# lms-07/LGTEUN

Hardware: AMD Instinct MI355X
Metric: train image-pairs/sec, GF-2 4-band 128x128, K=4, bs=32/GPU (higher is better)
Workload: dtype f32 (GEMMs and the local mixer: split 16-bit MFMA -- f16 pairs in the forward FFN, the W2 products of its backward and P V, bf16 triples elsewhere -- fp32 accumulate; fp32-equivalent); 1 GPU; BASELINE configs[1]: C=4, MS 32x32, PAN 128x128, K=4, 32 pairs/GPU, train step = fwd + L1 + bwd + Adam + StepLR tick; mode=faithful, global_batch=32, parallelism=dp1, dropout=True

## Files before the change

### include/lgteun_hip.h

```cpp
#ifndef LGTEUN_HIP_H
#define LGTEUN_HIP_H

#include <stddef.h>
#include <stdint.h>

#ifdef __cplusplus
extern "C" {
#endif

#define LG_TENSORS_SHARED 12
#define LG_TENSORS_PER_STAGE 119

#define LG_FLAG_FAITHFUL 1
#define LG_FLAG_SAVE 2
#define LG_FLAG_DROPOUT 4

#define LG_FLAG_BWD_LGT 8
#define LG_FLAG_BWD_DATA 16

#define LG_FLAG_CHAINED 32

#define LG_FLAG_DEFER_DEAD 64

enum lg_kernel_id {
    LG_K_NONE = 0, LG_K_FFN1, LG_K_FFN2, LG_K_FFT, LG_K_ATTN, LG_K_UPFUSE, LG_K_DOWN, LG_K_EMBED, LG_K_TAIL, LG_K_DATASTEP,
    LG_K_FFN1_BWD, LG_K_FFN2_BWD, LG_K_FFT_BWD, LG_K_ATTN_BWD, LG_K_WGRAD, LG_K_BATCH, LG_K_COUNT
};

typedef struct lg_config {
    int32_t C;
    int32_t K;
    int32_t H, W;
    int32_t precision;
    uint32_t variant;
} lg_config;

#define LG_VAR_FFN_IMPL_MASK 3u
#define LG_VAR_FFN_STRIP 1u
#define LG_VAR_FFN_TILE 2u
#define LG_VAR_FFN_XP 3u
#define LG_VAR_FFN_SAVE_MASK (3u << 2)
#define LG_VAR_FFN_SAVE3 (1u << 2)
#define LG_VAR_FFN_SAVE5 (2u << 2)
#define LG_VAR_FFN_BWD32_PAIR (1u << 4)
#define LG_VAR_FFN_DWBWD_TILE (1u << 5)
#define LG_VAR_ATTN_BWD_R3 (1u << 6)
#define LG_VAR_DSTEP_TILES (1u << 7)
#define LG_VAR_ATTN_FWD_VALU (1u << 8)
#define LG_VAR_FFN_BF16X3 (1u << 9)
#define LG_VAR_FFT_FULL (1u << 10)
#define LG_VAR_FFN_BWD_BF16X3 (1u << 11)
#define LG_VAR_ATTN_BWD_CORE_M (1u << 12)
#define LG_VAR_FFN_XS (1u << 13)
#define LG_VAR_ATTN_BF16X3 (1u << 14)
#define LG_VAR_FFN_H3_RECOMPUTE (1u << 15)
#define LG_VAR_ATTN_BWD_RESTATS (1u << 16)
#define LG_VAR_REDUCE_PER_BLOCK (1u << 17)
#define LG_VAR_ALL 0x3ffffu

typedef struct lg_plan lg_plan;

const char* lg_version(void);
#define LG_ABI_VERSION 2
int32_t lg_abi_version(void);
const char* lg_last_error(void);

int lg_plan_create(const lg_config* cfg, const int64_t* offsets, int32_t n_offsets, lg_plan** out);
void lg_plan_destroy(lg_plan* plan);
size_t lg_workspace_bytes(const lg_plan* plan, int32_t B, int32_t train);

int lgteun_forward(const lg_plan* plan, const float* params, const float* ms, const float* pan, float* out,
                   void* workspace, size_t workspace_bytes, int32_t B, int32_t flags, uint64_t seed, void* stream);

int lgteun_dead_forward(const lg_plan* plan, const float* params, void* workspace, size_t workspace_bytes, int32_t B, int32_t flags,
                        uint64_t seed, void* stream);

int lgteun_backward(const lg_plan* plan, const float* params, float* grads, const float* ms, const float* pan,
                    const float* dout, void* workspace, size_t workspace_bytes, int32_t B, int32_t flags,
                    uint64_t seed, void* stream);

int lg_l1_loss(const float* out, const float* gt, float* dout, float* loss_accum, int64_t n_local, int64_t n_global,
               float scale, void* stream);

int lg_adam_step(float* params, const float* grads, float* exp_avg, float* exp_avg_sq, const int64_t* ranges,
                 int32_t n_ranges, int64_t max_range, int32_t step, float lr, float beta1, float beta2, float eps,
                 float grad_scale, void* stream);

int lg_l2_loss(const float* out, const float* gt, float* dout, float* loss_accum, int64_t n_local, int64_t n_global,
               float scale, void* stream);

#define LG_OPT_ADAM 0
#define LG_OPT_ADAMW 1
#define LG_OPT_SGD 2
#define LG_OPT_RMSPROP 3
#define LG_OPT_AMSGRAD 1
#define LG_OPT_NESTEROV 2
#define LG_OPT_CENTERED 4
int lg_optim_step(float* params, const float* grads, float* state0, float* state1, float* state2, const int64_t* ranges,
                  int32_t n_ranges, int64_t max_range, int32_t step, int32_t algo, int32_t flags, double lr, double h0, double h1,
                  double eps, double weight_decay, double grad_scale, void* stream);

int lg_prof_enable(int32_t kernel_id, int32_t max_launches);
int lg_prof_reset(void);
void lg_prof_pause(int32_t paused);
int lg_prof_read(double* total_ms, int64_t* launches);
void lg_prof_disable(void);
const char* lg_kernel_name(int32_t kernel_id);

int lg_dropout_mask(uint64_t seed, int32_t stage, int32_t blk, int64_t first, int64_t n, float* out, void* stream);

int lg_op_resample(const float* x, float* y, int32_t planes, int32_t hi, int32_t wi, int32_t mode, void* stream);
int lg_op_data_step(const lg_plan* plan, const float* params, int32_t stage, const float* z_in, const float* ms,
                    const float* pan, float* z_out, float* tmp, int32_t B, void* stream);
int lg_op_lgt(const lg_plan* plan, const float* params, int32_t stage, const float* z, float* out, void* workspace,
              size_t workspace_bytes, int32_t B, int32_t flags, uint64_t seed, void* stream);
int lg_op_block(const lg_plan* plan, const float* params, int32_t stage, int32_t blk, int32_t which, const float* x,
                float* y, void* workspace, size_t workspace_bytes, int32_t B, void* stream);

int lg_op_block_bwd(const lg_plan* plan, const float* params, float* grads, int32_t stage, int32_t blk, int32_t which,
                    const float* x, const float* dy, float* dx, void* workspace, size_t workspace_bytes, int32_t B,
                    void* stream);

int lg_op_data_step_bwd(const lg_plan* plan, const float* params, float* grads, int32_t stage, const float* z_in, const float* ms,
                        const float* pan, const float* dz_out, float* dz_in, void* workspace, size_t workspace_bytes, int32_t B,
                        void* stream);
int lg_op_lgt_bwd(const lg_plan* plan, const float* params, float* grads, int32_t stage, const float* z, const float* dout, float* dz,
                  void* workspace, size_t workspace_bytes, int32_t B, int32_t flags, uint64_t seed, void* stream);

#define LG_IQA_PEAK 2047.5
#define LG_IQA_SSIM_TAPS 11
#define LG_IQA_SSIM_SIGMA 1.5
#define LG_IQA_Q_BLOCK 8
#define LG_IQA_RATIO 4
#define LG_IQA_QNR_BLOCK 32
#define LG_IQA_MTF_TAPS 41
#define LG_IQA_MTF_GAIN 0.15
#define LG_IQA_MAX_BANDS 16
size_t lg_iqa_workspace_bytes(int32_t B, int32_t C, int32_t H, int32_t W, int32_t no_ref);
int lg_iqa_ref(const float* pred, const float* gt, double* out, int32_t B, int32_t C, int32_t H, int32_t W, float scale,
               void* workspace, size_t workspace_bytes, void* stream);
int lg_iqa_no_ref(const float* pred, const float* pan, const float* ms, double* out, int32_t B, int32_t C, int32_t H, int32_t W,
                  float scale, void* workspace, size_t workspace_bytes, void* stream);

#define LG_DT_U8 0
#define LG_DT_U16 1
#define LG_DT_F32 2
int lg_pyr_down2(const void* pan, float* pan_l, int64_t planes, int32_t H, int32_t W, int32_t dtype, void* stream);
int lg_batch_assemble(const void* pan, const void* lr, const void* mul, const float* pan_l, int64_t N, const int32_t* idx, int64_t idx_offset,
                      const uint32_t* flips, float* o_pan, float* o_lr, float* o_mul, float* o_pan_l, int32_t B, int32_t C, int32_t H, int32_t W,
                      int32_t h, int32_t w, int32_t dtype, float divisor, int32_t n_div, float post_scale, void* stream);

#ifdef __cplusplus
}
#endif
#endif
```

### lgteun_amd/_lib.py

```python
import ctypes
import os
from ctypes import POINTER, c_char_p, c_double, c_float, c_int32, c_int64, c_size_t, c_uint64, c_void_p

_HERE = os.path.dirname(os.path.abspath(__file__))
LIB_PATH = os.environ.get('LGTEUN_HIP_LIB') or os.path.join(_HERE, '_lgteun_hip.so')

LG_FLAG_FAITHFUL = 1
LG_FLAG_SAVE = 2
LG_FLAG_DROPOUT = 4
LG_FLAG_BWD_LGT = 8
LG_FLAG_BWD_DATA = 16
LG_FLAG_CHAINED = 32
LG_FLAG_DEFER_DEAD = 64
KERNEL_IDS = {n: i for i, n in enumerate(['none', 'ffn1', 'ffn', 'fft', 'attn', 'upfuse', 'down', 'embed', 'tail', 'datastep', 'ffn1_bwd',
                                           'ffn2_bwd', 'fft_bwd', 'attn_bwd', 'wgrad', 'batch'])}


class LgConfig(ctypes.Structure):
    _fields_ = [('C', c_int32), ('K', c_int32), ('H', c_int32), ('W', c_int32), ('precision', c_int32), ('variant', ctypes.c_uint32)]


LG_VAR_FFN_STRIP, LG_VAR_FFN_TILE, LG_VAR_FFN_XP = 1, 2, 3
LG_VAR_FFN_SAVE3, LG_VAR_FFN_SAVE5 = 1 << 2, 2 << 2
LG_VAR_FFN_BWD32_PAIR, LG_VAR_FFN_DWBWD_TILE, LG_VAR_ATTN_BWD_R3 = 1 << 4, 1 << 5, 1 << 6
LG_VAR_DSTEP_TILES = 1 << 7
LG_VAR_ATTN_FWD_VALU = 1 << 8
LG_VAR_FFN_BF16X3 = 1 << 9
LG_VAR_FFT_FULL = 1 << 10
LG_VAR_FFN_BWD_BF16X3 = 1 << 11
LG_VAR_ATTN_BWD_CORE_M = 1 << 12
LG_VAR_FFN_XS = 1 << 13
LG_VAR_ATTN_BF16X3 = 1 << 14
LG_VAR_FFN_H3_RECOMPUTE = 1 << 15
LG_VAR_ATTN_BWD_RESTATS = 1 << 16
LG_VAR_REDUCE_PER_BLOCK = 1 << 17
LG_OPT_ADAM, LG_OPT_ADAMW, LG_OPT_SGD, LG_OPT_RMSPROP = 0, 1, 2, 3
LG_OPT_AMSGRAD, LG_OPT_NESTEROV, LG_OPT_CENTERED = 1, 2, 4
LG_DT_U8, LG_DT_U16, LG_DT_F32 = 0, 1, 2
LG_ABI_VERSION = 2


def variant_from_env(env=None):
    env = os.environ if env is None else env
    v = {'strip': LG_VAR_FFN_STRIP, 'tile': LG_VAR_FFN_TILE, 'xp': LG_VAR_FFN_XP}.get(env.get('LG_FFN_IMPL', ''), 0)
    v |= {'3': LG_VAR_FFN_SAVE3, '5': LG_VAR_FFN_SAVE5}.get(env.get('LG_FFN_SAVE', ''), 0)
    if env.get('LG_FFN_BWD32') == 'pair':
        v |= LG_VAR_FFN_BWD32_PAIR
    if env.get('LG_FFN_DWBWD') == 'tile':
        v |= LG_VAR_FFN_DWBWD_TILE
    if env.get('LG_ATTN_BWD') in ('old', 'r3'):
        v |= LG_VAR_ATTN_BWD_R3
    if env.get('LG_DSTEP') == 'tiles':
        v |= LG_VAR_DSTEP_TILES
    if env.get('LG_ATTN_FWD', '') == 'valu':
        v |= LG_VAR_ATTN_FWD_VALU
    if env.get('LG_FFN_SPLIT', '') == 'bf16x3':
        v |= LG_VAR_FFN_BF16X3
    if env.get('LG_FFT', '') == 'full':
        v |= LG_VAR_FFT_FULL
    if env.get('LG_FFN_BWD_SPLIT', '') == 'bf16x3':
        v |= LG_VAR_FFN_BWD_BF16X3
    if env.get('LG_ATTN_BWD_CORE', '') == 'm':
        v |= LG_VAR_ATTN_BWD_CORE_M
    if env.get('LG_FFN_FWD', '') == 'xs':
        v |= LG_VAR_FFN_XS
    if env.get('LG_ATTN_SPLIT', '') == 'bf16x3':
        v |= LG_VAR_ATTN_BF16X3
    if env.get('LG_FFN_H3', '') == 'recompute':
        v |= LG_VAR_FFN_H3_RECOMPUTE
    if env.get('LG_ATTN_BWD_STATS', '') == 'recompute':
        v |= LG_VAR_ATTN_BWD_RESTATS
    if env.get('LG_REDUCE', '') == 'per_block':
        v |= LG_VAR_REDUCE_PER_BLOCK
    return v


class LgteunHipError(RuntimeError):
    pass


_lib = None

SIGNATURES = {
    'lg_version': (c_char_p, []),
    'lg_abi_version': (c_int32, []),
    'lg_last_error': (c_char_p, []),
    'lg_plan_create': (c_int32, [POINTER(LgConfig), POINTER(c_int64), c_int32, POINTER(c_void_p)]),
    'lg_plan_destroy': (None, [c_void_p]),
    'lg_workspace_bytes': (c_size_t, [c_void_p, c_int32, c_int32]),
    'lgteun_forward': (c_int32, [c_void_p, c_void_p, c_void_p, c_void_p, c_void_p, c_void_p, c_size_t, c_int32, c_int32,
                                 c_uint64, c_void_p]),
    'lgteun_backward': (c_int32, [c_void_p, c_void_p, c_void_p, c_void_p, c_void_p, c_void_p, c_void_p, c_size_t, c_int32,
                                  c_int32, c_uint64, c_void_p]),
    'lgteun_dead_forward': (c_int32, [c_void_p, c_void_p, c_void_p, c_size_t, c_int32, c_int32, c_uint64, c_void_p]),
    'lg_l1_loss': (c_int32, [c_void_p, c_void_p, c_void_p, c_void_p, c_int64, c_int64, c_float, c_void_p]),
    'lg_adam_step': (c_int32, [c_void_p, c_void_p, c_void_p, c_void_p, c_void_p, c_int32, c_int64, c_int32, c_float, c_float,
                               c_float, c_float, c_float, c_void_p]),
    'lg_l2_loss': (c_int32, [c_void_p, c_void_p, c_void_p, c_void_p, c_int64, c_int64, c_float, c_void_p]),
    'lg_optim_step': (c_int32, [c_void_p, c_void_p, c_void_p, c_void_p, c_void_p, c_void_p, c_int32, c_int64, c_int32, c_int32, c_int32,
                                c_double, c_double, c_double, c_double, c_double, c_double, c_void_p]),
    'lg_op_resample': (c_int32, [c_void_p, c_void_p, c_int32, c_int32, c_int32, c_int32, c_void_p]),
    'lg_op_data_step': (c_int32, [c_void_p, c_void_p, c_int32, c_void_p, c_void_p, c_void_p, c_void_p, c_void_p, c_int32,
                                  c_void_p]),
    'lg_op_lgt': (c_int32, [c_void_p, c_void_p, c_int32, c_void_p, c_void_p, c_void_p, c_size_t, c_int32, c_int32, c_uint64,
                            c_void_p]),
    'lg_op_block': (c_int32, [c_void_p, c_void_p, c_int32, c_int32, c_int32, c_void_p, c_void_p, c_void_p, c_size_t, c_int32,
                              c_void_p]),
    'lg_dropout_mask': (c_int32, [c_uint64, c_int32, c_int32, c_int64, c_int64, c_void_p, c_void_p]),
    'lg_prof_enable': (c_int32, [c_int32, c_int32]),
    'lg_prof_reset': (c_int32, []),
    'lg_prof_pause': (None, [c_int32]),
    'lg_prof_read': (c_int32, [POINTER(ctypes.c_double), POINTER(c_int64)]),
    'lg_prof_disable': (None, []),
    'lg_kernel_name': (c_char_p, [c_int32]),
    'lg_op_data_step_bwd': (c_int32, [c_void_p, c_void_p, c_void_p, c_int32, c_void_p, c_void_p, c_void_p, c_void_p, c_void_p, c_void_p,
                                      c_size_t, c_int32, c_void_p]),
    'lg_op_lgt_bwd': (c_int32, [c_void_p, c_void_p, c_void_p, c_int32, c_void_p, c_void_p, c_void_p, c_void_p, c_size_t, c_int32, c_int32,
                                c_uint64, c_void_p]),
    'lg_op_block_bwd': (c_int32, [c_void_p, c_void_p, c_void_p, c_int32, c_int32, c_int32, c_void_p, c_void_p, c_void_p, c_void_p,
                                  c_size_t, c_int32, c_void_p]),
    'lg_iqa_workspace_bytes': (c_size_t, [c_int32, c_int32, c_int32, c_int32, c_int32]),
    'lg_iqa_ref': (c_int32, [c_void_p, c_void_p, c_void_p, c_int32, c_int32, c_int32, c_int32, c_float, c_void_p, c_size_t, c_void_p]),
    'lg_iqa_no_ref': (c_int32, [c_void_p, c_void_p, c_void_p, c_void_p, c_int32, c_int32, c_int32, c_int32, c_float, c_void_p, c_size_t,
                                c_void_p]),
    'lg_pyr_down2': (c_int32, [c_void_p, c_void_p, c_int64, c_int32, c_int32, c_int32, c_void_p]),
    'lg_batch_assemble': (c_int32, [c_void_p, c_void_p, c_void_p, c_void_p, c_int64, c_void_p, c_int64, c_void_p, c_void_p, c_void_p, c_void_p,
                                    c_void_p, c_int32, c_int32, c_int32, c_int32, c_int32, c_int32, c_int32, c_float, c_int32, c_float, c_void_p]),
}


def lib():
    global _lib
    if _lib is None:
        if not os.path.exists(LIB_PATH):
            raise LgteunHipError(
                f'HIP extension not built: {LIB_PATH} is missing. Run `make` (or __graft_entry__.build()). '
                'lgteun_amd has no CPU/PyTorch fallback.')
        L = ctypes.CDLL(LIB_PATH)
        for name, (res, args) in SIGNATURES.items():
            fn = getattr(L, name)
            fn.restype = res
            fn.argtypes = args
        got = int(L.lg_abi_version())
        if got != LG_ABI_VERSION:
            raise LgteunHipError(f'{LIB_PATH}: ABI version {got}, this binding was written for {LG_ABI_VERSION} (include/lgteun_hip.h): rebuild with `make`')
        _lib = L
    return _lib


def check(rc, what):
    if rc != 0:
        msg = lib().lg_last_error().decode(errors='replace')
        raise LgteunHipError(f'{what} failed (rc={rc}): {msg}')
```

### lgteun_amd/csrc/api.hip

```cpp
#include <stdarg.h>
#include <stdio.h>
#include <stdlib.h>
#include <string.h>
#include <math.h>
#include <atomic>
#include <mutex>

#pragma GCC visibility push(default)
#include "../../include/lgteun_hip.h"
#pragma GCC visibility pop

#include "kernels.h"
#include "workspace.h"
#include "backward.h"

static thread_local char g_err[512] = "";

void lg_set_error(const char* fmt, ...) {
    va_list ap;
    va_start(ap, fmt);
    vsnprintf(g_err, sizeof(g_err), fmt, ap);
    va_end(ap);
}

static struct {
    std::atomic<int> kid{0};
    std::atomic<int> paused{0};
    int cap = 0, n = 0;
    hipEvent_t* ev = nullptr;
    std::mutex mu;
} g_prof;

void lg_prof_begin(int kid, hipStream_t s) {
    if (kid != g_prof.kid.load(std::memory_order_relaxed) || g_prof.paused.load(std::memory_order_relaxed)) return;
    std::lock_guard<std::mutex> lk(g_prof.mu);
    if (kid != g_prof.kid.load(std::memory_order_relaxed) || g_prof.n >= g_prof.cap) return;
    hipEventRecord(g_prof.ev[2 * g_prof.n], s);
}
void lg_prof_end(int kid, hipStream_t s) {
    if (kid != g_prof.kid.load(std::memory_order_relaxed) || g_prof.paused.load(std::memory_order_relaxed)) return;
    std::lock_guard<std::mutex> lk(g_prof.mu);
    if (kid != g_prof.kid.load(std::memory_order_relaxed) || g_prof.n >= g_prof.cap) return;
    hipEventRecord(g_prof.ev[2 * g_prof.n + 1], s);
    g_prof.n++;
}
static void prof_disable_locked() {
    for (int i = 0; i < 2 * g_prof.cap; ++i) hipEventDestroy(g_prof.ev[i]);
    free(g_prof.ev);
    g_prof.ev = nullptr;
    g_prof.cap = g_prof.n = 0;
    g_prof.kid.store(0);
    g_prof.paused.store(0);
}
extern "C" void lg_prof_disable(void) {
    std::lock_guard<std::mutex> lk(g_prof.mu);
    prof_disable_locked();
}
extern "C" int lg_prof_enable(int32_t kernel_id, int32_t max_launches) {
    if (kernel_id <= 0 || kernel_id >= LG_K_COUNT || max_launches <= 0) { lg_set_error("prof_enable: invalid argument"); return -1; }
    std::lock_guard<std::mutex> lk(g_prof.mu);
    prof_disable_locked();
    g_prof.ev = (hipEvent_t*)malloc(sizeof(hipEvent_t) * 2 * max_launches);
    for (int i = 0; i < 2 * max_launches; ++i) {
        hipError_t e = hipEventCreate(&g_prof.ev[i]);
        if (e != hipSuccess) { lg_set_error("prof_enable: hipEventCreate: %s", hipGetErrorString(e)); return (int)e; }
    }
    g_prof.cap = max_launches;
    g_prof.kid.store(kernel_id);
    return 0;
}
extern "C" void lg_prof_pause(int32_t paused) { g_prof.paused.store(paused ? 1 : 0); }
extern "C" int lg_prof_reset(void) {
    std::lock_guard<std::mutex> lk(g_prof.mu);
    g_prof.n = 0;
    return 0;
}
extern "C" int lg_prof_read(double* total_ms, int64_t* launches) {
    if (!total_ms || !launches) { lg_set_error("prof_read: null argument"); return -1; }
    std::lock_guard<std::mutex> lk(g_prof.mu);
    double tot = 0.0;
    for (int i = 0; i < g_prof.n; ++i) {
        hipError_t e = hipEventSynchronize(g_prof.ev[2 * i + 1]);
        if (e != hipSuccess) { lg_set_error("prof_read: %s", hipGetErrorString(e)); return (int)e; }
        float ms = 0.f;
        hipEventElapsedTime(&ms, g_prof.ev[2 * i], g_prof.ev[2 * i + 1]);
        tot += ms;
    }
    *total_ms = tot;
    *launches = g_prof.n;
    return 0;
}
extern "C" const char* lg_kernel_name(int32_t k) {
    static const char* names[LG_K_COUNT] = {"none", "k_ffn1", "fused FFN forward (k_ffn_xr e=16 / k_ffn_x32 e=32 / k_ffn1_x64+k_ffn2_x64 e=64)", "k_fftmix", "k_attn", "k_upfuse", "k_down", "k_embed", "k_tail",
                                            "k_resample_dw", "k_ffn1_bwd", "k_ffn2_bwd", "k_fftmix_bwd", "k_attn_bwd", "k_wgrad", "k_batch_assemble"};
    return (k >= 0 && k < LG_K_COUNT) ? names[k] : "?";
}

extern "C" const char* lg_version(void) { return "lgteun_hip 0.2 (gfx950)"; }
extern "C" int32_t lg_abi_version(void) { return LG_ABI_VERSION; }
extern "C" const char* lg_last_error(void) { return g_err; }

extern "C" int lg_plan_create(const lg_config* cfg, const int64_t* offsets, int32_t n_offsets, lg_plan** out) {
    if (!cfg || !offsets || !out) { lg_set_error("plan_create: null argument"); return -1; }
    if (cfg->C != 4 && cfg->C != 8) { lg_set_error("plan_create: C must be 4 or 8 (got %d)", cfg->C); return -2; }
    if (cfg->precision != 0 && cfg->precision != 1) { lg_set_error("plan_create: precision must be 0 (fp32) or 1 (bf16 hidden storage)"); return -2; }
    if (cfg->K < 1 || cfg->K > LG_MAX_K) { lg_set_error("plan_create: K out of range (%d)", cfg->K); return -2; }
    if (cfg->H % 16 || cfg->W % 16 || cfg->H <= 0 || cfg->W <= 0) { lg_set_error("plan_create: H,W must be positive multiples of 16"); return -2; }
    if (cfg->H > 1024 || cfg->W > 1024) {
        lg_set_error("plan_create: PAN sizes up to 1024x1024 are supported (got %dx%d)", cfg->H, cfg->W);
        return -2;
    }
    const int expect = S_NSHARED + cfg->K + L_NSLOT * cfg->K;
    if (n_offsets != expect) { lg_set_error("plan_create: expected %d offsets, got %d", expect, n_offsets); return -2; }
    for (int i = 0; i < n_offsets; ++i)
        if (offsets[i] < 0 || (offsets[i] & 3)) { lg_set_error("plan_create: offset %d (=%lld) must be a non-negative multiple of 4 floats", i, (long long)offsets[i]); return -2; }
    if (cfg->variant & ~LG_VAR_ALL) { lg_set_error("plan_create: unknown variant bits 0x%x", cfg->variant & ~LG_VAR_ALL); return -2; }
    if ((cfg->variant & LG_VAR_FFN_SAVE_MASK) == LG_VAR_FFN_SAVE_MASK) { lg_set_error("plan_create: invalid FFN save variant"); return -2; }
#ifndef LG_BUILD_AB
    if ((cfg->variant & LG_VAR_FFN_IMPL_MASK) >= LG_VAR_FFN_TILE) { lg_set_error("plan_create: FFN variants 2 / 3 exist in `make AB=1` builds only"); return -2; }
    if (cfg->precision == 1 && (cfg->variant & LG_VAR_FFN_IMPL_MASK)) { lg_set_error("plan_create: precision = 1 with an FFN variant exists in `make AB=1` builds only"); return -2; }
#endif
    lg_plan* p = new lg_plan;
    p->cfg = *cfg;
    p->n_offsets = n_offsets;
    {
        const uint32_t v = cfg->variant;
        p->ffn_tile = (int)(v & LG_VAR_FFN_IMPL_MASK);
        const uint32_t sv = v & LG_VAR_FFN_SAVE_MASK;
        p->save_mode = sv == LG_VAR_FFN_SAVE5 ? 5 : (sv == LG_VAR_FFN_SAVE3 ? 3 : 2);
        p->bwd32_old = (v & LG_VAR_FFN_BWD32_PAIR) ? 1 : 0;
        p->dwbwd_tile = (v & LG_VAR_FFN_DWBWD_TILE) ? 1 : 0;
        p->attn_bwd_old = (v & LG_VAR_ATTN_BWD_R3) ? 1 : 0;
        p->dstep_tiles = (v & LG_VAR_DSTEP_TILES) ? 1 : 0;
        p->attn_fwd_valu = (v & LG_VAR_ATTN_FWD_VALU) ? 1 : 0;
        p->ffn_bf16x3 = (v & LG_VAR_FFN_BF16X3) ? 1 : 0;
        p->fft_full = (v & LG_VAR_FFT_FULL) ? 1 : 0;
        p->attn_bwd_core_m = (v & LG_VAR_ATTN_BWD_CORE_M) ? 1 : 0;
        p->ffn_bwd_bf16x3 = (v & LG_VAR_FFN_BWD_BF16X3) ? 1 : 0;
        p->ffn_xs = (v & LG_VAR_FFN_XS) ? 1 : 0;
        p->attn_bf16x3 = (v & LG_VAR_ATTN_BF16X3) ? 1 : 0;
        p->ffn_h3_re = (v & LG_VAR_FFN_H3_RECOMPUTE) ? 1 : 0;
        p->attn_restats = (v & LG_VAR_ATTN_BWD_RESTATS) ? 1 : 0;
        p->reduce_per_block = (v & LG_VAR_REDUCE_PER_BLOCK) ? 1 : 0;
    }
    p->off = (int64_t*)malloc(sizeof(int64_t) * n_offsets);
    memcpy(p->off, offsets, sizeof(int64_t) * n_offsets);
    *out = p;
    return 0;
}

extern "C" void lg_plan_destroy(lg_plan* plan) {
    if (!plan) return;
    free(plan->off);
    delete plan;
}

extern "C" size_t lg_workspace_bytes(const lg_plan* plan, int32_t B, int32_t train) {
    if (!plan || B <= 0 || train < 0 || train > 2) return 0;
    NetBufs nb;
    carve(plan, B, train, nullptr, nb);
    size_t fwd = nb.bytes;
    if (train) fwd += bwd_workspace_bytes(plan, B);
    return fwd;
}

static int data_step_fwd(const lg_plan* pl, const float* P, int stage, const float* z_in, const float* ms, const float* pan,
                         float* z_out, float* t1, float* r, float* s1, float* pr, int B, hipStream_t s) {
    const lg_config& c = pl->cfg;
    const int planes = B * c.C, H = c.H, W = c.W;
    if (pl->dstep_fused(H, W)) {
        DstepFwdArgs f;
        f.z = z_in; f.ms = ms; f.pan = pan; f.zout = z_out; f.t1 = t1; f.r = r; f.s1 = s1; f.pr = pr;
        f.d1w = P + pl->shared(S_D1W); f.d1b = P + pl->shared(S_D1B); f.d3w = P + pl->shared(S_D3W); f.d3b = P + pl->shared(S_D3B);
        f.dt1w = P + pl->shared(S_DT1W); f.dt1b = P + pl->shared(S_DT1B); f.dt3w = P + pl->shared(S_DT3W); f.dt3b = P + pl->shared(S_DT3B);
        f.rw = P + pl->shared(S_RW); f.rb = P + pl->shared(S_RB); f.rtw = P + pl->shared(S_RTW); f.rtb = P + pl->shared(S_RTB);
        f.eta = P + pl->eta(stage);
        f.B = B; f.C = c.C; f.N = H;
        return launch_dstep_fwd(f, s);
    }
    DwArgs a;
    memset(&a, 0, sizeof(a));
    a.C = c.C; a.planes = planes;
    int rc;
    a.in = z_in; a.out = t1; a.w9 = P + pl->shared(S_D1W); a.bias = P + pl->shared(S_D1B);
    a.hi = H; a.wi = W; a.ho = H / 2; a.wo = W / 2;
    if ((rc = launch_resample_dw(0, 0, a, s))) return rc;
    a.in = t1; a.out = r; a.w9 = P + pl->shared(S_D3W); a.bias = P + pl->shared(S_D3B); a.sub = ms;
    a.hi = H / 2; a.wi = W / 2; a.ho = H / 4; a.wo = W / 4;
    if ((rc = launch_resample_dw(0, 1, a, s))) return rc;
    a.in = r; a.out = s1; a.w9 = P + pl->shared(S_DT1W); a.bias = P + pl->shared(S_DT1B); a.sub = nullptr;
    a.hi = H / 4; a.wi = W / 4; a.ho = H / 2; a.wo = W / 2;
    if ((rc = launch_resample_dw(1, 0, a, s))) return rc;
    a.in = s1; a.out = z_out; a.w9 = P + pl->shared(S_DT3W); a.bias = P + pl->shared(S_DT3B);
    a.z = z_in; a.pan = pan; a.rw = P + pl->shared(S_RW); a.rb = P + pl->shared(S_RB);
    a.rtw = P + pl->shared(S_RTW); a.rtb = P + pl->shared(S_RTB); a.eta = P + pl->eta(stage);
    a.hi = H / 2; a.wi = W / 2; a.ho = H; a.wo = W;
    return launch_resample_dw(1, 2, a, s);
}

static int block_mixer_fwd(const lg_plan* pl, const float* P, int stage, int j, const BlockBufs& bb, const float* posT, int B,
                           int flags, uint64_t seed, hipStream_t s, float* fft_scratch = nullptr, const float* attn_scales = nullptr) {
    int rc;
    FftArgs f;
    f.g = bb.g; f.o = bb.o2;
    f.amp = (flags & LG_FLAG_SAVE) ? bb.amp : nullptr;
    f.pha = (flags & LG_FLAG_SAVE) ? bb.pha : nullptr;
    f.sgn = (flags & LG_FLAG_SAVE) ? bb.sgn : nullptr;
    f.scratch = fft_scratch;
    f.ampw = P + pl->blk(stage, j, B_AMPW); f.ampb = P + pl->blk(stage, j, B_AMPB);
    f.phaw = P + pl->blk(stage, j, B_PHAW); f.phab = P + pl->blk(stage, j, B_PHAB);
    f.ch = bb.e / 2; f.planes = B * f.ch; f.n = bb.h; f.h = bb.h; f.w = bb.w; f.full = pl->fft_full;
    if ((rc = launch_fftmix(f, s))) return rc;
    AttnArgs t;
    t.x = bb.xin; t.o2 = bb.o2; t.y = bb.xmid; t.posT = posT; t.pos = P + pl->blk(stage, j, B_POS);
    t.bf16 = pl->cfg.precision == 1 ? 1 : 0;
    t.ln1g = P + pl->blk(stage, j, B_LN1G); t.ln1b = P + pl->blk(stage, j, B_LN1B);
    t.qkvw = P + pl->blk(stage, j, B_QKVW); t.qkvb = P + pl->blk(stage, j, B_QKVB);
    t.projw = P + pl->blk(stage, j, B_PROJW); t.projb = P + pl->blk(stage, j, B_PROJB);
    t.B = B; t.h = bb.h; t.w = bb.w;
    t.dropout = (flags & LG_FLAG_DROPOUT) ? 1 : 0;
    t.seed = mix_seed(seed, stage, j);
    t.scales = (attn_scales && pl->attn_f16x2()) ? attn_scales + ((size_t)stage * 5 + j) * 4 : nullptr;
    if ((flags & LG_FLAG_SAVE) && pl->attn_saves_stats(bb.e)) { t.save_o = bb.att_o; t.save_l = bb.att_l; }
    return pl->attn_fwd_valu ? launch_attn(bb.e, t, s) : launch_attn_m(bb.e, t, s);
}

static int block_ffn_fwd(const lg_plan* pl, const float* P, int stage, int j, const BlockBufs& bb, float* g_next, int next_blk,
                         int B, int flags, hipStream_t s, float* wsplit, const float* ffn_scales) {
    int rc;
    Ffn1Args a1;
    const bool pre = pl->ffn_saves_preact(bb.e);
    const bool noh1 = pl->ffn_bwd_x(bb.e) || pl->ffn1_bwd_x32(bb.e);
    a1.x = bb.xmid; a1.a1s = ((flags & LG_FLAG_SAVE) && !noh1) ? bb.a1 : nullptr; a1.g1s = ((flags & LG_FLAG_SAVE) && !pre && !noh1) ? bb.g1 : nullptr; a1.h2 = bb.h2;
    a1.ln2g = P + pl->blk(stage, j, B_LN2G); a1.ln2b = P + pl->blk(stage, j, B_LN2B);
    a1.w1 = P + pl->blk(stage, j, B_W1); a1.b1 = P + pl->blk(stage, j, B_B1);
    a1.w2 = P + pl->blk(stage, j, B_W2); a1.b2 = P + pl->blk(stage, j, B_B2);
    a1.P = (long)B * bb.h * bb.w;
    a1.hbf = pl->hidden_bf16(bb.e) ? 1 : 0;
    a1.tile16 = pl->ffn_tile ? pl->ffn_tile : ((pl->ffn_xs && bb.e == 16) ? 4 : 0);
    a1.wsplit = wsplit ? wsplit + ((size_t)stage * 5 + j) * (ffn_wsplit_bytes(8 * pl->cfg.C) / sizeof(float)) : nullptr;
    a1.wsplit_ready = (wsplit && bb.e >= 32) ? 1 : 0;
    a1.scales = pl->ffn_f16x2(bb.e) ? ffn_scales + ((size_t)stage * 5 + j) * 8 : nullptr;
    Ffn2Args a2;
    a2.h2 = bb.h2; a2.x = bb.xmid; a2.a3s = ((flags & LG_FLAG_SAVE) && !pl->ffn_h3_recompute(bb.e)) ? bb.a3 : nullptr; a2.g3s = ((flags & LG_FLAG_SAVE) && !pre && !pl->ffn_dw_x32(bb.e, bb.h, bb.w)) ? bb.g3 : nullptr; a2.y = bb.xout;
    a2.g = g_next;
    a2.dww = P + pl->blk(stage, j, B_DWW); a2.dwb = P + pl->blk(stage, j, B_DWB);
    a2.w3 = P + pl->blk(stage, j, B_W3); a2.b3 = P + pl->blk(stage, j, B_B3);
    a2.n1g = g_next ? P + pl->blk(stage, next_blk, B_LN1G) : nullptr;
    a2.n1b = g_next ? P + pl->blk(stage, next_blk, B_LN1B) : nullptr;
    a2.B = B; a2.h = bb.h; a2.w = bb.w; a2.hbf = a1.hbf;
    a1.h2 = ((flags & LG_FLAG_SAVE) || bb.e == 64) ? bb.h2 : nullptr;
    rc = launch_ffn_fused(bb.e, a1, a2, s);
    if (rc != LG_FFN_NOT_FUSED) return rc;
    a1.h2 = bb.h2;
    if ((rc = launch_ffn1(bb.e, a1, s))) return rc;
    return launch_ffn2(bb.e, a2, s);
}

static int pos_transpose_stages(const lg_plan* pl, const float* P, int st0, int st1, float* posT_all, hipStream_t s) {
    if (st1 <= st0) return 0;
    const float* src[5 * LG_MAX_K];
    float* dst[5 * LG_MAX_K];
    int n = 0;
    for (int st = st0; st < st1; ++st)
        for (int j = 0; j < 5; ++j, ++n) { src[n] = P + pl->blk(st, j, B_POS); dst[n] = posT_all + ((size_t)st * 5 + j) * 2 * 64 * 64; }
    return launch_pos_transpose_n(n, src, dst, s);
}
static int prep_stages(const lg_plan* pl, const float* P, int st0, int st1, NetBufs& nb, hipStream_t s) {
    int rc = pl->attn_fwd_valu ? pos_transpose_stages(pl, P, st0, st1, nb.posT, s) : 0;
    if (rc || st1 <= st0) return rc;
    const int E = 4 * pl->cfg.C;
    if (pl->ffn_f16x2(E) || pl->ffn_f16x2(2 * E)) {
        FfnPrepJob jobs[5 * LG_MAX_K];
        int n = 0;
        for (int st = st0; st < st1; ++st)
            for (int j = 0; j < 5; ++j, ++n) {
                FfnPrepJob& q = jobs[n];
                q.ln2g = P + pl->blk(st, j, B_LN2G); q.ln2b = P + pl->blk(st, j, B_LN2B);
                q.w1 = P + pl->blk(st, j, B_W1); q.b1 = P + pl->blk(st, j, B_B1); q.w2 = P + pl->blk(st, j, B_W2); q.b2 = P + pl->blk(st, j, B_B2);
                q.dww = P + pl->blk(st, j, B_DWW); q.dwb = P + pl->blk(st, j, B_DWB); q.w3 = P + pl->blk(st, j, B_W3);
                q.e = j == 2 ? 2 * E : E;
                q.ln1g = P + pl->blk(st, j, B_LN1G); q.ln1b = P + pl->blk(st, j, B_LN1B); q.qkvw = P + pl->blk(st, j, B_QKVW); q.qkvb = P + pl->blk(st, j, B_QKVB);
            }
        if ((rc = launch_ffn_scales(n, jobs, nb.ffn_scales + (size_t)st0 * 5 * 8, s, pl->attn_f16x2() ? nb.attn_scales + (size_t)st0 * 5 * 4 : nullptr))) return rc;
    }
    SplitWJob sj[5 * LG_MAX_K];
    int ns = 0;
    const size_t slot = ffn_wsplit_bytes(2 * E) / sizeof(float);
    for (int st = st0; st < st1; ++st)
        for (int j = 0; j < 5; ++j) {
            const int e = j == 2 ? 2 * E : E;
            if (e < 32 || e % 32) continue;
            SplitWJob& q = sj[ns++];
            q.w1 = P + pl->blk(st, j, B_W1); q.w2 = P + pl->blk(st, j, B_W2); q.w3 = P + pl->blk(st, j, B_W3);
            q.e = e; q.np = pl->hidden_bf16(e) ? 1 : (pl->ffn_f16x2(e) ? 2 : 3);
            q.scales = q.np == 2 ? nb.ffn_scales + ((size_t)st * 5 + j) * 8 : nullptr;
            q.out = nb.wsplit + ((size_t)st * 5 + j) * slot;
        }
    return ns ? launch_split_w_jobs(ns, sj, s) : 0;
}

static int lgt_fwd(const lg_plan* pl, const float* P, int stage, const float* z, float* out, NetBufs& nb, int B, int flags,
                   uint64_t seed, hipStream_t s, bool pos_ready = false) {
    const lg_config& c = pl->cfg;
    const int E = 4 * c.C;
    int rc;
    float* posT = nb.posT + (size_t)stage * 5 * 2 * 64 * 64;
    if (!pos_ready && (rc = prep_stages(pl, P, stage, stage + 1, nb, s))) return rc;
    EmbedArgs ea;
    ea.z = z; ea.x = nb.x0; ea.g = nb.blk[0].g;
    ea.dww = P + pl->lgt(stage, L_PE_DWW); ea.dwb = P + pl->lgt(stage, L_PE_DWB);
    ea.w = P + pl->lgt(stage, L_PE_W); ea.b = P + pl->lgt(stage, L_PE_B);
    ea.lng = P + pl->lgt(stage, L_PE_LNG); ea.lnb = P + pl->lgt(stage, L_PE_LNB);
    ea.n1g = P + pl->blk(stage, 0, B_LN1G); ea.n1b = P + pl->blk(stage, 0, B_LN1B);
    ea.HW = c.H * c.W; ea.total = (long)B * c.H * c.W;
    if ((rc = launch_embed(c.C, ea, s))) return rc;
    if ((rc = block_mixer_fwd(pl, P, stage, 0, nb.blk[0], posT + 0 * 8192, B, flags, seed, s, nb.fft_scratch, nb.attn_scales))) return rc;
    if ((rc = block_ffn_fwd(pl, P, stage, 0, nb.blk[0], nb.blk[1].g, 1, B, flags, s, nb.wsplit, nb.ffn_scales))) return rc;
    if ((rc = block_mixer_fwd(pl, P, stage, 1, nb.blk[1], posT + 1 * 8192, B, flags, seed, s, nb.fft_scratch, nb.attn_scales))) return rc;
    if ((rc = block_ffn_fwd(pl, P, stage, 1, nb.blk[1], nullptr, 0, B, flags, s, nb.wsplit, nb.ffn_scales))) return rc;
    DownArgs da;
    da.x = nb.blk[1].xout; da.y = nb.blk[2].xin; da.g = nb.blk[2].g;
    da.u_save = (flags & LG_FLAG_SAVE) ? nb.u_down : nullptr;
    da.w = P + pl->lgt(stage, L_DOWNW); da.b = P + pl->lgt(stage, L_DOWNB);
    da.n1g = P + pl->blk(stage, 2, B_LN1G); da.n1b = P + pl->blk(stage, 2, B_LN1B);
    da.B = B; da.H = c.H; da.W = c.W;
    if ((rc = launch_down(E, da, s))) return rc;
    if ((rc = block_mixer_fwd(pl, P, stage, 2, nb.blk[2], posT + 2 * 8192, B, flags, seed, s, nb.fft_scratch, nb.attn_scales))) return rc;
    if ((rc = block_ffn_fwd(pl, P, stage, 2, nb.blk[2], nullptr, 0, B, flags, s, nb.wsplit, nb.ffn_scales))) return rc;
    UpFuseArgs ua;
    ua.xb = nb.blk[2].xout; ua.skip = nb.blk[1].xout; ua.y = nb.blk[3].xin; ua.g = nb.blk[3].g;
    ua.t_save = (flags & LG_FLAG_SAVE) ? nb.t_up : nullptr;
    ua.upw = P + pl->lgt(stage, L_UPW); ua.upb = P + pl->lgt(stage, L_UPB);
    ua.fw = P + pl->lgt(stage, L_FUSEW); ua.fb = P + pl->lgt(stage, L_FUSEB);
    ua.n1g = P + pl->blk(stage, 3, B_LN1G); ua.n1b = P + pl->blk(stage, 3, B_LN1B);
    ua.B = B; ua.H = c.H; ua.W = c.W;
    if ((rc = launch_upfuse(E, ua, s))) return rc;
    if ((rc = block_mixer_fwd(pl, P, stage, 3, nb.blk[3], posT + 3 * 8192, B, flags, seed, s, nb.fft_scratch, nb.attn_scales))) return rc;
    if ((rc = block_ffn_fwd(pl, P, stage, 3, nb.blk[3], nb.blk[4].g, 4, B, flags, s, nb.wsplit, nb.ffn_scales))) return rc;
    if ((rc = block_mixer_fwd(pl, P, stage, 4, nb.blk[4], posT + 4 * 8192, B, flags, seed, s, nb.fft_scratch, nb.attn_scales))) return rc;
    if ((rc = block_ffn_fwd(pl, P, stage, 4, nb.blk[4], nullptr, 0, B, flags, s, nb.wsplit, nb.ffn_scales))) return rc;
    TailArgs ta;
    ta.x = nb.blk[4].xout; ta.z = z; ta.out = out;
    ta.w = P + pl->lgt(stage, L_TAILW); ta.b = P + pl->lgt(stage, L_TAILB);
    ta.HW = c.H * c.W; ta.total = (long)B * c.H * c.W;
    return launch_tail(c.C, ta, s);
}

extern "C" int lgteun_forward(const lg_plan* plan, const float* params, const float* ms, const float* pan, float* out,
                              void* workspace, size_t workspace_bytes, int32_t B, int32_t flags, uint64_t seed, void* stream) {
    if (!plan || !params || !ms || !pan || !out || !workspace || B <= 0) { lg_set_error("forward: null/invalid argument"); return -1; }
    const bool chained = (flags & LG_FLAG_CHAINED) != 0;
    const int train = (flags & LG_FLAG_SAVE) ? (chained ? 2 : 1) : 0;
    if (workspace_bytes < lg_workspace_bytes(plan, B, train)) {
        lg_set_error("forward: workspace too small (%zu < %zu)", workspace_bytes, lg_workspace_bytes(plan, B, train));
        return -3;
    }
    hipStream_t s = (hipStream_t)stream;
    const lg_config& c = plan->cfg;
    NetBufs nb;
    carve(plan, B, train, workspace, nb);
    int rc;
    const bool all_stages = chained || ((flags & LG_FLAG_FAITHFUL) && !(flags & LG_FLAG_DEFER_DEAD));
    if ((rc = prep_stages(plan, params, all_stages ? 0 : c.K - 1, c.K, nb, s))) return rc;
    if ((rc = launch_resample(2, ms, nb.Z[0], B * c.C, c.H / 4, c.W / 4, s))) return rc;
    if (chained) {
        for (int i = 0; i < c.K; ++i) {
            if ((rc = data_step_fwd(plan, params, i, nb.X[i], ms, pan, nb.Z[i + 1], nb.t1[i], nb.r[i], nb.s1[i], nb.pr, B, s))) return rc;
            NetBufs sv = (train == 2) ? stage_view(nb, i) : nb;
            if ((rc = lgt_fwd(plan, params, i, nb.Z[i + 1], i == c.K - 1 ? out : nb.X[i + 1], sv, B, flags, seed, s, true))) return rc;
        }
        return 0;
    }
    for (int i = 0; i < c.K; ++i) {
        if ((rc = data_step_fwd(plan, params, i, nb.Z[i], ms, pan, nb.Z[i + 1], nb.t1[i], nb.r[i], nb.s1[i], nb.pr, B, s))) return rc;
        const bool last = (i == c.K - 1);
        if (last) {
            if ((rc = lgt_fwd(plan, params, i, nb.Z[i + 1], out, nb, B, flags, seed, s, true))) return rc;
        } else if ((flags & LG_FLAG_FAITHFUL) && !(flags & LG_FLAG_DEFER_DEAD)) {
            if ((rc = lgt_fwd(plan, params, i, nb.Z[i + 1], nb.deadout, nb, B, flags & ~LG_FLAG_SAVE, seed, s, true))) return rc;
        }
    }
    return 0;
}

extern "C" int lgteun_dead_forward(const lg_plan* plan, const float* params, void* workspace, size_t workspace_bytes, int32_t B,
                                   int32_t flags, uint64_t seed, void* stream) {
    if (!plan || !params || !workspace || B <= 0) { lg_set_error("dead_forward: null/invalid argument"); return -1; }
    if ((flags & LG_FLAG_CHAINED) || !(flags & LG_FLAG_FAITHFUL)) { lg_set_error("dead_forward: only the faithful unfolding has dead stages"); return -2; }
    const int train = (flags & LG_FLAG_SAVE) ? 1 : 0;
    if (workspace_bytes < lg_workspace_bytes(plan, B, train)) { lg_set_error("dead_forward: workspace too small"); return -3; }
    NetBufs nb;
    carve(plan, B, train, workspace, nb);
    {
        const int rc = prep_stages(plan, params, 0, plan->cfg.K - 1, nb, (hipStream_t)stream);
        if (rc) return rc;
    }
    for (int i = 0; i + 1 < plan->cfg.K; ++i) {
        const int rc = lgt_fwd(plan, params, i, nb.Z[i + 1], nb.deadout, nb, B, flags & ~LG_FLAG_SAVE, seed, (hipStream_t)stream, true);
        if (rc) return rc;
    }
    return 0;
}

extern "C" int lgteun_backward(const lg_plan* plan, const float* params, float* grads, const float* ms, const float* pan,
                               const float* dout, void* workspace, size_t workspace_bytes, int32_t B, int32_t flags, uint64_t seed,
                               void* stream) {
    if (!plan || !params || !grads || !ms || !pan || !dout || !workspace || B <= 0) { lg_set_error("backward: null/invalid argument"); return -1; }
    const int train = (flags & LG_FLAG_CHAINED) ? 2 : 1;
    if ((flags & LG_FLAG_CHAINED) && (flags & (LG_FLAG_BWD_LGT | LG_FLAG_BWD_DATA))) {
        lg_set_error("backward: LG_FLAG_BWD_LGT / LG_FLAG_BWD_DATA do not apply to LG_FLAG_CHAINED");
        return -2;
    }
    if (workspace_bytes < lg_workspace_bytes(plan, B, train)) { lg_set_error("backward: workspace too small"); return -3; }
    NetBufs nb;
    carve(plan, B, train, workspace, nb);
    return net_backward(plan, params, grads, ms, pan, dout, nb, (char*)workspace + nb.bytes, B, flags, seed, (hipStream_t)stream);
}

extern "C" int lg_op_resample(const float* x, float* y, int32_t planes, int32_t hi, int32_t wi, int32_t mode, void* stream) {
    if (!x || !y || planes <= 0 || hi <= 0 || wi <= 0 || mode < 0 || mode > 2) { lg_set_error("op_resample: invalid argument"); return -1; }
    if (mode == 0 && ((hi & 1) || (wi & 1))) { lg_set_error("op_resample: x0.5 needs even sizes"); return -2; }
    return launch_resample(mode, x, y, planes, hi, wi, (hipStream_t)stream);
}

extern "C" int lg_op_data_step(const lg_plan* plan, const float* params, int32_t stage, const float* z_in, const float* ms,
                               const float* pan, float* z_out, float* tmp, int32_t B, void* stream) {
    if (!plan || !params || !z_in || !ms || !pan || !z_out || !tmp || stage < 0 || stage >= plan->cfg.K) { lg_set_error("op_data_step: invalid argument"); return -1; }
    const lg_config& c = plan->cfg;
    size_t q = (size_t)B * c.C * c.H * c.W / 4;
    return data_step_fwd(plan, params, stage, z_in, ms, pan, z_out, tmp, tmp + q, tmp + 2 * q, tmp + 3 * q, B, (hipStream_t)stream);
}

extern "C" int lg_op_lgt(const lg_plan* plan, const float* params, int32_t stage, const float* z, float* out, void* workspace,
                         size_t workspace_bytes, int32_t B, int32_t flags, uint64_t seed, void* stream) {
    if (!plan || !params || !z || !out || !workspace || stage < 0 || stage >= plan->cfg.K) { lg_set_error("op_lgt: invalid argument"); return -1; }
    const int train = (flags & LG_FLAG_SAVE) ? 1 : 0;
    if (workspace_bytes < lg_workspace_bytes(plan, B, train)) { lg_set_error("op_lgt: workspace too small"); return -3; }
    NetBufs nb;
    carve(plan, B, train, workspace, nb);
    return lgt_fwd(plan, params, stage, z, out, nb, B, flags, seed, (hipStream_t)stream);
}

extern "C" int lg_op_block(const lg_plan* plan, const float* params, int32_t stage, int32_t blk, int32_t which, const float* x,
                           float* y, void* workspace, size_t workspace_bytes, int32_t B, void* stream) {
    if (!plan || !params || !x || !y || !workspace || stage < 0 || stage >= plan->cfg.K || blk < 0 || blk > 4 || which < 0 || which > 2) {
        lg_set_error("op_block: invalid argument");
        return -1;
    }
    if (workspace_bytes < lg_workspace_bytes(plan, B, 0)) { lg_set_error("op_block: workspace too small"); return -3; }
    hipStream_t s = (hipStream_t)stream;
    NetBufs nb;
    carve(plan, B, 0, workspace, nb);
    BlockBufs bb = nb.blk[blk];
    int rc;
    const size_t npix = (size_t)B * bb.h * bb.w;
    if (which == 0 || which == 1) {
        if ((rc = launch_ln_split(bb.e, x, params + plan->blk(stage, blk, B_LN1G), params + plan->blk(stage, blk, B_LN1B), bb.g, B,
                                  bb.h * bb.w, s)))
            return rc;
    }
    if (which == 0) {
        FftArgs f;
        f.g = bb.g; f.o = y; f.amp = nullptr; f.pha = nullptr; f.sgn = nullptr; f.scratch = nb.fft_scratch;
        f.ampw = params + plan->blk(stage, blk, B_AMPW); f.ampb = params + plan->blk(stage, blk, B_AMPB);
        f.phaw = params + plan->blk(stage, blk, B_PHAW); f.phab = params + plan->blk(stage, blk, B_PHAB);
        f.ch = bb.e / 2; f.planes = B * f.ch; f.n = bb.h; f.h = bb.h; f.w = bb.w; f.full = plan->fft_full;
        return launch_fftmix(f, s);
    }
    if (which == 1) {
        float* posT = nb.posT;
        if ((rc = prep_stages(plan, params, stage, stage + 1, nb, s))) return rc;
        if ((rc = launch_pos_transpose(params + plan->blk(stage, blk, B_POS), posT, s))) return rc;
        bb.xin = const_cast<float*>(x);
        bb.xmid = y;
        return block_mixer_fwd(plan, params, stage, blk, bb, posT, B, 0, 0, s, nb.fft_scratch, nb.attn_scales);
    }
    bb.xmid = const_cast<float*>(x);
    bb.xout = y;
    (void)npix;
    if ((rc = prep_stages(plan, params, stage, stage + 1, nb, s))) return rc;
    return block_ffn_fwd(plan, params, stage, blk, bb, nullptr, 0, B, 0, s, nb.wsplit, nb.ffn_scales);
}

extern "C" int lg_op_block_bwd(const lg_plan* plan, const float* params, float* grads, int32_t stage, int32_t blk, int32_t which,
                               const float* x, const float* dy, float* dx, void* workspace, size_t workspace_bytes, int32_t B,
                               void* stream) {
    if (!plan || !params || !grads || !x || !dy || !dx || !workspace || stage < 0 || stage >= plan->cfg.K || blk < 0 || blk > 4 ||
        which < 0 || which > 2) {
        lg_set_error("op_block_bwd: invalid argument");
        return -1;
    }
    if (workspace_bytes < lg_workspace_bytes(plan, B, 1)) { lg_set_error("op_block_bwd: workspace too small"); return -3; }
    hipStream_t s = (hipStream_t)stream;
    NetBufs nb;
    carve(plan, B, 1, workspace, nb);
    BlockBufs& bb = nb.blk[blk];
    int rc;
    if (which == 0 || which == 1) {
        if ((rc = launch_ln_split(bb.e, x, params + plan->blk(stage, blk, B_LN1G), params + plan->blk(stage, blk, B_LN1B), bb.g, B,
                                  bb.h * bb.w, s)))
            return rc;
        if ((rc = prep_stages(plan, params, stage, stage + 1, nb, s))) return rc;
        if ((rc = launch_pos_transpose(params + plan->blk(stage, blk, B_POS), nb.posT, s))) return rc;
        bb.xin = const_cast<float*>(x);
        if ((rc = block_mixer_fwd(plan, params, stage, blk, bb, nb.posT, B, LG_FLAG_SAVE, 0, s, nb.fft_scratch, nb.attn_scales))) return rc;
    } else {
        bb.xmid = const_cast<float*>(x);
        if ((rc = prep_stages(plan, params, stage, stage + 1, nb, s))) return rc;
        if ((rc = block_ffn_fwd(plan, params, stage, blk, bb, nullptr, 0, B, LG_FLAG_SAVE, s, nb.wsplit, nb.ffn_scales))) return rc;
    }
    return op_block_bwd(plan, params, grads, stage, blk, which, dy, dx, nb, (char*)workspace + nb.bytes, B, s);
}

extern "C" int lg_op_data_step_bwd(const lg_plan* plan, const float* params, float* grads, int32_t stage, const float* z_in,
                                   const float* ms, const float* pan, const float* dz_out, float* dz_in, void* workspace,
                                   size_t workspace_bytes, int32_t B, void* stream) {
    if (!plan || !params || !grads || !z_in || !ms || !pan || !dz_out || !dz_in || !workspace || B <= 0 || stage < 0 || stage >= plan->cfg.K) {
        lg_set_error("op_data_step_bwd: invalid argument");
        return -1;
    }
    if (workspace_bytes < lg_workspace_bytes(plan, B, 1)) { lg_set_error("op_data_step_bwd: workspace too small"); return -3; }
    hipStream_t s = (hipStream_t)stream;
    NetBufs nb;
    carve(plan, B, 1, workspace, nb);
    int rc;
    if ((rc = data_step_fwd(plan, params, stage, z_in, ms, pan, nb.Z[stage + 1], nb.t1[stage], nb.r[stage], nb.s1[stage], nb.pr, B, s))) return rc;
    return op_data_step_bwd(plan, params, grads, stage, nb, (char*)workspace + nb.bytes, z_in, pan, dz_out, dz_in, B, s);
}

extern "C" int lg_op_lgt_bwd(const lg_plan* plan, const float* params, float* grads, int32_t stage, const float* z, const float* dout,
                             float* dz, void* workspace, size_t workspace_bytes, int32_t B, int32_t flags, uint64_t seed, void* stream) {
    if (!plan || !params || !grads || !z || !dout || !dz || !workspace || B <= 0 || stage < 0 || stage >= plan->cfg.K) {
        lg_set_error("op_lgt_bwd: invalid argument");
        return -1;
    }
    if (flags & ~LG_FLAG_DROPOUT) { lg_set_error("op_lgt_bwd: only LG_FLAG_DROPOUT applies"); return -2; }
    if (workspace_bytes < lg_workspace_bytes(plan, B, 1)) { lg_set_error("op_lgt_bwd: workspace too small"); return -3; }
    hipStream_t s = (hipStream_t)stream;
    NetBufs nb;
    carve(plan, B, 1, workspace, nb);
    int rc;
    if ((rc = lgt_fwd(plan, params, stage, z, nb.deadout, nb, B, flags | LG_FLAG_SAVE, seed, s))) return rc;
    return op_lgt_bwd(plan, params, grads, stage, nb, (char*)workspace + nb.bytes, z, dout, dz, B, flags, seed, s);
}

__global__ __launch_bounds__(256) void k_dropout_mask(uint64_t seed, long first, long n, float* __restrict__ out) {
    for (long i = blockIdx.x * 256L + threadIdx.x; i < n; i += gridDim.x * 256L) out[i] = dropout_scale(seed, (uint64_t)(first + i));
}
extern "C" int lg_dropout_mask(uint64_t seed, int32_t stage, int32_t blk, int64_t first, int64_t n, float* out, void* stream) {
    if (!out || n < 0 || first < 0 || stage < 0 || stage >= LG_MAX_K || blk < 0 || blk > 4) { lg_set_error("dropout_mask: invalid argument"); return -1; }
    if (n == 0) return 0;
    const int grid = (int)((n + 255) / 256 < 1024 ? (n + 255) / 256 : 1024);
    k_dropout_mask<<<grid, 256, 0, (hipStream_t)stream>>>(mix_seed(seed, stage, blk), first, n, out);
    LG_CHECK_LAUNCH();
    return 0;
}

__global__ __launch_bounds__(256) void k_l1(const float* __restrict__ out, const float* __restrict__ gt, float* __restrict__ dout,
                                            float* loss_accum, long n, float inv_n, float gscale) {
    float part = 0.f;
    const long n4 = n >> 2, stride = (long)gridDim.x * 256L;
    const float4* __restrict__ o4 = reinterpret_cast<const float4*>(out);
    const float4* __restrict__ g4 = reinterpret_cast<const float4*>(gt);
    float4* __restrict__ d4 = reinterpret_cast<float4*>(dout);
    auto one = [&](float d) { part += fabsf(d); return d > 0.f ? gscale : (d < 0.f ? -gscale : 0.f); };
    long i = blockIdx.x * 256L + threadIdx.x;
    for (; i + 3 * stride < n4; i += 4 * stride) {
        float4 a[4], b[4];
#pragma unroll
        for (int u = 0; u < 4; ++u) { a[u] = o4[i + u * stride]; b[u] = g4[i + u * stride]; }
#pragma unroll
        for (int u = 0; u < 4; ++u)
            d4[i + u * stride] = make_float4(one(a[u].x - b[u].x), one(a[u].y - b[u].y), one(a[u].z - b[u].z), one(a[u].w - b[u].w));
    }
    for (; i < n4; i += stride) {
        const float4 a = o4[i], b = g4[i];
        d4[i] = make_float4(one(a.x - b.x), one(a.y - b.y), one(a.z - b.z), one(a.w - b.w));
    }
    for (long j = 4 * n4 + blockIdx.x * 256L + threadIdx.x; j < n; j += stride) dout[j] = one(out[j] - gt[j]);
#pragma unroll
    for (int off = 32; off > 0; off >>= 1) part += __shfl_xor(part, off);
    __shared__ float sm[4];
    if ((threadIdx.x & 63) == 0) sm[threadIdx.x >> 6] = part;
    __syncthreads();
    if (threadIdx.x == 0) atomicAdd(loss_accum, (sm[0] + sm[1] + sm[2] + sm[3]) * inv_n);
}

extern "C" int lg_l1_loss(const float* out, const float* gt, float* dout, float* loss_accum, int64_t n_local, int64_t n_global,
                          float scale, void* stream) {
    if (!out || !gt || !dout || !loss_accum || n_local <= 0 || n_global <= 0) { lg_set_error("l1_loss: invalid argument"); return -1; }
    if (((uintptr_t)out | (uintptr_t)gt | (uintptr_t)dout) & 15) { lg_set_error("l1_loss: tensors must be 16-byte aligned"); return -1; }
    int grid = (int)((n_local / 4 + 255) / 256);
    if (grid > 256) grid = 256;
    if (grid < 1) grid = 1;
    k_l1<<<grid, 256, 0, (hipStream_t)stream>>>(out, gt, dout, loss_accum, n_local, 1.0f / (float)n_global, scale / (float)n_global);
    LG_CHECK_LAUNCH();
    return 0;
}

#define LG_L2_SLOTS 64
struct l2_slot { double acc; unsigned int arrived; unsigned int pad; };
__device__ l2_slot g_l2_slots[LG_L2_SLOTS];

__global__ __launch_bounds__(256) void k_l2(const float* __restrict__ out, const float* __restrict__ gt, float* __restrict__ dout,
                                            float* loss_accum, long n, double inv_n, float norm, float scale, int slot_id) {
    l2_slot* slot = &g_l2_slots[slot_id];
    double part = 0.0;
    const long n4 = n >> 2, stride = (long)gridDim.x * 256L;
    const float4* __restrict__ o4 = reinterpret_cast<const float4*>(out);
    const float4* __restrict__ g4 = reinterpret_cast<const float4*>(gt);
    float4* __restrict__ d4 = reinterpret_cast<float4*>(dout);
    auto one = [&](float d) { part += (double)d * (double)d; return (norm * d) * scale; };
    long i = blockIdx.x * 256L + threadIdx.x;
    for (; i + 3 * stride < n4; i += 4 * stride) {
        float4 a[4], b[4];
#pragma unroll
        for (int u = 0; u < 4; ++u) { a[u] = o4[i + u * stride]; b[u] = g4[i + u * stride]; }
#pragma unroll
        for (int u = 0; u < 4; ++u)
            d4[i + u * stride] = make_float4(one(a[u].x - b[u].x), one(a[u].y - b[u].y), one(a[u].z - b[u].z), one(a[u].w - b[u].w));
    }
    for (; i < n4; i += stride) {
        const float4 a = o4[i], b = g4[i];
        d4[i] = make_float4(one(a.x - b.x), one(a.y - b.y), one(a.z - b.z), one(a.w - b.w));
    }
    for (long j = 4 * n4 + blockIdx.x * 256L + threadIdx.x; j < n; j += stride) dout[j] = one(out[j] - gt[j]);
#pragma unroll
    for (int off = 32; off > 0; off >>= 1) part += __shfl_xor(part, off);
    __shared__ double sm[4];
    if ((threadIdx.x & 63) == 0) sm[threadIdx.x >> 6] = part;
    __syncthreads();
    if (threadIdx.x == 0) {
        atomicAdd(&slot->acc, sm[0] + sm[1] + sm[2] + sm[3]);
        __threadfence();
        if (atomicAdd(&slot->arrived, 1u) == gridDim.x - 1) {
            __threadfence();
            const double total = __longlong_as_double((long long)atomicExch((unsigned long long*)&slot->acc, 0ull));
            atomicExch(&slot->arrived, 0u);
            atomicAdd(loss_accum, (float)(total * inv_n));
        }
    }
}

extern "C" int lg_l2_loss(const float* out, const float* gt, float* dout, float* loss_accum, int64_t n_local, int64_t n_global,
                          float scale, void* stream) {
    if (!out || !gt || !dout || !loss_accum || n_local <= 0 || n_global <= 0) { lg_set_error("l2_loss: invalid argument"); return -1; }
    if (((uintptr_t)out | (uintptr_t)gt | (uintptr_t)dout) & 15) { lg_set_error("l2_loss: tensors must be 16-byte aligned"); return -1; }
    int grid = (int)((n_local / 4 + 255) / 256);
    if (grid > 256) grid = 256;
    if (grid < 1) grid = 1;
    static std::atomic<unsigned> next_slot{0};
    k_l2<<<grid, 256, 0, (hipStream_t)stream>>>(out, gt, dout, loss_accum, n_local, 1.0 / (double)n_global, (float)(2.0 / (double)n_global), scale,
                                                (int)(next_slot.fetch_add(1) % LG_L2_SLOTS));
    LG_CHECK_LAUNCH();
    return 0;
}

extern "C" int lg_pyr_down2(const void* pan, float* pan_l, int64_t planes, int32_t H, int32_t W, int32_t dtype, void* stream) {
    return launch_pyr_down2(pan, pan_l, planes, H, W, dtype, (hipStream_t)stream);
}
extern "C" int lg_batch_assemble(const void* pan, const void* lr, const void* mul, const float* pan_l, int64_t N, const int32_t* idx, int64_t idx_offset,
                                 const uint32_t* flips, float* o_pan, float* o_lr, float* o_mul, float* o_pan_l, int32_t B, int32_t C, int32_t H, int32_t W,
                                 int32_t h, int32_t w, int32_t dtype, float divisor, int32_t n_div, float post_scale, void* stream) {
    return launch_batch_assemble(pan, lr, mul, pan_l, N, idx, idx_offset, flips, o_pan, o_lr, o_mul, o_pan_l, B, C, H, W, h, w, dtype, divisor, n_div,
                                 post_scale, (hipStream_t)stream);
}

extern "C" size_t lg_iqa_workspace_bytes(int32_t B, int32_t C, int32_t H, int32_t W, int32_t no_ref) {
    return iqa_workspace_bytes(B, C, H, W, no_ref);
}
extern "C" int lg_iqa_ref(const float* pred, const float* gt, double* out, int32_t B, int32_t C, int32_t H, int32_t W, float scale,
                          void* workspace, size_t workspace_bytes, void* stream) {
    return launch_iqa_ref(pred, gt, out, B, C, H, W, scale, workspace, workspace_bytes, (hipStream_t)stream);
}
extern "C" int lg_iqa_no_ref(const float* pred, const float* pan, const float* ms, double* out, int32_t B, int32_t C, int32_t H, int32_t W,
                             float scale, void* workspace, size_t workspace_bytes, void* stream) {
    return launch_iqa_no_ref(pred, pan, ms, out, B, C, H, W, scale, workspace, workspace_bytes, (hipStream_t)stream);
}

__global__ __launch_bounds__(256) void k_adam(float* __restrict__ p, const float* __restrict__ g, float* __restrict__ m,
                                              float* __restrict__ v, const int64_t* __restrict__ ranges, float step_size, float b1,
                                              float b2, float inv_bc2_sqrt, float eps, float gscale) {
    const int64_t lo = ranges[2 * blockIdx.y], hi = ranges[2 * blockIdx.y + 1];
    for (int64_t i = lo + blockIdx.x * 256L + threadIdx.x; i < hi; i += (int64_t)gridDim.x * 256L) {
        float gi = g[i] * gscale;
        float mi = b1 * m[i] + (1.0f - b1) * gi;
        float vi = b2 * v[i] + (1.0f - b2) * gi * gi;
        m[i] = mi;
        v[i] = vi;
        float denom = sqrtf(vi) * inv_bc2_sqrt + eps;
        p[i] = p[i] - step_size * (mi / denom);
    }
}

extern "C" int lg_adam_step(float* params, const float* grads, float* exp_avg, float* exp_avg_sq, const int64_t* ranges,
                            int32_t n_ranges, int64_t max_range, int32_t step, float lr, float beta1, float beta2, float eps,
                            float grad_scale, void* stream) {
    if (!params || !grads || !exp_avg || !exp_avg_sq || !ranges || n_ranges <= 0 || step < 1) { lg_set_error("adam_step: invalid argument"); return -1; }
    double bc1 = 1.0 - pow((double)beta1, (double)step);
    double bc2 = 1.0 - pow((double)beta2, (double)step);
    int gx = (int)((max_range + 255) / 256);
    if (gx < 1) gx = 1;
    if (gx > 512) gx = 512;
    dim3 grid(gx, n_ranges);
    k_adam<<<grid, 256, 0, (hipStream_t)stream>>>(params, grads, exp_avg, exp_avg_sq, ranges, (float)(lr / bc1), beta1, beta2,
                                                   (float)(1.0 / sqrt(bc2)), eps, grad_scale);
    LG_CHECK_LAUNCH();
    return 0;
}

enum { OPT_WD = 1, OPT_ALT = 2, OPT_MOM = 4, OPT_FIRST = 8 };
struct optim_args {
    float lr;
    float h0, h1;
    float c0, c1;
    float eps, wd, gscale;
    float bc2_sqrt;
    float decay;
};

#ifndef LG_OPT_FMA
#define LG_OPT_FMA(a, b, c) __builtin_fmaf(a, b, c)
#endif
template <int ALGO, int OPT>
__global__ __launch_bounds__(256) void k_optim(float* __restrict__ p, const float* __restrict__ g, float* __restrict__ s0,
                                               float* __restrict__ s1, float* __restrict__ s2, const int64_t* __restrict__ ranges,
                                               optim_args a) {
#pragma clang fp contract(off)
    const int64_t lo = ranges[2 * blockIdx.y], hi = ranges[2 * blockIdx.y + 1];
    for (int64_t i = lo + blockIdx.x * 256L + threadIdx.x; i < hi; i += (int64_t)gridDim.x * 256L) {
        float pi = p[i];
        float gi = g[i] * a.gscale;
        if constexpr (ALGO == LG_OPT_ADAMW) pi = pi * a.decay;
        else if constexpr ((OPT & OPT_WD) != 0) gi = LG_OPT_FMA(a.wd, pi, gi);
        if constexpr (ALGO == LG_OPT_ADAM || ALGO == LG_OPT_ADAMW) {
            float mi = s0[i];
            mi = LG_OPT_FMA(a.c0, gi - mi, mi);
            const float vb = s1[i] * a.h1;
            float vi = LG_OPT_FMA(a.c1, gi * gi, vb);
            s0[i] = mi;
            s1[i] = vi;
            if constexpr ((OPT & OPT_ALT) != 0) { vi = fmaxf(s2[i], vi); s2[i] = vi; }
            float denom = sqrtf(vi) / a.bc2_sqrt;
// ... 90 lines not shown
```

### lgteun_amd/csrc/common.h

```cpp
#pragma once
#include <hip/hip_runtime.h>
#include <stdint.h>
#include <stddef.h>
#include <atomic>
#include "../../include/lgteun_hip.h"

enum SharedSlot { S_D1W, S_D1B, S_D3W, S_D3B, S_DT1W, S_DT1B, S_DT3W, S_DT3B, S_RW, S_RB, S_RTW, S_RTB, S_NSHARED };

enum BlockSlot {
    B_POS, B_QKVW, B_QKVB, B_AMPW, B_AMPB, B_PHAW, B_PHAB, B_PROJW, B_PROJB, B_LN1G, B_LN1B,
    B_W1, B_B1, B_W2, B_B2, B_DWW, B_DWB, B_W3, B_B3, B_LN2G, B_LN2B, B_NSLOT
};
enum LgtSlot {
    L_PE_DWW = 0, L_PE_DWB, L_PE_W, L_PE_B, L_PE_LNG, L_PE_LNB,
    L_ENC0 = 6, L_ENC1 = 27, L_DOWNW = 48, L_DOWNB, L_BOTT = 50, L_UPW = 71, L_UPB, L_FUSEW, L_FUSEB,
    L_DEC0 = 75, L_DEC1 = 96, L_TAILW = 117, L_TAILB, L_NSLOT = 119
};
static inline int block_base(int blk) {
    const int b[5] = {L_ENC0, L_ENC1, L_BOTT, L_DEC0, L_DEC1};
    return b[blk];
}

struct lg_plan {
    lg_config cfg;
    int n_offsets;
    int ffn_tile;
    int save_mode;
    int dwbwd_tile;
    bool hidden_bf16(int e) const { return cfg.precision == 1 && e != 64; }
    int attn_bwd_old;
    int ffn_bwd_bf16x3;
    int attn_bwd_core_m;
    int fft_full;
    int ffn_bf16x3;
    bool ffn_f16x2(int e) const { return cfg.precision == 0 && ffn_tile == 0 && !ffn_bf16x3 && (e == 16 || e == 32 || e == 64); }
    int attn_restats;
    int ffn_h3_re;
    bool ffn_h3_recompute(int e) const { return e == 16 && ffn_bwd_x(e) && cfg.precision == 0 && !dwbwd_tile && ffn_h3_re && !ffn_xs && ffn_f16x2(e); }
    int ffn_xs;
    int attn_bf16x3;
    bool attn_saves_stats(int e) const { return cfg.precision == 0 && !attn_fwd_valu && !attn_restats && !(e == 32 && attn_bwd_core_m); }
    bool attn_f16x2() const { return cfg.precision == 0 && !attn_bf16x3 && !attn_fwd_valu && ffn_tile == 0 && !ffn_bf16x3; }
    int attn_fwd_valu;
    int reduce_per_block;
    int dstep_tiles;
    bool dstep_fused(int h, int w) const;
    int bwd32_old;
    bool ffn1_bwd_x32(int e) const { return e == 32 && ffn_tile == 0 && !bwd32_old; }
    bool ffn_dw_x32(int e, int h, int w) const { return e == 32 && ffn_tile == 0 && !dwbwd_tile && (h & 7) == 0 && (w & 15) == 0; }
    bool ffn_bwd_x(int e) const { return e == 16 && ffn_tile == 0 && save_mode == 2; }
    bool ffn_saves_preact(int e) const { return e == 16 && ffn_tile == 0 && (save_mode == 2 || (save_mode == 3 && cfg.precision == 0)); }
    int64_t* off;
    int64_t shared(int s) const { return off[s]; }
    int64_t eta(int i) const { return off[S_NSHARED + i]; }
    int64_t lgt(int stage, int slot) const { return off[S_NSHARED + cfg.K + stage * L_NSLOT + slot]; }
    int64_t blk(int stage, int b, int slot) const { return lgt(stage, block_base(b) + slot); }
};

void lg_set_error(const char* fmt, ...);

struct DeviceOnce {
    std::atomic<uint64_t> mask{0};
    static int dev() { int d = 0; (void)hipGetDevice(&d); return d & 63; }
    bool need() const { return !((mask.load(std::memory_order_acquire) >> dev()) & 1); }
    void done() { mask.fetch_or(1ull << dev(), std::memory_order_release); }
};

static inline uint64_t mix_seed(uint64_t seed, int stage, int blk) {
    uint64_t z = seed + 0x9E3779B97F4A7C15ull * (uint64_t)(stage * 8 + blk + 1);
    z = (z ^ (z >> 30)) * 0xBF58476D1CE4E5B9ull;
    z = (z ^ (z >> 27)) * 0x94D049BB133111EBull;
    return z ^ (z >> 31);
}


#define LG_CHECK_LAUNCH()                                                              \
    do {                                                                               \
        hipError_t e__ = hipGetLastError();                                            \
        if (e__ != hipSuccess) {                                                       \
            lg_set_error("%s:%d launch failed: %s", __FILE__, __LINE__, hipGetErrorString(e__)); \
            return (int)e__;                                                           \
        }                                                                              \
    } while (0)

#define LG_EPS 1e-5f

void lg_prof_begin(int kid, hipStream_t s);
void lg_prof_end(int kid, hipStream_t s);
struct ProfScope {
    int kid;
    hipStream_t s;
    ProfScope(int k, hipStream_t st) : kid(k), s(st) { lg_prof_begin(kid, s); }
    ~ProfScope() { lg_prof_end(kid, s); }
};

#ifdef __HIPCC__
__device__ __forceinline__ float erfc_abs_f(float az) {
    const float t = __builtin_amdgcn_rcpf(1.0f + 0.3275911f * az);
    const float poly = ((((1.061405429f * t - 1.453152027f) * t + 1.421413741f) * t - 0.284496736f) * t + 0.254829592f) * t;
    return poly * __expf(-az * az);
}
__device__ __forceinline__ float gelu_f(float x) {
    const float z = x * 0.70710678118654752440f;
    const float e = 0.5f * erfc_abs_f(fabsf(z));
    const float phi = z >= 0.f ? 1.0f - e : e;
    return x * phi;
}
__device__ __forceinline__ void gelu_both_f(float x, float& a, float& g) {
    const float az = fabsf(x) * 0.70710678118654752440f;
    const float t = __builtin_amdgcn_rcpf(1.0f + 0.3275911f * az);
    const float poly = ((((1.061405429f * t - 1.453152027f) * t + 1.421413741f) * t - 0.284496736f) * t + 0.254829592f) * t;
    const float ex = __expf(-az * az);
    const float e = 0.5f * poly * ex;
    const float cdf = x >= 0.f ? 1.0f - e : e;
    a = x * cdf;
    g = cdf + x * (0.39894228040143267794f * ex);
}
typedef float lg_v2f __attribute__((ext_vector_type(2)));
__device__ __forceinline__ lg_v2f gelu2_core(lg_v2f x, lg_v2f& absx, lg_v2f& ex) {
    absx = (lg_v2f){fabsf(x.x), fabsf(x.y)};
    const lg_v2f az = absx * 0.70710678118654752440f;
    const lg_v2f d = az * 0.3275911f + 1.0f;
    const lg_v2f t = (lg_v2f){__builtin_amdgcn_rcpf(d.x), __builtin_amdgcn_rcpf(d.y)};
    const lg_v2f poly = ((((1.061405429f * t - 1.453152027f) * t + 1.421413741f) * t - 0.284496736f) * t + 0.254829592f) * t;
    const lg_v2f m = az * az * -1.44269504088896340736f;
    ex = (lg_v2f){__builtin_amdgcn_exp2f(m.x), __builtin_amdgcn_exp2f(m.y)};
    return poly * ex * -0.5f + 0.5f;
}
__device__ __forceinline__ lg_v2f gelu2_f(lg_v2f x) {
    lg_v2f absx, ex;
    const lg_v2f sv = gelu2_core(x, absx, ex);
    return absx * sv + x * 0.5f;
}
__device__ __forceinline__ void gelu2_both_f(lg_v2f x, lg_v2f& a, lg_v2f& g) {
    lg_v2f absx, ex;
    const lg_v2f sv = gelu2_core(x, absx, ex);
    a = absx * sv + x * 0.5f;
    const lg_v2f cs = (lg_v2f){copysignf(sv.x, x.x), copysignf(sv.y, x.y)};
    g = x * (ex * 0.39894228040143267794f) + (cs + 0.5f);
}
__device__ __forceinline__ lg_v2f gelu2_scaled(lg_v2f x, float c1, float hr) {
    const lg_v2f absx = (lg_v2f){fabsf(x.x), fabsf(x.y)};
    const lg_v2f az = absx * c1;
    const lg_v2f d = az * 0.3275911f + 1.0f;
    const lg_v2f t = (lg_v2f){__builtin_amdgcn_rcpf(d.x), __builtin_amdgcn_rcpf(d.y)};
    const lg_v2f poly = ((((1.061405429f * t - 1.453152027f) * t + 1.421413741f) * t - 0.284496736f) * t + 0.254829592f) * t;
    const lg_v2f m = az * az * -1.44269504088896340736f;
    const lg_v2f ex = (lg_v2f){__builtin_amdgcn_exp2f(m.x), __builtin_amdgcn_exp2f(m.y)};
    const lg_v2f sv = poly * ex * (0.0f - hr) + hr;
    return absx * sv + x * hr;
}
struct GeluK { float k1, kd, hr, a1, a2, a3, a4, a5; };
__device__ __forceinline__ GeluK gelu_k(float c1, float hr) {
    GeluK k;
    k.k1 = c1 * 1.20112240878645f;
    k.kd = 0.3275911f / 1.20112240878645f;
    k.hr = hr;
    k.a1 = -hr * 0.254829592f; k.a2 = -hr * -0.284496736f; k.a3 = -hr * 1.421413741f; k.a4 = -hr * -1.453152027f; k.a5 = -hr * 1.061405429f;
    return k;
}
__device__ __forceinline__ lg_v2f gelu2_k(lg_v2f x, const GeluK& k) {
    const lg_v2f w = (lg_v2f){fabsf(x.x) * k.k1, fabsf(x.y) * k.k1};
    const lg_v2f d = w * k.kd + 1.0f;
    const lg_v2f t = (lg_v2f){__builtin_amdgcn_rcpf(d.x), __builtin_amdgcn_rcpf(d.y)};
    const lg_v2f ph = ((((k.a5 * t + k.a4) * t + k.a3) * t + k.a2) * t + k.a1) * t;
    const lg_v2f w2 = w * w;
    const lg_v2f ex = (lg_v2f){__builtin_amdgcn_exp2f(-w2.x), __builtin_amdgcn_exp2f(-w2.y)};
    const lg_v2f sv = ph * ex + k.hr;
    return (lg_v2f){__builtin_fmaf(fabsf(x.x), sv.x, x.x * k.hr), __builtin_fmaf(fabsf(x.y), sv.y, x.y * k.hr)};
}
__device__ __forceinline__ lg_v2f gelu2_fast_sig(lg_v2f x, lg_v2f& x2) {
    x2 = x * x;
    const lg_v2f v = x * (x2 * -0.1029432395800235f + -2.302208198144325f);
    const lg_v2f d = (lg_v2f){__builtin_amdgcn_exp2f(v.x), __builtin_amdgcn_exp2f(v.y)} + 1.0f;
    return (lg_v2f){__builtin_amdgcn_rcpf(d.x), __builtin_amdgcn_rcpf(d.y)};
}
template <bool FAST>
__device__ __forceinline__ lg_v2f gelu2_t(lg_v2f x) {
    if constexpr (FAST) {
        lg_v2f x2;
        return x * gelu2_fast_sig(x, x2);
    } else {
        return gelu2_f(x);
    }
}
template <bool FAST>
__device__ __forceinline__ void gelu2_both_t(lg_v2f x, lg_v2f& a, lg_v2f& g) {
    if constexpr (FAST) {
        lg_v2f x2;
        const lg_v2f sg = gelu2_fast_sig(x, x2);
        a = x * sg;
        g = a * (1.0f - sg) * (x2 * 0.21406444881780073f + 1.5957691216057308f) + sg;
    } else {
        gelu2_both_f(x, a, g);
    }
}
__device__ __forceinline__ float gelu_grad_f(float x) {
    const float z = x * 0.70710678118654752440f;
    const float e = 0.5f * erfc_abs_f(fabsf(z));
    const float cdf = z >= 0.f ? 1.0f - e : e;
    const float pdf = 0.39894228040143267794f * __expf(-0.5f * x * x);
    return cdf + x * pdf;
}
__device__ __forceinline__ int clampi(int v, int lo, int hi) { return v < lo ? lo : (v > hi ? hi : v); }

__device__ __forceinline__ void cubic_w(float t, float w[4]) {
    const float A = -0.75f;
    float x;
    x = t + 1.0f; w[0] = ((A * x - 5.0f * A) * x + 8.0f * A) * x - 4.0f * A;
    x = t;        w[1] = ((A + 2.0f) * x - (A + 3.0f)) * x * x + 1.0f;
    x = 1.0f - t; w[2] = ((A + 2.0f) * x - (A + 3.0f)) * x * x + 1.0f;
    x = 2.0f - t; w[3] = ((A * x - 5.0f * A) * x + 8.0f * A) * x - 4.0f * A;
}
template <int MODE>
__device__ __forceinline__ void resample_plan(int o, int& i0, float w[4]) {
    if (MODE == 0) { i0 = 2 * o; cubic_w(0.5f, w); }
    else if (MODE == 1) {
        int m = o >> 1;
        if (o & 1) { i0 = m; cubic_w(0.25f, w); } else { i0 = m - 1; cubic_w(0.75f, w); }
    } else {
        int m = o >> 2, r = o & 3;
        if (r == 0) { i0 = m - 1; cubic_w(0.625f, w); }
        else if (r == 1) { i0 = m - 1; cubic_w(0.875f, w); }
        else if (r == 2) { i0 = m; cubic_w(0.125f, w); }
        else { i0 = m; cubic_w(0.375f, w); }
    }
}
template <int MODE>
__device__ __forceinline__ float resample_at(const float* __restrict__ p, int hi, int wi, int oy, int ox) {
    int iy0, ix0;
    float wy[4], wx[4];
    resample_plan<MODE>(oy, iy0, wy);
    resample_plan<MODE>(ox, ix0, wx);
    float acc = 0.f;
#pragma unroll
    for (int a = 0; a < 4; ++a) {
        int yy = clampi(iy0 - 1 + a, 0, hi - 1);
        float r = 0.f;
#pragma unroll
        for (int b = 0; b < 4; ++b) r += wx[b] * p[yy * wi + clampi(ix0 - 1 + b, 0, wi - 1)];
        acc += wy[a] * r;
    }
    return acc;
}

template <int E>
__device__ __forceinline__ void ln_stats(const float (&x)[E], float& mu, float& rstd) {
    float s = 0.f;
#pragma unroll
    for (int i = 0; i < E; ++i) s += x[i];
    mu = s * (1.0f / E);
    float v = 0.f;
#pragma unroll
    for (int i = 0; i < E; ++i) { float d = x[i] - mu; v += d * d; }
    rstd = __builtin_amdgcn_rsqf(v * (1.0f / E) + LG_EPS);
}

template <int N>
__device__ __forceinline__ float lane_group_sum(float v) {
    static_assert(N == 4 || N == 8 || N == 16, "group of 4, 8 or 16 lanes");
    v += __builtin_bit_cast(float, __builtin_amdgcn_mov_dpp(__builtin_bit_cast(int, v), 0xB1, 0xF, 0xF, true));
    v += __builtin_bit_cast(float, __builtin_amdgcn_mov_dpp(__builtin_bit_cast(int, v), 0x4E, 0xF, 0xF, true));
    if (N >= 8) v += __shfl_xor(v, 4);
    if (N >= 16) v += __shfl_xor(v, 8);
    return v;
}
#define LG_DROP_T16 6554u
__device__ __forceinline__ uint32_t dropout_hash(uint64_t seed, uint64_t pair) {
    uint32_t x = (uint32_t)pair + (uint32_t)seed;
    x ^= x >> 16; x *= 0x7feb352du;
    x ^= (uint32_t)(seed >> 32) ^ (uint32_t)(pair >> 32);
    x ^= x >> 15; x *= 0x846ca68bu;
    x ^= x >> 16;
    return x;
}
__device__ __forceinline__ float dropout_scale(uint64_t seed, uint64_t idx) {
    const uint32_t x = dropout_hash(seed, idx >> 1);
    return ((idx & 1) ? (x >> 16) : (x & 0xffffu)) < LG_DROP_T16 ? 0.0f : (1.0f / 0.9f);
}
__device__ __forceinline__ void dropout_scale2(uint64_t seed, uint64_t idx_even, float& s0, float& s1) {
    const uint32_t x = dropout_hash(seed, idx_even >> 1);
    s0 = (x & 0xffffu) < LG_DROP_T16 ? 0.0f : (1.0f / 0.9f);
    s1 = (x >> 16) < LG_DROP_T16 ? 0.0f : (1.0f / 0.9f);
}
__device__ __forceinline__ void lds_stage(float* dst, const float* __restrict__ src, int n) {
    for (int i = threadIdx.x; i < n; i += blockDim.x) dst[i] = src[i];
}
template <int NT, int N>
__device__ __forceinline__ void lds_stage_ld(float (&v)[(N + NT - 1) / NT], const float* __restrict__ src) {
#pragma unroll
    for (int k = 0; k < (N + NT - 1) / NT; ++k) { const int i = k * NT + (int)threadIdx.x; v[k] = src[i < N ? i : N - 1]; }
}
template <int NT, int N>
__device__ __forceinline__ void lds_stage_st(float* dst, const float (&v)[(N + NT - 1) / NT]) {
#pragma unroll
    for (int k = 0; k < (N + NT - 1) / NT; ++k) { const int i = k * NT + (int)threadIdx.x; if (i < N) dst[i] = v[k]; }
}
#endif
```

### lgteun_amd/csrc/k_ffn.hip

```cpp
#include "kernels.h"

#include "mfma.h"
#include "hstore.h"

template <int E, int MT, bool BF>
__global__ __launch_bounds__(256) void k_ffn1(Ffn1Args a) {
    constexpr int N1 = 4 * E, MW = 16 * MT, LDA = E + 4, LDH = N1 + 4;
    constexpr int LPP = 64 / MW;
    constexpr int CPL = E / LPP;
    extern __shared__ float smem[];
    const int wave = threadIdx.x >> 6, lane = threadIdx.x & 63, r = lane & 15, g = lane >> 4;
    float* bufA = smem + wave * (MW * LDA);
    float* bufH = smem + 4 * MW * LDA + wave * (MW * LDH);
    const long p0 = ((long)blockIdx.x * 4 + wave) * MW;
    {
        const int m = lane % MW, part = lane / MW;
        long p = p0 + m;
        if (p >= a.P) p = a.P - 1;
        float xv[CPL];
        const float4* src = reinterpret_cast<const float4*>(a.x + p * E + part * CPL);
#pragma unroll
        for (int k = 0; k < CPL / 4; ++k) {
            float4 v = src[k];
            xv[4 * k] = v.x; xv[4 * k + 1] = v.y; xv[4 * k + 2] = v.z; xv[4 * k + 3] = v.w;
// ... 783 lines not shown
    static DeviceOnce attr_once;
    if (attr_once.need()) {
        hipError_t e = hipFuncSetAttribute((const void*)k_ffn_strip<false>, hipFuncAttributeMaxDynamicSharedMemorySize, 152 * 1024);
        if (e == hipSuccess) e = hipFuncSetAttribute((const void*)k_ffn_strip<true>, hipFuncAttributeMaxDynamicSharedMemorySize, 152 * 1024);
        if (e != hipSuccess) { lg_set_error("ffn_strip: hipFuncSetAttribute: %s", hipGetErrorString(e)); return (int)e; }
        attr_once.done();
    }
    const int tiles_x = (a2.w + 15) / 16;
    int SH = (a2.h + 7) / 8 * 8;
    while (SH > 16 && (long)a2.B * tiles_x * ((a2.h + SH - 1) / SH) < 512) SH = (SH / 2 + 7) / 8 * 8;
    const int strips_y = (a2.h + SH - 1) / SH;
    const int nstrips = a2.B * tiles_x * strips_y;
    const int grid = nstrips < 512 ? nstrips : 512;
    if (a1.a1s != nullptr) k_ffn_strip<true><<<grid, 256, lds, s>>>(a1, a2, tiles_x, strips_y, nstrips, SH);
    else k_ffn_strip<false><<<grid, 256, lds, s>>>(a1, a2, tiles_x, strips_y, nstrips, SH);
    LG_CHECK_LAUNCH();
    return 0;
}

template <int E>
static int launch_ffn_fused_t(const Ffn1Args& a1, const Ffn2Args& a2, hipStream_t s) {
    ProfScope prof__(LG_K_FFN2, s);
    constexpr int N1 = 4 * E;
    size_t lds = (size_t)(192 * (E == 16 ? E : E + 4) + 180 * (N1 + 4) + 4 * 16 * (N1 + 4)) * sizeof(float);
    static DeviceOnce attr_once;
    if (attr_once.need()) {
        hipError_t e = hipFuncSetAttribute((const void*)k_ffn_fused<E, false, false>, hipFuncAttributeMaxDynamicSharedMemorySize, 152 * 1024);
        if (e == hipSuccess) e = hipFuncSetAttribute((const void*)k_ffn_fused<E, true, false>, hipFuncAttributeMaxDynamicSharedMemorySize, 152 * 1024);
        if (e == hipSuccess) e = hipFuncSetAttribute((const void*)k_ffn_fused<E, true, true>, hipFuncAttributeMaxDynamicSharedMemorySize, 152 * 1024);
        if (e != hipSuccess) { lg_set_error("ffn_fused: hipFuncSetAttribute: %s", hipGetErrorString(e)); return (int)e; }
        attr_once.done();
    }
    int tiles_x = (a2.w + 15) / 16, tiles_y = (a2.h + 7) / 8;
    const int ntiles = a2.B * tiles_x * tiles_y;
    const int cap = (E == 32) ? 256 : 512;
    const int grid = ntiles < cap ? ntiles : cap;
    const bool save = a1.a1s != nullptr;
    if (save && a1.hbf) k_ffn_fused<E, true, true><<<grid, 256, lds, s>>>(a1, a2, tiles_x, tiles_y, ntiles);
    else if (save) k_ffn_fused<E, true, false><<<grid, 256, lds, s>>>(a1, a2, tiles_x, tiles_y, ntiles);
    else k_ffn_fused<E, false, false><<<grid, 256, lds, s>>>(a1, a2, tiles_x, tiles_y, ntiles);
    LG_CHECK_LAUNCH();
    return 0;
}


template <int E, bool SAVE, bool BF>
__global__ __launch_bounds__(256) void k_ffn_fused_bf(Ffn1Args a1, Ffn2Args a2, int tiles_x, int tiles_y, int ntiles) {
    constexpr int N1 = 4 * E, TY = 8, TX = 16, HX = TX + 2, HY = TY + 2, NH = HX * HY , MH = 192, M = TY * TX;
    constexpr int LDA = E + 8, LDS16 = N1 + 8 , LDH = N1 + 4, LDO = E + 1, CQ = N1 / 4, NT3 = E / 16;
    constexpr int KB2 = N1 / 32;
    extern __shared__ __attribute__((aligned(16))) float smem[];
    float* bufH2 = smem;
    float* bufO = bufH2 + NH * LDH;
    __bf16* bufA = reinterpret_cast<__bf16*>(bufO + M * LDO + 3);
    bufA = reinterpret_cast<__bf16*>((reinterpret_cast<uintptr_t>(bufA) + 15) & ~(uintptr_t)15);
    __bf16* scr = bufA + MH * LDA;
    const int wave = threadIdx.x >> 6, lane = threadIdx.x & 63, r = lane & 15, g = lane >> 4;
    __bf16* my = scr + wave * 16 * LDS16;
    const int h = a2.h, w = a2.w;
    __shared__ __attribute__((aligned(16))) float sPar[5 * E + 10 * N1 + 2 * N1];
    float* sLn2g = sPar;            float* sLn2b = sPar + E;
    float* sN1g = sPar + 2 * E;     float* sN1b = sPar + 3 * E;
    float* sB3 = sPar + 4 * E;      float* sDww = sPar + 5 * E;
    float* sDwb = sDww + 9 * N1;    float* sB1 = sDwb + N1;         float* sB2 = sB1 + N1;
    for (int i = threadIdx.x; i < E; i += 256) {
        sLn2g[i] = a1.ln2g[i]; sLn2b[i] = a1.ln2b[i]; sB3[i] = a2.b3[i];
        sN1g[i] = a2.g ? a2.n1g[i] : 0.f; sN1b[i] = a2.g ? a2.n1b[i] : 0.f;
    }
    for (int i = threadIdx.x; i < 9 * N1; i += 256) sDww[i] = a2.dww[i];
    for (int i = threadIdx.x; i < N1; i += 256) { sDwb[i] = a2.dwb[i]; sB1[i] = a1.b1[i]; sB2[i] = a1.b2[i]; }
    s16x4 w1k16[4];
    bf16x8 w2f[4][KB2], w3f[NT3][KB2];
    if constexpr (E == 16) {
        load_bfrag_bf16_k16<4>(w1k16, a1.w1);
        load_bfrag_bf16<4, KB2>(w2f, a1.w2, N1);
        load_bfrag_bf16<NT3, KB2>(w3f, a2.w3, N1);
    }
#pragma unroll 1
    for (int tile = blockIdx.x; tile < ntiles; tile += gridDim.x) {
    int t = tile;
    const int tx_i = t % tiles_x;
    t /= tiles_x;
    const int ty_i = t % tiles_y;
    const long b = t / tiles_y;
    const int y0 = ty_i * TY, x0 = tx_i * TX;
    __syncthreads();
    if (threadIdx.x < MH) {
        const int m = threadIdx.x;
        const int hy = m / HX, hx = m - hy * HX;
        const int y = y0 + hy - 1, x = x0 + hx - 1;
        float xv[E];
        const bool in = (m < NH) && y >= 0 && y < h && x >= 0 && x < w;
        if (in) {
            const float4* src = reinterpret_cast<const float4*>(a1.x + ((b * h + y) * (long)w + x) * E);
#pragma unroll
            for (int k = 0; k < E / 4; ++k) {
                float4 v = src[k];
                xv[4 * k] = v.x; xv[4 * k + 1] = v.y; xv[4 * k + 2] = v.z; xv[4 * k + 3] = v.w;
            }
            float mu, rstd;
            ln_stats<E>(xv, mu, rstd);
#pragma unroll
            for (int c = 0; c < E; ++c) xv[c] = (xv[c] - mu) * rstd * sLn2g[c] + sLn2b[c];
        } else {
#pragma unroll
            for (int c = 0; c < E; ++c) xv[c] = 0.f;
        }
#pragma unroll
        for (int k = 0; k < E / 4; ++k) {
            const bf16x4 hv = (bf16x4){(__bf16)xv[4 * k], (__bf16)xv[4 * k + 1], (__bf16)xv[4 * k + 2], (__bf16)xv[4 * k + 3]};
            *reinterpret_cast<bf16x4*>(bufA + m * LDA + 4 * k) = hv;
        }
    }
    __syncthreads();
    for (int ch = 0; ch < 3; ++ch) {
        const int row0 = (wave * 3 + ch) * 16;
        long prow[4];
        bool inner[4], inimg[4];
#pragma unroll
        for (int v = 0; v < 4; ++v) {
            const int m = row0 + 4 * g + v;
            const int hy = m / HX, hx = m - hy * HX;
            const int y = y0 + hy - 1, x = x0 + hx - 1;
            inimg[v] = (m < NH) && y >= 0 && y < h && x >= 0 && x < w;
            inner[v] = inimg[v] && hy >= 1 && hy <= TY && hx >= 1 && hx <= TX;
            prow[v] = (b * h + y) * (long)w + x;
        }
        for (int nc = 0; nc < N1; nc += 64) {
            f32x4 acc[1][4];
#pragma unroll
            for (int nt = 0; nt < 4; ++nt) acc[0][nt] = (f32x4){0.f, 0.f, 0.f, 0.f};
            if constexpr (E == 16) {
                wave_gemm_bf_k16<1, 4>(acc, bufA + row0 * LDA, LDA, w1k16);
            } else {
                constexpr int KB1 = E / 32;
                bf16x8 wf[4][KB1];
                load_bfrag_bf16<4, KB1>(wf, a1.w1 + (size_t)nc * E, E);
                wave_gemm_bf<1, 4, KB1>(acc, bufA + row0 * LDA, LDA, wf);
            }
#pragma unroll
            for (int nt = 0; nt < 4; ++nt) {
                const int col = nc + nt * 16 + r;
                const float bias = sB1[col];
#pragma unroll
                for (int v = 0; v < 4; v += 2) {
                    const lg_v2f hh = (lg_v2f){acc[0][nt][v] + bias, acc[0][nt][v + 1] + bias};
                    lg_v2f av;
                    if (SAVE) {
                        lg_v2f gv;
                        gelu2_both_f(hh, av, gv);
                        if (inner[v]) { HS<BF>::st1(a1.a1s, prow[v] * N1 + col, av.x); HS<BF>::st1(a1.g1s, prow[v] * N1 + col, gv.x); }
                        if (inner[v + 1]) { HS<BF>::st1(a1.a1s, prow[v + 1] * N1 + col, av.y); HS<BF>::st1(a1.g1s, prow[v + 1] * N1 + col, gv.y); }
                    } else {
                        av = gelu2_f(hh);
                    }
                    my[(4 * g + v) * LDS16 + col] = (__bf16)av.x;
                    my[(4 * g + v + 1) * LDS16 + col] = (__bf16)av.y;
                }
            }
        }
        __builtin_amdgcn_fence(__ATOMIC_RELEASE, "wavefront");
        __builtin_amdgcn_wave_barrier();
        for (int nc = 0; nc < N1; nc += 64) {
            f32x4 acc[1][4];
#pragma unroll
            for (int nt = 0; nt < 4; ++nt) acc[0][nt] = (f32x4){0.f, 0.f, 0.f, 0.f};
            if constexpr (E == 16) {
                wave_gemm_bf<1, 4, KB2>(acc, my, LDS16, w2f);
            } else {
                bf16x8 wf[4][KB2];
                load_bfrag_bf16<4, KB2>(wf, a1.w2 + (size_t)nc * N1, N1);
                wave_gemm_bf<1, 4, KB2>(acc, my, LDS16, wf);
            }
#pragma unroll
            for (int nt = 0; nt < 4; ++nt) {
                const int col = nc + nt * 16 + r;
                const float bias = sB2[col];
#pragma unroll
                for (int v = 0; v < 4; ++v) {
                    const int m = row0 + 4 * g + v;
                    const float hh = inimg[v] ? acc[0][nt][v] + bias : 0.f;
                    if (SAVE && inner[v]) HS<BF>::st1(a1.h2, prow[v] * N1 + col, hh);
                    if (m < NH) bufH2[m * LDH + col] = hh;
                }
            }
        }
        __builtin_amdgcn_wave_barrier();
    }
    __syncthreads();
    {
        const int q = lane % CQ;
        float wq[4][9], bq[4];
#pragma unroll
        for (int u = 0; u < 4; ++u) {
#pragma unroll
            for (int k = 0; k < 9; ++k) wq[u][k] = sDww[(4 * q + u) * 9 + k];
            bq[u] = sDwb[4 * q + u];
        }
        for (int ch = 0; ch < 2; ++ch) {
            const int m0 = (wave * 2 + ch) * 16;
            for (int mm = lane / CQ; mm < 16; mm += 64 / CQ) {
                const int m = m0 + mm;
                const int ty = m / TX, tx = m - ty * TX;
                float4 acc = make_float4(bq[0], bq[1], bq[2], bq[3]);
#pragma unroll
                for (int dy = 0; dy < 3; ++dy)
#pragma unroll
                    for (int dx = 0; dx < 3; ++dx) {
                        const float4 v = *reinterpret_cast<const float4*>(bufH2 + ((ty + dy) * HX + tx + dx) * LDH + 4 * q);
                        acc.x += wq[0][dy * 3 + dx] * v.x; acc.y += wq[1][dy * 3 + dx] * v.y;
                        acc.z += wq[2][dy * 3 + dx] * v.z; acc.w += wq[3][dy * 3 + dx] * v.w;
                    }
                const int y = y0 + ty, x = x0 + tx;
                float4 av;
                if (SAVE) {
                    lg_v2f a01, a23, g01, g23;
                    gelu2_both_f((lg_v2f){acc.x, acc.y}, a01, g01);
                    gelu2_both_f((lg_v2f){acc.z, acc.w}, a23, g23);
                    av = make_float4(a01.x, a01.y, a23.x, a23.y);
                    if (y < h && x < w) {
                        const long o = ((b * h + y) * (long)w + x) * N1 + 4 * q;
                        HS<BF>::st4(a2.a3s, o, av);
                        HS<BF>::st4(a2.g3s, o, make_float4(g01.x, g01.y, g23.x, g23.y));
                    }
                } else {
                    const lg_v2f a01 = gelu2_f((lg_v2f){acc.x, acc.y}), a23 = gelu2_f((lg_v2f){acc.z, acc.w});
                    av = make_float4(a01.x, a01.y, a23.x, a23.y);
                }
                *reinterpret_cast<bf16x4*>(my + mm * LDS16 + 4 * q) = (bf16x4){(__bf16)av.x, (__bf16)av.y, (__bf16)av.z, (__bf16)av.w};
            }
            __builtin_amdgcn_fence(__ATOMIC_RELEASE, "wavefront");
            __builtin_amdgcn_wave_barrier();
            f32x4 acc3[1][NT3];
#pragma unroll
            for (int nt = 0; nt < NT3; ++nt) acc3[0][nt] = (f32x4){0.f, 0.f, 0.f, 0.f};
            if constexpr (E == 16) {
                wave_gemm_bf<1, NT3, KB2>(acc3, my, LDS16, w3f);
            } else {
                bf16x8 wf[NT3][KB2];
                load_bfrag_bf16<NT3, KB2>(wf, a2.w3, N1);
                wave_gemm_bf<1, NT3, KB2>(acc3, my, LDS16, wf);
            }
#pragma unroll
            for (int nt = 0; nt < NT3; ++nt) {
                const int col = nt * 16 + r;
                const float bias = sB3[col];
#pragma unroll
                for (int v = 0; v < 4; ++v) bufO[(m0 + 4 * g + v) * LDO + col] = acc3[0][nt][v] + bias;
            }
            __builtin_amdgcn_wave_barrier();
        }
    }
    __syncthreads();
    if (threadIdx.x < M) {
        const int m = threadIdx.x;
        const int y = y0 + m / TX, x = x0 + m % TX;
        if (y < h && x < w) {
            const long p = (b * h + y) * (long)w + x;
            float o[E];
            const float4* xs = reinterpret_cast<const float4*>(a2.x + p * E);
            float4* yo = reinterpret_cast<float4*>(a2.y + p * E);
#pragma unroll
            for (int k = 0; k < E / 4; ++k) {
                float4 xr = xs[k];
                o[4 * k] = xr.x + bufO[m * LDO + 4 * k];
                o[4 * k + 1] = xr.y + bufO[m * LDO + 4 * k + 1];
                o[4 * k + 2] = xr.z + bufO[m * LDO + 4 * k + 2];
                o[4 * k + 3] = xr.w + bufO[m * LDO + 4 * k + 3];
                yo[k] = make_float4(o[4 * k], o[4 * k + 1], o[4 * k + 2], o[4 * k + 3]);
            }
            if (a2.g) {
                float mu, rstd;
                ln_stats<E>(o, mu, rstd);
                const long hw = (long)h * w, s = (long)y * w + x;
#pragma unroll
                for (int n = E / 2; n < E; ++n) a2.g[(b * (E / 2) + (n - E / 2)) * hw + s] = (o[n] - mu) * rstd * sN1g[n] + sN1b[n];
            }
        }
    }
    }
}

template <int E>
static int launch_ffn_fused_bf_t(const Ffn1Args& a1, const Ffn2Args& a2, hipStream_t s) {
    ProfScope prof__(LG_K_FFN2, s);
    constexpr int N1 = 4 * E;
    const size_t lds = (size_t)(180 * (N1 + 4) + 128 * (E + 1) + 8) * sizeof(float) + (size_t)(192 * (E + 8) + 4 * 16 * (N1 + 8)) * 2;
    static DeviceOnce attr_once;
    if (attr_once.need()) {
        hipError_t e = hipFuncSetAttribute((const void*)k_ffn_fused_bf<E, false, true>, hipFuncAttributeMaxDynamicSharedMemorySize, 152 * 1024);
        if (e == hipSuccess) e = hipFuncSetAttribute((const void*)k_ffn_fused_bf<E, true, true>, hipFuncAttributeMaxDynamicSharedMemorySize, 152 * 1024);
        if (e != hipSuccess) { lg_set_error("ffn_fused_bf: hipFuncSetAttribute: %s", hipGetErrorString(e)); return (int)e; }
        attr_once.done();
    }
    int tiles_x = (a2.w + 15) / 16, tiles_y = (a2.h + 7) / 8;
    const int ntiles = a2.B * tiles_x * tiles_y;
    const int grid = ntiles < 512 ? ntiles : 512;
    if (a1.a1s != nullptr) k_ffn_fused_bf<E, true, true><<<grid, 256, lds, s>>>(a1, a2, tiles_x, tiles_y, ntiles);
    else k_ffn_fused_bf<E, false, true><<<grid, 256, lds, s>>>(a1, a2, tiles_x, tiles_y, ntiles);
    LG_CHECK_LAUNCH();
    return 0;
}

int launch_ffn_fused(int e, const Ffn1Args& a1, const Ffn2Args& a2, hipStream_t s) {
    if (a1.hbf) {
#ifdef LG_BUILD_AB
        if (e == 16 && a1.tile16 != 0) return launch_ffn_fused_bf_t<16>(a1, a2, s);
        if (e == 32 && (a1.tile16 != 0 || !a1.wsplit)) return launch_ffn_fused_bf_t<32>(a1, a2, s);
#endif
        if (e == 16 && (a1.tile16 == 0 || a1.tile16 == 4)) {
            const bool save = a1.h2 != nullptr, h2h3 = save && !a1.a1s && !a1.g1s && a2.a3s && !a2.g3s;
            if (a1.tile16 == 0 && (!save || h2h3)) return launch_ffn_xr(a1, a2, s);
            return launch_ffn_xs(a1, a2, s);
        }
        if (e == 32 && a1.tile16 == 0 && a1.wsplit) return launch_ffn_x32(a1, a2, s);
        if (e == 64) return LG_FFN_NOT_FUSED;
        lg_set_error("ffn: precision = 1 with an FFN variant needs a `make AB=1` build");
        return -2;
    }
#ifdef LG_BUILD_AB
    if (e == 16 && a1.tile16 == 3) return launch_ffn_xp(a1, a2, s);
#else
    if (e == 16 && a1.tile16 == 3) { lg_set_error("LG_FFN_IMPL=xp: k_ffn_xp is an A/B kernel, build the library with `make AB=1`"); return -2; }
#endif
#ifdef LG_BUILD_AB
    if (e == 16 && a1.tile16 == 2) return launch_ffn_fused_t<16>(a1, a2, s);
#endif
    if (e == 16 && a1.tile16 == 1) return launch_ffn_strip(a1, a2, s);
    if (e == 16) {
        const bool save = a1.h2 != nullptr, h2h3 = save && !a1.a1s && !a1.g1s && !a2.g3s;
        if (a1.tile16 == 0 && a1.scales && (!save || h2h3)) return launch_ffn_xr(a1, a2, s);
        return launch_ffn_xs(a1, a2, s);
    }
    if (e == 32) return (a1.tile16 == 0 && a1.wsplit) ? launch_ffn_x32(a1, a2, s) : launch_ffn_fused_t<32>(a1, a2, s);
    if (e == 64 && a1.tile16 == 0 && a1.wsplit && a1.h2) return launch_ffn_x64(a1, a2, s);
    return LG_FFN_NOT_FUSED;
}
```

### lgteun_amd/csrc/k_ffn_xr.hip

```cpp
#include "kernels.h"

#include "hstore.h"
#include "split_bf16.h"

#ifndef LG_XR_GRID
#define LG_XR_GRID 512
#endif
#ifdef LG_STAMPS
__device__ unsigned long long g_xr_stamps[512 * 4 * 10 * 8];
#define XSTAMP_AT(si_, i) do { unsigned long long t__; asm volatile("s_memtime %0\n\ts_waitcnt lgkmcnt(0)" : "=s"(t__)); \
                       g_xr_stamps[(((blockIdx.x & 511) * 4 + wave) * 10 + (si_)) * 8 + (i)] = t__; } while (0)
#define XSTAMP(i) do { unsigned long long t__; asm volatile("s_memtime %0\n\ts_waitcnt lgkmcnt(0)" : "=s"(t__)); \
                       g_xr_stamps[(((blockIdx.x & 511) * 4 + wave) * 10 + (stamp_si < 9 ? stamp_si : 9)) * 8 + (i)] = t__; } while (0)
extern "C" __attribute__((visibility("default"))) int lg_debug_xr_stamps(unsigned long long* host) {
    return (int)hipMemcpyFromSymbol(host, HIP_SYMBOL(g_xr_stamps), sizeof(g_xr_stamps));
}
#else
#define XSTAMP_AT(si_, i) do { } while (0)
#define XSTAMP(i) do { } while (0)
#endif

#ifndef LG_XR_TURN
#define LG_XR_TURN 0
#endif
#ifndef LG_XR_UNEVEN
#define LG_XR_UNEVEN 16
#endif
#define XR_TAKE_TURNS() do { if (LG_XR_TURN) { \
        const unsigned long long tt__ = __builtin_amdgcn_s_memtime(); \
        if ((((unsigned)(tt__ >> LG_XR_TURN)) ^ slot_par) & 1u) __builtin_amdgcn_s_setprio(3); else __builtin_amdgcn_s_setprio(0); } } while (0)
__device__ unsigned g_xr_turn[8192];

namespace xr {

constexpr int E = 16, N1 = 64, TX = 16, HX = 18, TY = 8, RING = 10, LDR = 68;
constexpr int NF1 = 8, NF2 = 16, NF3 = 4, NFRAG = NF1 + NF2 + NF3;
constexpr size_t OFF_W = 0;
constexpr size_t OFF_TAPS = OFF_W + (size_t)NFRAG * 64 * 16;
constexpr size_t OFF_PAR = OFF_TAPS + (size_t)N1 * 9 * 4;
constexpr int P_B1 = 0, P_B2 = 64, P_DWB = 128, P_B3 = 192, P_N1G = 208, P_N1B = 224, P_FLOATS = 240;
constexpr size_t OFF_RING = OFF_PAR + (size_t)P_FLOATS * 4;
constexpr size_t LDS_BYTES = OFF_RING + (size_t)RING * HX * LDR * 4;
static_assert(LDS_BYTES <= 80 * 1024, "two workgroups per CU");
static_assert(OFF_RING % 16 == 0 && OFF_TAPS % 16 == 0 && OFF_PAR % 16 == 0, "16-byte aligned LDS regions");

#ifndef LG_XR_NT
#define LG_XR_NT 0
#endif
#ifndef LG_XR_FENCES
#define LG_XR_FENCES 1
#endif
#define XR_ST2(base, idx, v) do { if (LG_XR_NT & 1) HS<BF>::st4_nt(base, idx, v); else HS<BF>::st4(base, idx, v); } while (0)
#define XR_ST3(base, idx, v) do { if (LG_XR_NT & 2) HS<BF>::st4_nt(base, idx, v); else HS<BF>::st4(base, idx, v); } while (0)
#define XR_FENCE() do { if (LG_XR_FENCES) __builtin_amdgcn_sched_barrier(0); } while (0)
template <int N>
struct IC { static constexpr int value = N; };

__device__ __forceinline__ float xg_sum(float v) {
    u32x2_t r = __builtin_amdgcn_permlane32_swap(__float_as_uint(v), __float_as_uint(v), false, false);
    v = __uint_as_float(r.x) + __uint_as_float(r.y);
    r = __builtin_amdgcn_permlane16_swap(__float_as_uint(v), __float_as_uint(v), false, false);
    return __uint_as_float(r.x) + __uint_as_float(r.y);
}
__device__ __forceinline__ f32x4_t mfma_h(u32x4_t a, u32x4_t b, f32x4_t c) {
    return __builtin_amdgcn_mfma_f32_16x16x32_f16(__builtin_bit_cast(f16x8_t, a), __builtin_bit_cast(f16x8_t, b), c, 0, 0, 0);
}
__device__ __forceinline__ void pair2(float a, float b, uint32_t& hi, uint32_t& lo) {
    hi = sb_cvt_f16x2(a, b);
    lo = sb_cvt_f16x2(sb_res_lo(hi, a), sb_res_hi(hi, b));
}

template <int NP>
__device__ __forceinline__ void pairN(float a, float b, uint32_t& hi, uint32_t& lo) {
    if (NP == 2) pair2(a, b, hi, lo);
    else {
        typedef __bf16 bf16x2_t __attribute__((ext_vector_type(2)));
        const bf16x2_t v = {(__bf16)a, (__bf16)b};
        hi = __builtin_bit_cast(uint32_t, v);
        lo = 0u;
    }
}
__device__ __forceinline__ f32x4_t mfma_b(u32x4_t a, u32x4_t b, f32x4_t c) {
    return __builtin_amdgcn_mfma_f32_16x16x32_bf16(__builtin_bit_cast(bf16x8_t, a), __builtin_bit_cast(bf16x8_t, b), c, 0, 0, 0);
}
template <int NP>
__device__ __forceinline__ f32x4_t mfma3(u32x4_t wh, u32x4_t wl, u32x4_t bh, u32x4_t bl, f32x4_t acc) {
    if (NP == 2) {
        acc = mfma_h(wl, bh, acc);
        acc = mfma_h(wh, bl, acc);
        return mfma_h(wh, bh, acc);
    }
    return mfma_b(wh, bh, acc);
}
template <int NP>
__device__ __forceinline__ f32x4_t mfma_g1(u32x4_t wa, u32x4_t wb, u32x4_t xb1, u32x4_t xb2, f32x4_t acc) {
    if (NP == 2) {
        acc = mfma_h(wa, xb1, acc);
        return mfma_h(wb, xb2, acc);
    }
    return mfma_b(wb, xb2, acc);
}
struct GKold { float c1, hr; };
__device__ __forceinline__ lg_v2f gelu2_k(lg_v2f x, const GKold& k) { return gelu2_scaled(x, k.c1, k.hr); }

template <int NP, class GK>
__device__ __forceinline__ lg_v2f geluN(lg_v2f x, const GK& k) {
    if constexpr (NP == 2) return gelu2_k(x, k);
    else return gelu2_t<true>(x);
}

}

template <int SAVE, int NP>
__global__ __launch_bounds__(256) __attribute__((amdgpu_waves_per_eu(2))) void k_ffn_xr(Ffn1Args a1, Ffn2Args a2, int tiles_x, int strips_y, int nstrips,
                                                                                       int SH, int dS) {
    using namespace xr;
    extern __shared__ __attribute__((aligned(16))) unsigned char smem_raw[];
    float* ring = reinterpret_cast<float*>(smem_raw + OFF_RING);
    u32x4_t* sW = reinterpret_cast<u32x4_t*>(smem_raw + OFF_W);
    float* sTaps = reinterpret_cast<float*>(smem_raw + OFF_TAPS);
    float* sPar = reinterpret_cast<float*>(smem_raw + OFF_PAR);
    const int wave = threadIdx.x >> 6, lane = threadIdx.x & 63, g = lane >> 4, c_ = lane & 15, c = c_;
    const int uwave = __builtin_amdgcn_readfirstlane(wave);
    unsigned slot_par = 0;
    if (LG_XR_TURN) {
        const unsigned hw = __builtin_amdgcn_s_getreg((12 - 1) << 11 | 4 << 6 | 4);
        const unsigned xcc = __builtin_amdgcn_s_getreg((3 - 1) << 11 | 0 << 6 | 20);
        const unsigned key = (xcc << 10) | (((hw >> 9) & 7u) << 7) | (((hw >> 8) & 1u) << 6) | (((hw >> 4) & 15u) << 2) | (hw & 3u);
        unsigned old_ = 0;
        if (lane == 0) old_ = atomicXor(&g_xr_turn[key & 8191u], 1u);
        slot_par = (unsigned)__builtin_amdgcn_readfirstlane((int)old_) & 1u;
    }
    const int h = a2.h, w = a2.w;
    constexpr bool BF = NP == 1;
    float sx = 1.f, sa1 = 1.f, sa3 = 1.f, sw1 = 1.f, sw2 = 1.f, sw3 = 1.f;
    if (NP == 2) { sx = a1.scales[0]; sa1 = a1.scales[1]; sa3 = a1.scales[2]; sw1 = a1.scales[3]; sw2 = a1.scales[4]; sw3 = a1.scales[5]; }
    const float S1 = sx * sw1, S2 = sa1 * sw2, S3 = sa3 * sw3;
    const float inv2 = 1.0f / S2, inv3 = 1.0f / S3;
#ifdef LG_XR_OLDGELU
    const xr::GKold gk1 = {0.70710678118654752440f / S1, 0.5f * sa1 / S1}, gk3 = {0.70710678118654752440f, 0.5f * sa3};
#else
    const GeluK gk1 = gelu_k(0.70710678118654752440f / S1, 0.5f * sa1 / S1), gk3 = gelu_k(0.70710678118654752440f, 0.5f * sa3);
#endif

    auto strip_geo = [&](int strip, int& tx_i, long& b, int& Y0, int& Yend) {
        if (dS) {
            const int half = nstrips >> 1, shortone = strip >= half ? 1 : 0;
            int p_ = strip - (shortone ? half : 0);
            tx_i = p_ % tiles_x;
            p_ /= tiles_x;
            const int hy2 = strips_y >> 1, ky = p_ % hy2;
            b = p_ / hy2;
            Y0 = ky * 2 * SH + (shortone ? SH + dS : 0);
            Yend = min(Y0 + (shortone ? SH - dS : SH + dS), h);
        } else {
            int t_ = strip;
            tx_i = t_ % tiles_x;
            t_ /= tiles_x;
            const int sy = t_ % strips_y;
            b = t_ / strips_y;
            Y0 = sy * SH;
            Yend = min(Y0 + SH, h);
        }
    };
    XSTAMP_AT(9, 0);
    float4 xp_first;
    {
        int tx_i, Y0f, Yendf;
        long b;
        strip_geo(blockIdx.x, tx_i, b, Y0f, Yendf);
        const int m = 16 * (wave < 3 ? wave : 0) + c, hy = m / HX, hx = m - hy * HX;
        const int y = clampi(Y0f - 1 + hy, 0, h - 1), x = clampi(tx_i * TX + hx - 1, 0, w - 1);
        xp_first = *reinterpret_cast<const float4*>(a1.x + ((b * h + y) * (long)w + x) * E + 4 * g);
    }
    float4 lng, lnb;
    {
        const int t = threadIdx.x, ln = t >> 2, i = t & 3, lg = ln >> 4, lr = ln & 15;
        constexpr int NTP = (N1 * 9 + 255) / 256;
        float tp[NTP];
#pragma unroll
        for (int j = 0; j < NTP; ++j) {
            const int k = min(t + 256 * j, N1 * 9 - 1);
            tp[j] = a2.dww[(4 * (k / 36) + (k & 3)) * 9 + (k % 36) / 4];
        }
        const int tn = t < N1 ? t : N1 - 1, te = t < E ? t : E - 1;
        const float pb1 = a1.b1[tn], pb2 = a1.b2[tn], pdwb = a2.dwb[tn], pb3 = a2.b3[te];
        const float* const ng = a2.g ? a2.n1g : a2.b3;
        const float* const nb_ = a2.g ? a2.n1b : a2.b3;
        const float png = ng[te], pnb = nb_[te];
        lng = *reinterpret_cast<const float4*>(a1.ln2g + 4 * g);
        lnb = *reinterpret_cast<const float4*>(a1.ln2b + 4 * g);
        float2 v1[4], v2[8], v3[2];
#pragma unroll
        for (int mt = 0; mt < 4; ++mt) v1[mt] = *reinterpret_cast<const float2*>(a1.w1 + (size_t)(16 * mt + lr) * E + 4 * lg + 2 * (i & 1));
#pragma unroll
        for (int f = 0; f < 8; ++f) {
            const int mt2 = f >> 1, s = f & 1;
            v2[f] = *reinterpret_cast<const float2*>(a1.w2 + (size_t)(16 * mt2 + lr) * N1 + 16 * (2 * s + (i >> 1)) + 4 * lg + 2 * (i & 1));
        }
#pragma unroll
        for (int s = 0; s < 2; ++s) v3[s] = *reinterpret_cast<const float2*>(a2.w3 + (size_t)lr * N1 + 16 * (2 * s + (i >> 1)) + 4 * lg + 2 * (i & 1));
        __builtin_amdgcn_sched_barrier(0);
        uint32_t* d32 = reinterpret_cast<uint32_t*>(sW);
#pragma unroll
        for (int mt = 0; mt < 4; ++mt) {
            uint32_t hi, lo;
            pairN<NP>(v1[mt].x * sw1, v1[mt].y * sw1, hi, lo);
            d32[(2 * mt) * 256 + t] = i < 2 ? lo : hi;
            d32[(2 * mt + 1) * 256 + t] = i < 2 ? hi : 0u;
        }
#pragma unroll
        for (int f = 0; f < 8; ++f) {
            uint32_t hi, lo;
            pairN<NP>(v2[f].x * sw2, v2[f].y * sw2, hi, lo);
            d32[(NF1 + 2 * f) * 256 + t] = hi;
            d32[(NF1 + 2 * f + 1) * 256 + t] = lo;
        }
#pragma unroll
        for (int s = 0; s < 2; ++s) {
            uint32_t hi, lo;
            pairN<NP>(v3[s].x * sw3, v3[s].y * sw3, hi, lo);
            d32[(NF1 + NF2 + 2 * s) * 256 + t] = hi;
            d32[(NF1 + NF2 + 2 * s + 1) * 256 + t] = lo;
        }
#pragma unroll
        for (int j = 0; j < NTP; ++j) asm volatile("" : "+v"(tp[j]));
#pragma unroll
        for (int j = 0; j < NTP; ++j)
            if (t + 256 * j < N1 * 9) sTaps[t + 256 * j] = tp[j];
        if (t < N1) { sPar[P_B1 + t] = pb1 * S1; sPar[P_B2 + t] = pb2 * S2; sPar[P_DWB + t] = pdwb; }
        if (t < E) {
            sPar[P_B3 + t] = pb3 * S3;
            sPar[P_N1G + t] = a2.g ? png : 0.f;
            sPar[P_N1B + t] = a2.g ? pnb : 0.f;
        }
    }
    lng = make_float4(lng.x * sx, lng.y * sx, lng.z * sx, lng.w * sx);
    lnb = make_float4(lnb.x * sx, lnb.y * sx, lnb.z * sx, lnb.w * sx);
    __syncthreads();
    XSTAMP_AT(9, 1);

#pragma unroll 1
    for (int strip = blockIdx.x; strip < nstrips; strip += gridDim.x) {
        int tx_i, Y0, Yend;
        long b;
        strip_geo(strip, tx_i, b, Y0, Yend);
#ifdef LG_XR_SAMEX
        b = 0;
#endif
        const int x0 = tx_i * TX;

        auto xload = [&](int ya, int blk) -> float4 {
            const int m = 16 * blk + c;
            const int hy = m / HX, hx = m - hy * HX;
            const int y = clampi(ya + hy, 0, h - 1), x = clampi(x0 + hx - 1, 0, w - 1);
            return *reinterpret_cast<const float4*>(a1.x + ((b * h + y) * (long)w + x) * E + 4 * g);
        };

        struct Geo { float mk; int rp; bool inner; uint32_t prow; };
        auto halo = [&](auto nbc, auto partc, int ya, int npx, int blk0, const float4* xin, f32x4_t* part, Geo* geo_out) {
            constexpr int NB = decltype(nbc)::value, PART = decltype(partc)::value;
            constexpr int MT0 = PART == 2 ? 2 : 0, NMT = PART == 0 ? 4 : 2;
            constexpr int S0 = PART == 2 ? 1 : 0, NS = PART == 0 ? 2 : 1;
            int c = c_;
            asm volatile("" : "+v"(c));
            const int ring0 = ((ya - Y0 + 1) % RING) * HX;
            u32x4_t wa[NMT], wb[NMT];
            float4 b1v[NMT];
#pragma unroll
            for (int i = 0; i < NMT; ++i) {
                wa[i] = sW[(2 * (MT0 + i)) * 64 + lane];
                wb[i] = sW[(2 * (MT0 + i) + 1) * 64 + lane];
                b1v[i] = *reinterpret_cast<const float4*>(sPar + P_B1 + 16 * (MT0 + i) + 4 * g);
            }
            u32x4_t xb1[NB], xb2[NB];
            Geo geo[NB];
#pragma unroll
            for (int nb = 0; nb < NB; ++nb) {
                const int m = 16 * (blk0 + nb) + c;
                const int hy = m / HX, hx = m - hy * HX;
                const int y = ya + hy, x = x0 + hx - 1;
                const bool in = m < npx && y >= 0 && y < h && x >= 0 && x < w;
                geo[nb].mk = in ? inv2 : 0.0f;
                int r_ = ring0 + m;
                r_ = r_ >= RING * HX ? r_ - RING * HX : r_;
                geo[nb].rp = m < npx ? r_ : -1;
                geo[nb].inner = SAVE && m < npx && hx >= 1 && hx <= TX && x < w && y >= Y0 && y < Yend;
                geo[nb].prow = (uint32_t)(((b * h + y) * (long)w + x) * N1 + 4 * g);
                const float4 xv = xin[nb];
                const float s = xg_sum((xv.x + xv.y) + (xv.z + xv.w));
                const float mu = s * (1.0f / E);
                const float d0 = xv.x - mu, d1 = xv.y - mu, d2 = xv.z - mu, d3 = xv.w - mu;
                const float vs = xg_sum((d0 * d0 + d1 * d1) + (d2 * d2 + d3 * d3));
                const float rstd = __builtin_amdgcn_rsqf(vs * (1.0f / E) + LG_EPS);
                uint32_t h01, l01, h23, l23;
                pairN<NP>(d0 * rstd * lng.x + lnb.x, d1 * rstd * lng.y + lnb.y, h01, l01);
                pairN<NP>(d2 * rstd * lng.z + lnb.z, d3 * rstd * lng.w + lnb.w, h23, l23);
                xb1[nb] = (u32x4_t){h01, h23, l01, l23};
                xb2[nb] = (u32x4_t){h01, h23, 0u, 0u};
            }
            XR_FENCE();
            f32x4_t a1c[NB][NMT];
#pragma unroll
            for (int i = 0; i < NMT; ++i)
#pragma unroll
                for (int nb = 0; nb < NB; ++nb) {
                    f32x4_t acc = {b1v[i].x, b1v[i].y, b1v[i].z, b1v[i].w};
                    a1c[nb][i] = mfma_g1<NP>(wa[i], wb[i], xb1[nb], xb2[nb], acc);
                }
            u32x4_t wh[NS], wl[NS];
            float4 b2v = make_float4(0.f, 0.f, 0.f, 0.f);
#pragma unroll
            for (int s = 0; s < NS; ++s) { wh[s] = sW[(NF1 + 2 * (S0 + s)) * 64 + lane]; wl[s] = sW[(NF1 + 2 * (S0 + s) + 1) * 64 + lane]; }
            if (PART != 2) b2v = *reinterpret_cast<const float4*>(sPar + P_B2 + 4 * g);
            XR_FENCE();
            uint32_t ghi[NB][NMT][2], glo[NB][NMT][2];
#pragma unroll
            for (int i = 0; i < NMT; ++i) {
#pragma unroll
                for (int nb = 0; nb < NB; ++nb) {
                    const lg_v2f a01 = geluN<NP>((lg_v2f){a1c[nb][i][0], a1c[nb][i][1]}, gk1);
                    const lg_v2f a23 = geluN<NP>((lg_v2f){a1c[nb][i][2], a1c[nb][i][3]}, gk1);
                    pairN<NP>(a01.x, a01.y, ghi[nb][i][0], glo[nb][i][0]);
                    pairN<NP>(a23.x, a23.y, ghi[nb][i][1], glo[nb][i][1]);
                    asm volatile("" : "+v"(ghi[nb][i][0]), "+v"(glo[nb][i][0]), "+v"(ghi[nb][i][1]), "+v"(glo[nb][i][1]));
                }
                XR_FENCE();
            }
            auto leave = [&](int mt2, const f32x4_t (&k0)[NB], const f32x4_t (&k1)[NB]) {
#pragma unroll
                for (int nb = 0; nb < NB; ++nb) {
                    if (PART == 2) { part[mt2] = k1[nb]; continue; }
                    const float mk = geo[nb].mk;
                    float4 hh = make_float4(k0[nb][0] * mk, k0[nb][1] * mk, k0[nb][2] * mk, k0[nb][3] * mk);
                    if (PART == 0) hh = make_float4(__builtin_fmaf(k1[nb][0], mk, hh.x), __builtin_fmaf(k1[nb][1], mk, hh.y), __builtin_fmaf(k1[nb][2], mk, hh.z), __builtin_fmaf(k1[nb][3], mk, hh.w));
                    if (SAVE && PART == 0 && geo[nb].inner) XR_ST2(a1.h2, geo[nb].prow + 16 * mt2, hh);
                    if (geo[nb].rp >= 0) *reinterpret_cast<float4*>(ring + geo[nb].rp * LDR + 16 * mt2 + 4 * g) = hh;
                }
            };
            f32x4_t accp0[NB], accp1[NB];
#pragma unroll
            for (int mt2 = 0; mt2 < 4; ++mt2) {
                f32x4_t acc0[NB], acc1[NB];
#pragma unroll
                for (int nb = 0; nb < NB; ++nb) { acc0[nb] = (f32x4_t){b2v.x, b2v.y, b2v.z, b2v.w}; acc1[nb] = (f32x4_t){0.f, 0.f, 0.f, 0.f}; }
#pragma unroll
                for (int s = 0; s < NS; ++s)
#pragma unroll
                    for (int nb = 0; nb < NB; ++nb) {
                        const u32x4_t bh = {ghi[nb][2 * s][0], ghi[nb][2 * s][1], ghi[nb][2 * s + 1][0], ghi[nb][2 * s + 1][1]};
                        const u32x4_t bl = {glo[nb][2 * s][0], glo[nb][2 * s][1], glo[nb][2 * s + 1][0], glo[nb][2 * s + 1][1]};
                        f32x4_t& acc = (S0 + s) == 0 ? acc0[nb] : acc1[nb];
                        acc = mfma3<NP>(wh[s], wl[s], bh, bl, acc);
                    }
                if (mt2 < 3) {
#pragma unroll
                    for (int s = 0; s < NS; ++s) {
                        wh[s] = sW[(NF1 + 2 * (2 * (mt2 + 1) + S0 + s)) * 64 + lane];
                        wl[s] = sW[(NF1 + 2 * (2 * (mt2 + 1) + S0 + s) + 1) * 64 + lane];
                    }
                    if (PART != 2) b2v = *reinterpret_cast<const float4*>(sPar + P_B2 + 16 * (mt2 + 1) + 4 * g);
                }
                if (mt2 > 0) leave(mt2 - 1, accp0, accp1);
#pragma unroll
                for (int nb = 0; nb < NB; ++nb) { accp0[nb] = acc0[nb]; accp1[nb] = acc1[nb]; }
                XR_FENCE();
            }
            leave(3, accp0, accp1);
            if (PART == 2) *geo_out = geo[0];
        };
        auto halo_pair = [&](int ya, int blk0, const float4* xin) {
            constexpr int npx = TY * HX;
            int c = c_;
            asm volatile("" : "+v"(c));
            const int ring0 = ((ya - Y0 + 1) % RING) * HX;
            u32x4_t wa[4], wb[4];
            float4 b1v[4];
#pragma unroll
            for (int i = 0; i < 4; ++i) {
                wa[i] = sW[(2 * i) * 64 + lane];
                wb[i] = sW[(2 * i + 1) * 64 + lane];
                b1v[i] = *reinterpret_cast<const float4*>(sPar + P_B1 + 16 * i + 4 * g);
            }
            u32x4_t xb1[2], xb2[2];
            Geo geo[2];
#pragma unroll
            for (int nb = 0; nb < 2; ++nb) {
                const int m = 16 * (blk0 + nb) + c;
                const int hy = m / HX, hx = m - hy * HX;
                const int y = ya + hy, x = x0 + hx - 1;
                const bool in = y >= 0 && y < h && x >= 0 && x < w;
                geo[nb].mk = in ? inv2 : 0.0f;
                int r_ = ring0 + m;
                r_ = r_ >= RING * HX ? r_ - RING * HX : r_;
                geo[nb].rp = r_;
                geo[nb].inner = SAVE && hx >= 1 && hx <= TX && x < w && y >= Y0 && y < Yend;
                geo[nb].prow = (uint32_t)(((b * h + y) * (long)w + x) * N1 + 4 * g);
                const float4 xv = xin[nb];
                const float s = xg_sum((xv.x + xv.y) + (xv.z + xv.w));
                const float mu = s * (1.0f / E);
                const float d0 = xv.x - mu, d1 = xv.y - mu, d2 = xv.z - mu, d3 = xv.w - mu;
                const float vs = xg_sum((d0 * d0 + d1 * d1) + (d2 * d2 + d3 * d3));
                const float rstd = __builtin_amdgcn_rsqf(vs * (1.0f / E) + LG_EPS);
                uint32_t h01, l01, h23, l23;
                pairN<NP>(d0 * rstd * lng.x + lnb.x, d1 * rstd * lng.y + lnb.y, h01, l01);
                pairN<NP>(d2 * rstd * lng.z + lnb.z, d3 * rstd * lng.w + lnb.w, h23, l23);
                xb1[nb] = (u32x4_t){h01, h23, l01, l23};
                xb2[nb] = (u32x4_t){h01, h23, 0u, 0u};
            }
            XR_FENCE();
            f32x4_t a1c[2][4];
#pragma unroll
            for (int nb = 0; nb < 2; ++nb)
#pragma unroll
                for (int i = 0; i < 4; ++i) {
                    f32x4_t acc = {b1v[i].x, b1v[i].y, b1v[i].z, b1v[i].w};
                    a1c[nb][i] = mfma_g1<NP>(wa[i], wb[i], xb1[nb], xb2[nb], acc);
                }
            u32x4_t wh[2], wl[2];
#pragma unroll
            for (int s = 0; s < 2; ++s) { wh[s] = sW[(NF1 + 2 * s) * 64 + lane]; wl[s] = sW[(NF1 + 2 * s + 1) * 64 + lane]; }
            float4 b2v = *reinterpret_cast<const float4*>(sPar + P_B2 + 4 * g);
            XR_FENCE();
            uint32_t ghi[2][4][2], glo[2][4][2];
            auto gelu_tile = [&](int nb, int i) {
                const lg_v2f a01 = geluN<NP>((lg_v2f){a1c[nb][i][0], a1c[nb][i][1]}, gk1);
                const lg_v2f a23 = geluN<NP>((lg_v2f){a1c[nb][i][2], a1c[nb][i][3]}, gk1);
                pairN<NP>(a01.x, a01.y, ghi[nb][i][0], glo[nb][i][0]);
                pairN<NP>(a23.x, a23.y, ghi[nb][i][1], glo[nb][i][1]);
                asm volatile("" : "+v"(ghi[nb][i][0]), "+v"(glo[nb][i][0]), "+v"(ghi[nb][i][1]), "+v"(glo[nb][i][1]));
            };
            struct Acc2 { f32x4_t k0, k1; };
            auto gemm2_tile = [&](int nb) -> Acc2 {
                Acc2 r;
                r.k0 = (f32x4_t){b2v.x, b2v.y, b2v.z, b2v.w};
                r.k1 = (f32x4_t){0.f, 0.f, 0.f, 0.f};
#pragma unroll
                for (int s = 0; s < 2; ++s) {
                    const u32x4_t bh = {ghi[nb][2 * s][0], ghi[nb][2 * s][1], ghi[nb][2 * s + 1][0], ghi[nb][2 * s + 1][1]};
                    const u32x4_t bl = {glo[nb][2 * s][0], glo[nb][2 * s][1], glo[nb][2 * s + 1][0], glo[nb][2 * s + 1][1]};
                    f32x4_t& acc = s == 0 ? r.k0 : r.k1;
                    acc = mfma3<NP>(wh[s], wl[s], bh, bl, acc);
                }
                return r;
            };
            auto next_w2 = [&](int mt2) {
#pragma unroll
                for (int s = 0; s < 2; ++s) {
                    wh[s] = sW[(NF1 + 2 * (2 * mt2 + s)) * 64 + lane];
                    wl[s] = sW[(NF1 + 2 * (2 * mt2 + s) + 1) * 64 + lane];
                }
                b2v = *reinterpret_cast<const float4*>(sPar + P_B2 + 16 * mt2 + 4 * g);
            };
            auto leave = [&](int nb, int mt2, const Acc2& acc) {
                const float mk = geo[nb].mk;
                const float4 hh = make_float4(__builtin_fmaf(acc.k1[0], mk, acc.k0[0] * mk), __builtin_fmaf(acc.k1[1], mk, acc.k0[1] * mk),
                                              __builtin_fmaf(acc.k1[2], mk, acc.k0[2] * mk), __builtin_fmaf(acc.k1[3], mk, acc.k0[3] * mk));
                if (SAVE && geo[nb].inner) XR_ST2(a1.h2, geo[nb].prow + 16 * mt2, hh);
                *reinterpret_cast<float4*>(ring + geo[nb].rp * LDR + 16 * mt2 + 4 * g) = hh;
            };
#pragma unroll
            for (int i = 0; i < 4; ++i) { gelu_tile(0, i); XR_FENCE(); }
            Acc2 accp;
#pragma unroll
            for (int j = 0; j < 4; ++j) {
                const Acc2 acc = gemm2_tile(0);
                next_w2(j < 3 ? j + 1 : 0);
                gelu_tile(1, j);
                if (j > 0) leave(0, j - 1, accp);
                accp = acc;
                XR_FENCE();
            }
#pragma unroll
            for (int j = 0; j < 4; ++j) {
                const Acc2 acc = gemm2_tile(1);
                if (j < 3) next_w2(j + 1);
                leave(j > 0 ? 1 : 0, j > 0 ? j - 1 : 3, accp);
                accp = acc;
                XR_FENCE();
            }
            leave(1, 3, accp);
        };
        auto ninth_add = [&](const f32x4_t (&part)[4], const Geo& ge) {
            if (ge.rp < 0) return;
#pragma unroll
            for (int mt2 = 0; mt2 < 4; ++mt2) {
                float4* rp4 = reinterpret_cast<float4*>(ring + ge.rp * LDR + 16 * mt2 + 4 * g);
                float4 r = *rp4;
                r = make_float4(__builtin_fmaf(part[mt2][0], ge.mk, r.x), __builtin_fmaf(part[mt2][1], ge.mk, r.y), __builtin_fmaf(part[mt2][2], ge.mk, r.z), __builtin_fmaf(part[mt2][3], ge.mk, r.w));
                *rp4 = r;
                if (SAVE && ge.inner) XR_ST2(a1.h2, ge.prow + 16 * mt2, r);
            }
        };

        float4 xh[3];
        {
            const float4 xp = strip == (int)blockIdx.x ? xp_first : xload(Y0 - 1, wave < 3 ? wave : 0);
            xh[0] = xload(Y0 + 1, 2 * wave); xh[1] = xload(Y0 + 1, 2 * wave + 1); xh[2] = xload(Y0 + 1, 8);
            __syncthreads();
            if (uwave < 3) halo(IC<1>{}, IC<0>{}, Y0 - 1, 2 * HX, wave, &xp, nullptr, nullptr);
            XSTAMP_AT(9, 2);
        }
#pragma unroll 1
        for (int y0 = Y0; y0 < Yend; y0 += TY) {
            const int si = (y0 - Y0) >> 3;
            const int role = (uwave + si) & 3, ty0 = 2 * role;
#ifdef LG_STAMPS
            const int stamp_si = si;
#endif
            XSTAMP(0);
            float4 xres[2];
#pragma unroll
            for (int r2 = 0; r2 < 2; ++r2) {
                const int y = min(y0 + ty0 + r2, h - 1), x = min(x0 + c, w - 1);
                xres[r2] = *reinterpret_cast<const float4*>(a2.x + ((b * h + y) * (long)w + x) * E + 4 * g);
            }
            halo_pair(y0 + 1, 2 * wave, xh);
            XSTAMP(1);
            f32x4_t part9[4];
            Geo geo9;
            if (role == 1) halo(IC<1>{}, IC<1>{}, y0 + 1, TY * HX, 8, xh + 2, nullptr, nullptr);
            if (role == 3) halo(IC<1>{}, IC<2>{}, y0 + 1, TY * HX, 8, xh + 2, part9, &geo9);
            XSTAMP(2);
            xh[0] = xload(y0 + TY + 1, 2 * wave); xh[1] = xload(y0 + TY + 1, 2 * wave + 1); xh[2] = xload(y0 + TY + 1, 8);
            __syncthreads();
            XR_TAKE_TURNS();
            XSTAMP(3);
            if (role == 3) ninth_add(part9, geo9);
            {
                const int sbase = (y0 - Y0) % RING;
                const float* rrow[4];
#pragma unroll
                for (int r4 = 0; r4 < 4; ++r4) {
                    int sl = sbase + ty0 + r4;
                    sl = sl >= RING ? sl - RING : sl;
                    sl = sl >= RING ? sl - RING : sl;
                    rrow[r4] = ring + (sl * HX + c) * LDR + 4 * g;
                }
                float h3[2][4][4];
                float4 tq[9], tqn[9], rv[3], rvn[3], bq, bqn;
#pragma unroll
                for (int k = 0; k < 9; ++k) { tq[k] = *reinterpret_cast<const float4*>(sTaps + 36 * g + 4 * k); tqn[k] = tq[k]; }
                bq = *reinterpret_cast<const float4*>(sPar + P_DWB + 4 * g); bqn = bq;
#pragma unroll
                for (int dx = 0; dx < 3; ++dx) rv[dx] = *reinterpret_cast<const float4*>(rrow[0] + dx * LDR);
                lg_v2f acc01[2], acc23[2];
#pragma unroll
                for (int it = 0; it < 16; ++it) {
                    const int m = it >> 2, r4 = it & 3;
                    if (r4 == 0) {
                        acc01[0] = acc01[1] = (lg_v2f){bq.x, bq.y};
                        acc23[0] = acc23[1] = (lg_v2f){bq.z, bq.w};
                    }
                    if (it < 15) {
                        const int mn = (it + 1) >> 2, rn = (it + 1) & 3;
#pragma unroll
                        for (int dx = 0; dx < 3; ++dx) rvn[dx] = *reinterpret_cast<const float4*>(rrow[rn] + dx * LDR + 16 * mn);
                    }
                    if (r4 == 1 && m < 3) {
#pragma unroll
                        for (int k = 0; k < 9; ++k) tqn[k] = *reinterpret_cast<const float4*>(sTaps + 36 * (4 * (m + 1) + g) + 4 * k);
                        bqn = *reinterpret_cast<const float4*>(sPar + P_DWB + 16 * (m + 1) + 4 * g);
                    }
#pragma unroll
                    for (int dx = 0; dx < 3; ++dx) {
                        const lg_v2f v01 = (lg_v2f){rv[dx].x, rv[dx].y}, v23 = (lg_v2f){rv[dx].z, rv[dx].w};
                        if (r4 <= 2) {
                            const float4 t4 = tq[r4 * 3 + dx];
                            acc01[0] = (lg_v2f){t4.x, t4.y} * v01 + acc01[0]; acc23[0] = (lg_v2f){t4.z, t4.w} * v23 + acc23[0];
                        }
                        if (r4 >= 1) {
                            const float4 t4 = tq[(r4 - 1) * 3 + dx];
                            acc01[1] = (lg_v2f){t4.x, t4.y} * v01 + acc01[1]; acc23[1] = (lg_v2f){t4.z, t4.w} * v23 + acc23[1];
                        }
                    }
                    asm volatile("" : "+v"(acc01[0]), "+v"(acc23[0]), "+v"(acc01[1]), "+v"(acc23[1]));
                    if (r4 == 3) {
#pragma unroll
                        for (int r2 = 0; r2 < 2; ++r2) { h3[r2][m][0] = acc01[r2].x; h3[r2][m][1] = acc01[r2].y; h3[r2][m][2] = acc23[r2].x; h3[r2][m][3] = acc23[r2].y; }
#pragma unroll
                        for (int k = 0; k < 9; ++k) tq[k] = tqn[k];
                        bq = bqn;
                    }
#pragma unroll
                    for (int dx = 0; dx < 3; ++dx) rv[dx] = rvn[dx];
                    XR_FENCE();
                }
                u32x4_t w3h[2], w3l[2];
#pragma unroll
                for (int s = 0; s < 2; ++s) { w3h[s] = sW[(NF1 + NF2 + 2 * s) * 64 + lane]; w3l[s] = sW[(NF1 + NF2 + 2 * s + 1) * 64 + lane]; }
                const float4 b3v = *reinterpret_cast<const float4*>(sPar + P_B3 + 4 * g);
                const float4 ng = *reinterpret_cast<const float4*>(sPar + P_N1G + 4 * g), nbv = *reinterpret_cast<const float4*>(sPar + P_N1B + 4 * g);
#pragma unroll
                for (int r2 = 0; r2 < 2; ++r2) {
                    const int y = y0 + ty0 + r2, x = x0 + c;
                    const bool ok = y < Yend && x < w;
                    uint32_t phi[4][2], plo[4][2];
#pragma unroll
                    for (int m = 0; m < 4; ++m) {
#ifndef LG_XR_NOH3
                        if (SAVE && ok && a2.a3s) XR_ST3(a2.a3s, ((b * h + y) * (long)w + x) * N1 + 16 * m + 4 * g, make_float4(h3[r2][m][0], h3[r2][m][1], h3[r2][m][2], h3[r2][m][3]));
#endif
                        const lg_v2f a01 = geluN<NP>((lg_v2f){h3[r2][m][0], h3[r2][m][1]}, gk3);
                        const lg_v2f a23 = geluN<NP>((lg_v2f){h3[r2][m][2], h3[r2][m][3]}, gk3);
                        pairN<NP>(a01.x, a01.y, phi[m][0], plo[m][0]);
                        pairN<NP>(a23.x, a23.y, phi[m][1], plo[m][1]);
                    }
                    f32x4_t o = {b3v.x, b3v.y, b3v.z, b3v.w};
#pragma unroll
                    for (int s = 0; s < 2; ++s) {
                        const u32x4_t bh = {phi[2 * s][0], phi[2 * s][1], phi[2 * s + 1][0], phi[2 * s + 1][1]};
                        const u32x4_t bl = {plo[2 * s][0], plo[2 * s][1], plo[2 * s + 1][0], plo[2 * s + 1][1]};
                        o = mfma3<NP>(w3h[s], w3l[s], bh, bl, o);
                    }
                    const float o0 = o[0] * inv3 + xres[r2].x, o1 = o[1] * inv3 + xres[r2].y, o2 = o[2] * inv3 + xres[r2].z, o3 = o[3] * inv3 + xres[r2].w;
#ifdef LG_XR_NOSTORE
                    if (ok && o0 == 12345.678f) *reinterpret_cast<float4*>(a2.y + ((b * h + y) * (long)w + x) * E + 4 * g) = make_float4(o0, o1, o2, o3);
#else
                    if (ok) *reinterpret_cast<float4*>(a2.y + ((b * h + y) * (long)w + x) * E + 4 * g) = make_float4(o0, o1, o2, o3);
#endif
                    if (a2.g) {
                        const float s = xg_sum((o0 + o1) + (o2 + o3));
                        const float mu = s * (1.0f / E);
                        const float d0 = o0 - mu, d1 = o1 - mu, d2 = o2 - mu, d3 = o3 - mu;
                        const float vs = xg_sum((d0 * d0 + d1 * d1) + (d2 * d2 + d3 * d3));
                        const float rstd = __builtin_amdgcn_rsqf(vs * (1.0f / E) + LG_EPS);
#ifdef LG_XR_NOSTORE
                        if (ok && g >= 2 && d0 == 12345.678f) {
#else
                        if (ok && g >= 2) {
#endif
                            const long hw = (long)h * w, sp = (long)y * w + x;
                            float* dst = a2.g + (b * (E / 2) + (4 * g - E / 2)) * hw + sp;
                            dst[0] = d0 * rstd * ng.x + nbv.x;
                            dst[hw] = d1 * rstd * ng.y + nbv.y;
                            dst[2 * hw] = d2 * rstd * ng.z + nbv.z;
                            dst[3 * hw] = d3 * rstd * ng.w + nbv.w;
                        }
                    }
                    XR_FENCE();
                }
            }
            XSTAMP(4);
            __syncthreads();
            XR_TAKE_TURNS();
            XSTAMP(5);
        }
    }
}

int launch_ffn_xr(const Ffn1Args& a1, const Ffn2Args& a2, hipStream_t s) {
    using namespace xr;
    ProfScope prof__(LG_K_FFN2, s);
    static DeviceOnce attr_once;
    if (attr_once.need()) {
        hipError_t e = hipFuncSetAttribute((const void*)k_ffn_xr<0, 2>, hipFuncAttributeMaxDynamicSharedMemorySize, (int)LDS_BYTES);
        if (e == hipSuccess) e = hipFuncSetAttribute((const void*)k_ffn_xr<3, 2>, hipFuncAttributeMaxDynamicSharedMemorySize, (int)LDS_BYTES);
        if (e == hipSuccess) e = hipFuncSetAttribute((const void*)k_ffn_xr<0, 1>, hipFuncAttributeMaxDynamicSharedMemorySize, (int)LDS_BYTES);
        if (e == hipSuccess) e = hipFuncSetAttribute((const void*)k_ffn_xr<3, 1>, hipFuncAttributeMaxDynamicSharedMemorySize, (int)LDS_BYTES);
        if (e != hipSuccess) { lg_set_error("ffn_xr: hipFuncSetAttribute: %s", hipGetErrorString(e)); return (int)e; }
        attr_once.done();
    }
    if (!a1.hbf && !a1.scales) { lg_set_error("ffn_xr: the f16-pair instance needs the operand scales"); return -2; }
    const bool save = a1.h2 != nullptr;
    if (save && (a1.a1s || a1.g1s || a2.g3s)) { lg_set_error("ffn_xr: saves h2 / h3 (or h2 alone: a3s null, the backward re-computes h3) only"); return -2; }
    if ((long)a2.B * a2.h * a2.w * N1 >= (1ll << 32)) { lg_set_error("ffn_xr: hidden tensor of %ld elements exceeds the 32-bit save index", (long)a2.B * a2.h * a2.w * N1); return -2; }
    const int tiles_x = (a2.w + 15) / 16;
    int SH = (a2.h + 7) / 8 * 8;
    while (SH > 16 && (long)a2.B * tiles_x * ((a2.h + SH - 1) / SH) < LG_XR_GRID) SH = (SH / 2 + 7) / 8 * 8;
    const int strips_y = (a2.h + SH - 1) / SH;
    const int nstrips = a2.B * tiles_x * strips_y;
    const int grid = nstrips < LG_XR_GRID ? nstrips : LG_XR_GRID;
    int dS = 0;
    if (LG_XR_UNEVEN && nstrips == LG_XR_GRID && LG_XR_GRID == 512 && (strips_y & 1) == 0 && SH >= 32 && a2.h % (2 * SH) == 0) dS = (SH * LG_XR_UNEVEN / 64 + 7) / 8 * 8;
    if (a1.hbf) {
        if (save) k_ffn_xr<3, 1><<<grid, 256, LDS_BYTES, s>>>(a1, a2, tiles_x, strips_y, nstrips, SH, dS);
        else k_ffn_xr<0, 1><<<grid, 256, LDS_BYTES, s>>>(a1, a2, tiles_x, strips_y, nstrips, SH, dS);
    } else if (save) k_ffn_xr<3, 2><<<grid, 256, LDS_BYTES, s>>>(a1, a2, tiles_x, strips_y, nstrips, SH, dS);
    else k_ffn_xr<0, 2><<<grid, 256, LDS_BYTES, s>>>(a1, a2, tiles_x, strips_y, nstrips, SH, dS);
    LG_CHECK_LAUNCH();
    return 0;
}
```

### lgteun_amd/csrc/k_pixel.hip

```cpp
#include "kernels.h"
#include "resample_tile.h"

template <int MODE>
__global__ __launch_bounds__(256) void k_resample(const float* __restrict__ x, float* __restrict__ y, int planes, int hi,
                                                  int wi, int ho, int wo) {
    long total = (long)planes * ho * wo;
    for (long i = blockIdx.x * 256L + threadIdx.x; i < total; i += (long)gridDim.x * 256L) {
        int ox = (int)(i % wo);
        long r = i / wo;
        int oy = (int)(r % ho);
        long p = r / ho;
        y[i] = resample_at<MODE>(x + p * hi * wi, hi, wi, oy, ox);
    }
}

int launch_resample(int mode, const float* x, float* y, int planes, int hi, int wi, hipStream_t s) {
    int ho, wo;
    if (mode == 0) { ho = hi / 2; wo = wi / 2; } else if (mode == 1) { ho = hi * 2; wo = wi * 2; } else { ho = hi * 4; wo = wi * 4; }
    long total = (long)planes * ho * wo;
    int grid = (int)((total + 255) / 256);
    if (grid > 4096) grid = 4096;
    if (mode == 0) k_resample<0><<<grid, 256, 0, s>>>(x, y, planes, hi, wi, ho, wo);
    else if (mode == 1) k_resample<1><<<grid, 256, 0, s>>>(x, y, planes, hi, wi, ho, wo);
    else k_resample<2><<<grid, 256, 0, s>>>(x, y, planes, hi, wi, ho, wo);
    LG_CHECK_LAUNCH();
    return 0;
}

template <int MODE, int EPI>
__global__ __launch_bounds__(256) void k_resample_dw(DwArgs a) {
    __shared__ float U[34][35];
    __shared__ float rs_scratch[MODE == 1 ? RsTile<1>::FLOATS : 1];
    const int plane = blockIdx.z;
    const int c = plane % a.C;
    const int b = plane / a.C;
    const int ty0 = blockIdx.y * 32, tx0 = blockIdx.x * 32;
    const float* __restrict__ in = a.in + (size_t)plane * a.hi * a.wi;
    float rzp[EPI == 2 ? 4 : 1], zc[EPI == 2 ? 4 : 1];
    if constexpr (EPI == 2) {
        const size_t hw = (size_t)a.ho * a.wo;
        const float* __restrict__ zb = a.z + (size_t)b * a.C * hw;
        constexpr int CMAX = 8;
        float zv[4][CMAX], pn[4], rwv[CMAX];
#pragma unroll
        for (int cc = 0; cc < CMAX; ++cc) rwv[cc] = cc < a.C ? a.rw[cc < a.C ? cc : 0] : 0.f;
#pragma unroll
        for (int k = 0; k < 4; ++k) {
            const int i = threadIdx.x + 256 * k;
            const int oy = ty0 + (i >> 5), ox = tx0 + (i & 31);
            const size_t pix = (oy < a.ho && ox < a.wo) ? (size_t)oy * a.wo + ox : 0;
#pragma unroll
            for (int cc = 0; cc < CMAX; ++cc) zv[k][cc] = zb[(size_t)(cc < a.C ? cc : a.C - 1) * hw + pix];
            pn[k] = a.pan[(size_t)b * hw + pix];
        }
        const float rb0 = a.rb[0];
#pragma unroll
        for (int k = 0; k < 4; ++k) {
            float r = rb0;
            zc[k] = 0.f;
#pragma unroll
            for (int cc = 0; cc < CMAX; ++cc) {
                if (cc < a.C) r += rwv[cc] * zv[k][cc];
                zc[k] = cc == c ? zv[k][cc] : zc[k];
            }
            rzp[k] = r - pn[k];
        }
    }
    if constexpr (MODE == 1) resample_tile34<1>(in, a.hi, a.wi, a.ho, a.wo, ty0, tx0, U, rs_scratch);
    else {
        for (int i = threadIdx.x; i < 34 * 34; i += 256) {
            int uy = i / 34, ux = i - uy * 34;
            int oy = ty0 + uy - 1, ox = tx0 + ux - 1;
            float v = 0.f;
            if (oy >= 0 && oy < a.ho && ox >= 0 && ox < a.wo) v = resample_at<MODE>(in, a.hi, a.wi, oy, ox);
            U[uy][ux] = v;
        }
    }
    __syncthreads();
    float w[9];
#pragma unroll
    for (int k = 0; k < 9; ++k) w[k] = a.w9[c * 9 + k];
    const float bias = a.bias[c];
    float rtw_c = 0.f, rtb_c = 0.f, eta = 0.f;
    if (EPI == 2) { rtw_c = a.rtw[c]; rtb_c = a.rtb[c]; eta = a.eta[0]; }
#pragma unroll
    for (int k = 0; k < 4; ++k) {
        const int i = threadIdx.x + 256 * k;
        int ly = i >> 5, lx = i & 31;
        int oy = ty0 + ly, ox = tx0 + lx;
        if (oy < a.ho && ox < a.wo) {
            float v = 0.f;
#pragma unroll
            for (int dy = 0; dy < 3; ++dy)
#pragma unroll
                for (int dx = 0; dx < 3; ++dx) v += w[dy * 3 + dx] * U[ly + dy][lx + dx];
            v += bias;
            size_t o = ((size_t)plane * a.ho + oy) * a.wo + ox;
            if (EPI == 1) v -= a.sub[o];
            if (EPI == 2) {
                const float pan_term = rtw_c * rzp[k] + rtb_c;
                v = zc[k] - eta * (v + pan_term);
            }
            a.out[o] = v;
        }
    }
}

int launch_resample_dw(int mode, int epi, const DwArgs& a, hipStream_t s) {
    ProfScope prof__(LG_K_DATASTEP, s);
    dim3 grid((a.wo + 31) / 32, (a.ho + 31) / 32, a.planes);
    if (epi == 2 && a.C > 8) { lg_set_error("resample_dw: the fused update holds at most 8 bands per pixel (C=%d)", a.C); return -2; }
#define LG_RDW(M, E) k_resample_dw<M, E><<<grid, 256, 0, s>>>(a)
    if (mode == 0 && epi == 0) LG_RDW(0, 0);
    else if (mode == 0 && epi == 1) LG_RDW(0, 1);
    else if (mode == 1 && epi == 0) LG_RDW(1, 0);
    else if (mode == 1 && epi == 2) LG_RDW(1, 2);
    else { lg_set_error("resample_dw: unsupported mode/epi %d/%d", mode, epi); return -1; }
#undef LG_RDW
    LG_CHECK_LAUNCH();
    return 0;
}

template <int E>
__device__ __forceinline__ void emit_g(const float (&x)[E], const float* __restrict__ n1g, const float* __restrict__ n1b,
                                       float* __restrict__ g, long b, long s, long HW) {
    float mu, rstd;
    ln_stats<E>(x, mu, rstd);
#pragma unroll
    for (int n = E / 2; n < E; ++n) g[(b * (E / 2) + (n - E / 2)) * HW + s] = (x[n] - mu) * rstd * n1g[n] + n1b[n];
}

template <int C, int E>
__global__ __launch_bounds__(256) void k_embed(EmbedArgs a) {
    long p = blockIdx.x * 256L + threadIdx.x;
    if (p >= a.total) return;
    long b = p / a.HW, s = p - b * a.HW;
    float t[C];
#pragma unroll
    for (int c = 0; c < C; ++c) t[c] = a.z[(b * C + c) * a.HW + s] * a.dww[c] + a.dwb[c];
    float e[E];
#pragma unroll
    for (int n = 0; n < E; ++n) {
        float v = 0.f;
#pragma unroll
        for (int c = 0; c < C; ++c) v += a.w[n * C + c] * t[c];
        e[n] = v + a.b[n];
    }
    float mu, rstd;
    ln_stats<E>(e, mu, rstd);
#pragma unroll
    for (int n = 0; n < E; ++n) e[n] = (e[n] - mu) * rstd * a.lng[n] + a.lnb[n];
#ifndef LG_EMBED_TR
#define LG_EMBED_TR 1
#endif
    if (LG_EMBED_TR && a.total % 64 == 0) {
        constexpr int Q4 = E / 4, LDT = E + 4;
            __shared__ __attribute__((aligned(16))) float tr[4][64 * LDT];
        const int lane = threadIdx.x & 63;
        float* mine = tr[threadIdx.x >> 6];
#pragma unroll
        for (int n = 0; n < Q4; ++n) *reinterpret_cast<float4*>(mine + lane * LDT + 4 * n) = make_float4(e[4 * n], e[4 * n + 1], e[4 * n + 2], e[4 * n + 3]);
        __builtin_amdgcn_fence(__ATOMIC_RELEASE, "wavefront");
        __builtin_amdgcn_wave_barrier();
        __builtin_amdgcn_fence(__ATOMIC_ACQUIRE, "wavefront");
        float4* xo = reinterpret_cast<float4*>(a.x + (p - lane) * E);
#pragma unroll
        for (int j = 0; j < Q4; ++j) {
            const int i = j * 64 + lane;
            xo[i] = *reinterpret_cast<const float4*>(mine + (i / Q4) * LDT + 4 * (i % Q4));
        }
    } else {
        float4* xo = reinterpret_cast<float4*>(a.x + p * E);
#pragma unroll
        for (int n = 0; n < E / 4; ++n) xo[n] = make_float4(e[4 * n], e[4 * n + 1], e[4 * n + 2], e[4 * n + 3]);
    }
    if (a.g) emit_g<E>(e, a.n1g, a.n1b, a.g, b, s, a.HW);
}

int launch_embed(int C, const EmbedArgs& a, hipStream_t s) {
    ProfScope prof__(LG_K_EMBED, s);
    int grid = (int)((a.total + 255) / 256);
    if (C == 4) k_embed<4, 16><<<grid, 256, 0, s>>>(a);
    else if (C == 8) k_embed<8, 32><<<grid, 256, 0, s>>>(a);
    else { lg_set_error("embed: C=%d unsupported", C); return -1; }
    LG_CHECK_LAUNCH();
    return 0;
}

template <int E>
__global__ __launch_bounds__(256) void k_down(DownArgs a) {
    constexpr int LPP = E / 4, PPW = 256 / LPP, NO = 2 * E / LPP, LDU = E + 4;
    static_assert(NO == 8, "eight outputs per lane");
    __shared__ __attribute__((aligned(16))) float sW[2 * E * E];
    __shared__ float sB[2 * E], sNg[2 * E], sNb[2 * E];
    __shared__ __attribute__((aligned(16))) float ux[PPW * LDU];
    {
        float vw[(2 * E * E + 255) / 256], vb[1], vg[1], vn[1];
        lds_stage_ld<256, 2 * E * E>(vw, a.w);
        lds_stage_ld<256, 2 * E>(vb, a.b);
        lds_stage_ld<256, 2 * E>(vg, a.g ? a.n1g : a.b);
        lds_stage_ld<256, 2 * E>(vn, a.g ? a.n1b : a.b);
#pragma unroll
        for (int k = 0; k < (2 * E * E + 255) / 256; ++k) {
            const int i = k * 256 + threadIdx.x;
            if (i < 2 * E * E) sW[(i % E) * (2 * E) + i / E] = vw[k];
        }
        lds_stage_st<256, 2 * E>(sB, vb);
        lds_stage_st<256, 2 * E>(sNg, vg);
        lds_stage_st<256, 2 * E>(sNb, vn);
    }
    __syncthreads();
    const int q = threadIdx.x % LPP, slot = threadIdx.x / LPP;
    const int ho = a.H / 2, wo = a.W / 2;
    const long total = (long)a.B * ho * wo;
    const long p = (long)blockIdx.x * PPW + slot;
    const bool pv = p < total;
    const long pc_ = pv ? p : 0;
    const int ox = (int)(pc_ % wo);
    const long r = pc_ / wo;
    const int oy = (int)(r % ho);
    const long b = r / ho;
    int iy0, ix0;
    float wy[4], wx[4];
    resample_plan<0>(oy, iy0, wy);
    resample_plan<0>(ox, ix0, wx);
    float4 u4 = make_float4(0.f, 0.f, 0.f, 0.f);
    const float* __restrict__ xin = a.x + 4 * q;
#pragma unroll
    for (int ta = 0; ta < 4; ++ta) {
        const int yy = clampi(iy0 - 1 + ta, 0, a.H - 1);
#pragma unroll
        for (int tb = 0; tb < 4; ++tb) {
            const int xx = clampi(ix0 - 1 + tb, 0, a.W - 1);
            const float wgt = wy[ta] * wx[tb];
            const float4 v = *reinterpret_cast<const float4*>(xin + ((b * a.H + yy) * (long)a.W + xx) * E);
            u4.x += wgt * v.x; u4.y += wgt * v.y; u4.z += wgt * v.z; u4.w += wgt * v.w;
        }
    }
    if (a.u_save && pv) *reinterpret_cast<float4*>(a.u_save + p * E + 4 * q) = u4;
    *reinterpret_cast<float4*>(ux + slot * LDU + 4 * q) = u4;
    __builtin_amdgcn_fence(__ATOMIC_RELEASE, "wavefront");
    __builtin_amdgcn_wave_barrier();
    __builtin_amdgcn_fence(__ATOMIC_ACQUIRE, "wavefront");
    float u[E];
#pragma unroll
    for (int k = 0; k < E / 4; ++k) {
        const float4 v = *reinterpret_cast<const float4*>(ux + slot * LDU + 4 * k);
        u[4 * k] = v.x; u[4 * k + 1] = v.y; u[4 * k + 2] = v.z; u[4 * k + 3] = v.w;
    }
    float o[NO];
#pragma unroll
    for (int j = 0; j < NO; ++j) o[j] = 0.f;
#pragma unroll
    for (int k = 0; k < E; ++k) {
        const float4 w0 = *reinterpret_cast<const float4*>(sW + k * (2 * E) + NO * q), w1 = *reinterpret_cast<const float4*>(sW + k * (2 * E) + NO * q + 4);
        o[0] += w0.x * u[k]; o[1] += w0.y * u[k]; o[2] += w0.z * u[k]; o[3] += w0.w * u[k];
        o[4] += w1.x * u[k]; o[5] += w1.y * u[k]; o[6] += w1.z * u[k]; o[7] += w1.w * u[k];
    }
#pragma unroll
    for (int j = 0; j < NO; ++j) o[j] += sB[NO * q + j];
    if (pv) {
        float4* yo = reinterpret_cast<float4*>(a.y + p * (2 * E) + NO * q);
        yo[0] = make_float4(o[0], o[1], o[2], o[3]);
        yo[1] = make_float4(o[4], o[5], o[6], o[7]);
    }
    if (a.g) {
        float s = 0.f;
#pragma unroll
        for (int j = 0; j < NO; ++j) s += o[j];
        const float mu = lane_group_sum<LPP>(s) * (1.0f / (2 * E));
        float vs = 0.f;
#pragma unroll
        for (int j = 0; j < NO; ++j) { const float d = o[j] - mu; vs += d * d; }
        const float rstd = __builtin_amdgcn_rsqf(lane_group_sum<LPP>(vs) * (1.0f / (2 * E)) + LG_EPS);
        if (pv && q >= LPP / 2) {
            const long HWo = (long)ho * wo, sp = (long)oy * wo + ox;
#pragma unroll
            for (int j = 0; j < NO; ++j) {
                const int n = NO * q + j;
                a.g[(b * E + (n - E)) * HWo + sp] = (o[j] - mu) * rstd * sNg[n] + sNb[n];
            }
        }
    }
}

int launch_down(int E, const DownArgs& a, hipStream_t s) {
    ProfScope prof__(LG_K_DOWN, s);
    const long total = (long)a.B * (a.H / 2) * (a.W / 2);
    const int ppw = 256 / (E / 4);
    int grid = (int)((total + ppw - 1) / ppw);
    if (E == 16) k_down<16><<<grid, 256, 0, s>>>(a);
    else if (E == 32) k_down<32><<<grid, 256, 0, s>>>(a);
    else { lg_set_error("down: E=%d unsupported", E); return -1; }
    LG_CHECK_LAUNCH();
    return 0;
}

#ifdef LG_UPF_STAMPS
__device__ unsigned long long g_upf_stamps[4096 * 4 * 12];
#define USTAMP(i) do { unsigned long long t__; asm volatile("s_memtime %0\n\ts_waitcnt lgkmcnt(0)" : "=s"(t__)); \
                       g_upf_stamps[((blockIdx.x & 4095) * 4 + (threadIdx.x >> 6)) * 12 + (i)] = t__; } while (0)
extern "C" __attribute__((visibility("default"))) int lg_debug_upf_stamps(unsigned long long* host) {
    return (int)hipMemcpyFromSymbol(host, HIP_SYMBOL(g_upf_stamps), sizeof(g_upf_stamps));
}
#else
#define USTAMP(i) do { } while (0)
#endif
template <int E>
__global__ __launch_bounds__(256) __attribute__((amdgpu_waves_per_eu(E == 16 ? 4 : 2, E == 16 ? 4 : 2))) void k_upfuse(UpFuseArgs a, int tiles_x, int tiles_y) {
    constexpr int TY = 8, TX = 32, SY = TY / 2 + 4, SX = TX / 2 + 4, NS = SY * SX , LDV = E + 4, Q = 2 * E / 4;
    USTAMP(0);
    constexpr int QP = Q + 1;
    __shared__ float4 srcb[NS * QP];
    __shared__ __attribute__((aligned(16))) float vb[NS * LDV];
    __shared__ float sFw[E * 2 * E], sFb[2 * E];
    const int hi = a.H / 2, wi = a.W / 2;
    int t = blockIdx.x;
    const int tx_i = t % tiles_x;
    t /= tiles_x;
    const int ty_i = t % tiles_y;
    const long b = t / tiles_y;
    const int Y0 = ty_i * TY, X0 = tx_i * TX;
// ... 287 lines not shown
```

### lgteun_amd/csrc/kernels.h

```cpp
#pragma once
#include "common.h"

int launch_pyr_down2(const void* pan, float* pan_l, int64_t planes, int H, int W, int dtype, hipStream_t s);
int launch_batch_assemble(const void* pan, const void* lr, const void* mul, const float* pan_l, int64_t N, const int32_t* idx, int64_t idx_offset,
                          const uint32_t* flips, float* o_pan, float* o_lr, float* o_mul, float* o_pan_l, int B, int C, int H, int W, int h, int w,
                          int dtype, float divisor, int n_div, float post_scale, hipStream_t s);
size_t iqa_workspace_bytes(int B, int C, int H, int W, int no_ref);
int launch_iqa_ref(const float* pred, const float* gt, double* out, int B, int C, int H, int W, float scale, void* workspace,
                   size_t workspace_bytes, hipStream_t s);
int launch_iqa_no_ref(const float* pred, const float* pan, const float* ms, double* out, int B, int C, int H, int W, float scale,
                      void* workspace, size_t workspace_bytes, hipStream_t s);

struct DwArgs {
    const float* in;
    float* out;
    const float* w9;
    const float* bias;
    const float* sub;
    const float* z;
    const float* pan;
    const float* rw;
    const float* rb;
    const float* rtw;
    const float* rtb;
    const float* eta;
    int C, planes, hi, wi, ho, wo;
};
int launch_resample_dw(int mode, int epi, const DwArgs& a, hipStream_t s);
int launch_resample(int mode, const float* x, float* y, int planes, int hi, int wi, hipStream_t s);
struct DstepFwdArgs {
    const float* z;
    const float* ms;
    const float* pan;
    float* zout;
    float *t1, *r, *s1;
    float* pr;
    const float *d1w, *d1b, *d3w, *d3b, *dt1w, *dt1b, *dt3w, *dt3b, *rw, *rb, *rtw, *rtb, *eta;
    int B, C, N;
};
bool dstep_fused_ok(int C, int H, int W);
int launch_dstep_fwd(const DstepFwdArgs& a, hipStream_t s);

struct EmbedArgs {
    const float* z;
    float* x;
    float* g;
    const float *dww, *dwb, *w, *b, *lng, *lnb, *n1g, *n1b;
    int HW;
    long total;
};
int launch_embed(int C, const EmbedArgs& a, hipStream_t s);

struct DownArgs {
    const float* x;
    float* y;
    float* g;
    float* u_save;
    const float *w, *b, *n1g, *n1b;
    int B, H, W;
};
int launch_down(int E, const DownArgs& a, hipStream_t s);

struct UpFuseArgs {
    const float* xb;
    const float* skip;
    float* y;
    float* g;
    float* t_save;
    const float *upw, *upb, *fw, *fb, *n1g, *n1b;
    int B, H, W;
};
int launch_upfuse(int E, const UpFuseArgs& a, hipStream_t s);

struct TailArgs {
    const float* x;
    const float* z;
    float* out;
    const float *w, *b;
    int HW;
    long total;
};
int launch_tail(int C, const TailArgs& a, hipStream_t s);

struct FftArgs {
    const float* g;
    float* o;
    float* amp;
    float* pha;
    float* sgn;
    float* scratch;
    const float *ampw, *ampb, *phaw, *phab;
    int planes, ch, n;
    int h, w;
    int full = 0;
};
int launch_fftmix(const FftArgs& a, hipStream_t s);
size_t fft_scratch_floats(int planes, int n);
size_t fft_scratch_floats_hw(int planes, int h, int w);
bool fft_is_generic(int h, int w);

struct AttnArgs {
    const float* x;
    const float* o2;
    float* y;
    const float* posT;
    const float* pos;
    const float *ln1g, *ln1b, *qkvw, *qkvb, *projw, *projb;
    int B, h, w;
    int dropout;
    uint64_t seed;
    int bf16;
    float* save_o = nullptr;
    float* save_l = nullptr;
    const float* scales = nullptr;
};
int launch_attn(int e, const AttnArgs& a, hipStream_t s);
int launch_attn_m(int e, const AttnArgs& a, hipStream_t s);
int launch_pos_transpose(const float* pos, float* posT, hipStream_t s);
int launch_pos_transpose_n(int n, const float* const* pos, float* const* posT, hipStream_t s);

struct Ffn1Args {
    const float* x;
    void* a1s;
    void* g1s;
    void* h2;
    int hbf;
    int tile16;
    const float *ln2g, *ln2b, *w1, *b1, *w2, *b2;
    long P;
    void* wsplit;
    int wsplit_ready = 0;
    const float* scales;
};
struct FfnPrepJob { const float *ln2g, *ln2b, *w1, *b1, *w2, *b2, *dww, *dwb, *w3; int e; const float *ln1g, *ln1b, *qkvw, *qkvb; };
#define LG_MAX_FFN_PREP_JOBS 40
struct FfnPrepTable { FfnPrepJob j[LG_MAX_FFN_PREP_JOBS]; };
int launch_ffn_scales(int n, const FfnPrepJob* jobs, float* out, hipStream_t s, float* attn_out = nullptr);
struct SplitWJob { const float *w1, *w2, *w3, *scales; void* out; int e, np; };
struct SplitWTable { SplitWJob j[LG_MAX_FFN_PREP_JOBS]; };
int launch_split_w_jobs(int n, const SplitWJob* jobs, hipStream_t s);
int launch_ffn1(int e, const Ffn1Args& a, hipStream_t s);
struct Ffn2Args {
    const void* h2;
    const float* x;
    void* a3s;
    void* g3s;
    int hbf;
    float* y;
    float* g;
    const float *dww, *dwb, *w3, *b3, *n1g, *n1b;
    int B, h, w;
};
int launch_ffn2(int e, const Ffn2Args& a, hipStream_t s);
#define LG_FFN_NOT_FUSED (-1000)
int launch_ffn_fused(int e, const Ffn1Args& a1, const Ffn2Args& a2, hipStream_t s);
int launch_ffn_xs(const Ffn1Args& a1, const Ffn2Args& a2, hipStream_t s);
int launch_ffn_xr(const Ffn1Args& a1, const Ffn2Args& a2, hipStream_t s);
int launch_ffn_xp(const Ffn1Args& a1, const Ffn2Args& a2, hipStream_t s);
int launch_ffn_x32(const Ffn1Args& a1, const Ffn2Args& a2, hipStream_t s);
size_t ffn_wsplit_bytes(int e);
int launch_split_w(const float* w1, const float* w2, const float* w3, void* out, int e, int np, hipStream_t s, const float* scales = nullptr);
int launch_ffn_x64(const Ffn1Args& a1, const Ffn2Args& a2, hipStream_t s);

int launch_ln_split(int e, const float* x, const float* n1g, const float* n1b, float* g, int B, int HW, hipStream_t s);
```

Before: 6035 image-pairs/sec.

## Fuse LGT tail projection into final FFN xr kernel and vectorize x4 resample

```diff
diff --git a/include/lgteun_hip.h b/include/lgteun_hip.h
--- a/include/lgteun_hip.h
+++ b/include/lgteun_hip.h
@@ -56,7 +56,8 @@
 #define LG_VAR_FFN_H3_RECOMPUTE (1u << 15)
 #define LG_VAR_ATTN_BWD_RESTATS (1u << 16)
 #define LG_VAR_REDUCE_PER_BLOCK (1u << 17)
-#define LG_VAR_ALL 0x3ffffu
+#define LG_VAR_TAIL_LAUNCH (1u << 18)
+#define LG_VAR_ALL 0x7ffffu
 
 typedef struct lg_plan lg_plan;
 
diff --git a/lgteun_amd/_lib.py b/lgteun_amd/_lib.py
--- a/lgteun_amd/_lib.py
+++ b/lgteun_amd/_lib.py
@@ -34,6 +34,7 @@
 LG_VAR_FFN_H3_RECOMPUTE = 1 << 15
 LG_VAR_ATTN_BWD_RESTATS = 1 << 16
 LG_VAR_REDUCE_PER_BLOCK = 1 << 17
+LG_VAR_TAIL_LAUNCH = 1 << 18
 LG_OPT_ADAM, LG_OPT_ADAMW, LG_OPT_SGD, LG_OPT_RMSPROP = 0, 1, 2, 3
 LG_OPT_AMSGRAD, LG_OPT_NESTEROV, LG_OPT_CENTERED = 1, 2, 4
 LG_DT_U8, LG_DT_U16, LG_DT_F32 = 0, 1, 2
@@ -72,6 +73,8 @@
         v |= LG_VAR_ATTN_BWD_RESTATS
     if env.get('LG_REDUCE', '') == 'per_block':
         v |= LG_VAR_REDUCE_PER_BLOCK
+    if env.get('LG_TAIL', '') == 'launch':
+        v |= LG_VAR_TAIL_LAUNCH
     return v
 
 
diff --git a/lgteun_amd/csrc/api.hip b/lgteun_amd/csrc/api.hip
--- a/lgteun_amd/csrc/api.hip
+++ b/lgteun_amd/csrc/api.hip
@@ -142,6 +142,7 @@
         p->ffn_h3_re = (v & LG_VAR_FFN_H3_RECOMPUTE) ? 1 : 0;
         p->attn_restats = (v & LG_VAR_ATTN_BWD_RESTATS) ? 1 : 0;
         p->reduce_per_block = (v & LG_VAR_REDUCE_PER_BLOCK) ? 1 : 0;
+        p->tail_launch = (v & LG_VAR_TAIL_LAUNCH) ? 1 : 0;
     }
     p->off = (int64_t*)malloc(sizeof(int64_t) * n_offsets);
     memcpy(p->off, offsets, sizeof(int64_t) * n_offsets);
@@ -226,7 +227,7 @@
 }
 
 static int block_ffn_fwd(const lg_plan* pl, const float* P, int stage, int j, const BlockBufs& bb, float* g_next, int next_blk,
-                         int B, int flags, hipStream_t s, float* wsplit, const float* ffn_scales) {
+                         int B, int flags, hipStream_t s, float* wsplit, const float* ffn_scales, TailArgs* tail = nullptr) {
     int rc;
     Ffn1Args a1;
     const bool pre = pl->ffn_saves_preact(bb.e);
@@ -250,6 +251,11 @@
     a2.n1b = g_next ? P + pl->blk(stage, next_blk, B_LN1B) : nullptr;
     a2.B = B; a2.h = bb.h; a2.w = bb.w; a2.hbf = a1.hbf;
     a1.h2 = ((flags & LG_FLAG_SAVE) || bb.e == 64) ? bb.h2 : nullptr;
+    if (tail && !g_next && pl->cfg.C == 4 && !pl->tail_launch && ffn_fused_is_xr(bb.e, a1, a2)) {
+        a2.tail_w = tail->w; a2.tail_b = tail->b; a2.tail_z = tail->z; a2.tail_out = tail->out;
+        if (!(flags & LG_FLAG_SAVE)) a2.y = nullptr;
+        tail->out = nullptr;
+    }
     rc = launch_ffn_fused(bb.e, a1, a2, s);
     if (rc != LG_FFN_NOT_FUSED) return rc;
     a1.h2 = bb.h2;
@@ -339,12 +345,12 @@
     if ((rc = block_mixer_fwd(pl, P, stage, 3, nb.blk[3], posT + 3 * 8192, B, flags, seed, s, nb.fft_scratch, nb.attn_scales))) return rc;
     if ((rc = block_ffn_fwd(pl, P, stage, 3, nb.blk[3], nb.blk[4].g, 4, B, flags, s, nb.wsplit, nb.ffn_scales))) return rc;
     if ((rc = block_mixer_fwd(pl, P, stage, 4, nb.blk[4], posT + 4 * 8192, B, flags, seed, s, nb.fft_scratch, nb.attn_scales))) return rc;
-    if ((rc = block_ffn_fwd(pl, P, stage, 4, nb.blk[4], nullptr, 0, B, flags, s, nb.wsplit, nb.ffn_scales))) return rc;
     TailArgs ta;
     ta.x = nb.blk[4].xout; ta.z = z; ta.out = out;
     ta.w = P + pl->lgt(stage, L_TAILW); ta.b = P + pl->lgt(stage, L_TAILB);
     ta.HW = c.H * c.W; ta.total = (long)B * c.H * c.W;
-    return launch_tail(c.C, ta, s);
+    if ((rc = block_ffn_fwd(pl, P, stage, 4, nb.blk[4], nullptr, 0, B, flags, s, nb.wsplit, nb.ffn_scales, &ta))) return rc;
+    return ta.out ? launch_tail(c.C, ta, s) : 0;
 }
 
 extern "C" int lgteun_forward(const lg_plan* plan, const float* params, const float* ms, const float* pan, float* out,
@@ -424,6 +430,11 @@
     return launch_resample(mode, x, y, planes, hi, wi, (hipStream_t)stream);
 }
 
+extern "C" __attribute__((visibility("default"))) int lg_debug_resample_x4_scalar(const float* x, float* y, int32_t planes, int32_t hi, int32_t wi, void* stream) {
+    if (!x || !y || planes <= 0 || hi <= 0 || wi <= 0) { lg_set_error("debug_resample_x4_scalar: invalid argument"); return -1; }
+    return launch_resample(2, x, y, planes, hi, wi, (hipStream_t)stream, true);
+}
+
 extern "C" int lg_op_data_step(const lg_plan* plan, const float* params, int32_t stage, const float* z_in, const float* ms,
                                const float* pan, float* z_out, float* tmp, int32_t B, void* stream) {
     if (!plan || !params || !z_in || !ms || !pan || !z_out || !tmp || stage < 0 || stage >= plan->cfg.K) { lg_set_error("op_data_step: invalid argument"); return -1; }
@@ -440,6 +451,59 @@
     NetBufs nb;
     carve(plan, B, train, workspace, nb);
     return lgt_fwd(plan, params, stage, z, out, nb, B, flags, seed, (hipStream_t)stream);
+}
+
+extern "C" __attribute__((visibility("default"))) long long lg_debug_tail_y_offset(const lg_plan* plan, int32_t B, int32_t train) {
+    if (!plan || B <= 0 || train < 0 || train > 2) return -1;
+    NetBufs nb;
+    const uintptr_t base = 4096;
+    carve(plan, B, train, reinterpret_cast<void*>(base), nb);
+    return (long long)(reinterpret_cast<uintptr_t>(nb.blk[4].xout) - base);
+}
+
+extern "C" __attribute__((visibility("default"))) int lg_debug_ffn_tail(const lg_plan* plan, const float* params, int32_t stage, const float* x, const float* z,
+                                                                        float* out, float* y, float* scratch8, int32_t B, int32_t h, int32_t w, int32_t fused, void* stream) {
+    if (!plan || !params || !x || !z || !out || !scratch8 || B <= 0 || h <= 0 || w <= 0 || stage < 0 || stage >= plan->cfg.K || (!fused && !y)) { lg_set_error("debug_ffn_tail: invalid argument"); return -1; }
+    if (plan->cfg.C != 4) { lg_set_error("debug_ffn_tail: C = 4 only"); return -2; }
+    hipStream_t s = (hipStream_t)stream;
+    const float* P = params;
+    const int j = 4;
+    float* scales = nullptr;
+    int rc = 0;
+    if (plan->ffn_f16x2(16)) {
+        scales = scratch8;
+        FfnPrepJob q;
+        q.ln2g = P + plan->blk(stage, j, B_LN2G); q.ln2b = P + plan->blk(stage, j, B_LN2B);
+        q.w1 = P + plan->blk(stage, j, B_W1); q.b1 = P + plan->blk(stage, j, B_B1); q.w2 = P + plan->blk(stage, j, B_W2); q.b2 = P + plan->blk(stage, j, B_B2);
+        q.dww = P + plan->blk(stage, j, B_DWW); q.dwb = P + plan->blk(stage, j, B_DWB); q.w3 = P + plan->blk(stage, j, B_W3);
+        q.e = 16;
+        q.ln1g = P + plan->blk(stage, j, B_LN1G); q.ln1b = P + plan->blk(stage, j, B_LN1B); q.qkvw = P + plan->blk(stage, j, B_QKVW); q.qkvb = P + plan->blk(stage, j, B_QKVB);
+        rc = launch_ffn_scales(1, &q, scales, s, nullptr);
+    }
+    Ffn1Args a1;
+    memset(&a1, 0, sizeof(a1));
+    a1.x = x;
+    a1.ln2g = P + plan->blk(stage, j, B_LN2G); a1.ln2b = P + plan->blk(stage, j, B_LN2B);
+    a1.w1 = P + plan->blk(stage, j, B_W1); a1.b1 = P + plan->blk(stage, j, B_B1);
+    a1.w2 = P + plan->blk(stage, j, B_W2); a1.b2 = P + plan->blk(stage, j, B_B2);
+    a1.P = (long)B * h * w;
+    a1.hbf = plan->hidden_bf16(16) ? 1 : 0;
+    a1.scales = scales;
+    Ffn2Args a2;
+    memset(&a2, 0, sizeof(a2));
+    a2.x = x; a2.y = y; a2.hbf = a1.hbf;
+    a2.dww = P + plan->blk(stage, j, B_DWW); a2.dwb = P + plan->blk(stage, j, B_DWB);
+    a2.w3 = P + plan->blk(stage, j, B_W3); a2.b3 = P + plan->blk(stage, j, B_B3);
+    a2.B = B; a2.h = h; a2.w = w;
+    TailArgs ta;
+    ta.x = y; ta.z = z; ta.out = out;
+    ta.w = P + plan->lgt(stage, L_TAILW); ta.b = P + plan->lgt(stage, L_TAILB);
+    ta.HW = h * w; ta.total = (long)B * h * w;
+    if (!rc && !ffn_fused_is_xr(16, a1, a2)) { lg_set_error("debug_ffn_tail: this plan's e = 16 feed_forward is not k_ffn_xr"); rc = -2; }
+    if (!rc && fused) { a2.tail_w = ta.w; a2.tail_b = ta.b; a2.tail_z = z; a2.tail_out = out; }
+    if (!rc) rc = launch_ffn_xr(a1, a2, s);
+    if (!rc && !fused) rc = launch_tail(4, ta, s);
+    return rc;
 }
 
 extern "C" int lg_op_block(const lg_plan* plan, const float* params, int32_t stage, int32_t blk, int32_t which, const float* x,
diff --git a/lgteun_amd/csrc/common.h b/lgteun_amd/csrc/common.h
--- a/lgteun_amd/csrc/common.h
+++ b/lgteun_amd/csrc/common.h
@@ -43,6 +43,7 @@
     bool attn_f16x2() const { return cfg.precision == 0 && !attn_bf16x3 && !attn_fwd_valu && ffn_tile == 0 && !ffn_bf16x3; }
     int attn_fwd_valu;
     int reduce_per_block;
+    int tail_launch;
     int dstep_tiles;
     bool dstep_fused(int h, int w) const;
     int bwd32_old;
diff --git a/lgteun_amd/csrc/k_ffn.hip b/lgteun_amd/csrc/k_ffn.hip
--- a/lgteun_amd/csrc/k_ffn.hip
+++ b/lgteun_amd/csrc/k_ffn.hip
@@ -1109,15 +1109,22 @@
     return 0;
 }
 
+bool ffn_fused_is_xr(int e, const Ffn1Args& a1, const Ffn2Args& a2) {
+    if (e != 16 || a1.tile16 != 0) return false;
+    const bool save = a1.h2 != nullptr;
+    if (a1.hbf) return !save || (!a1.a1s && !a1.g1s && a2.a3s && !a2.g3s);
+    return a1.scales && (!save || (!a1.a1s && !a1.g1s && !a2.g3s));
+}
+
 int launch_ffn_fused(int e, const Ffn1Args& a1, const Ffn2Args& a2, hipStream_t s) {
+    if (a2.tail_out && !ffn_fused_is_xr(e, a1, a2)) { lg_set_error("ffn: the tail epilogue exists in k_ffn_xr only"); return -2; }
     if (a1.hbf) {
 #ifdef LG_BUILD_AB
         if (e == 16 && a1.tile16 != 0) return launch_ffn_fused_bf_t<16>(a1, a2, s);
         if (e == 32 && (a1.tile16 != 0 || !a1.wsplit)) return launch_ffn_fused_bf_t<32>(a1, a2, s);
 #endif
         if (e == 16 && (a1.tile16 == 0 || a1.tile16 == 4)) {
-            const bool save = a1.h2 != nullptr, h2h3 = save && !a1.a1s && !a1.g1s && a2.a3s && !a2.g3s;
-            if (a1.tile16 == 0 && (!save || h2h3)) return launch_ffn_xr(a1, a2, s);
+            if (ffn_fused_is_xr(e, a1, a2)) return launch_ffn_xr(a1, a2, s);
             return launch_ffn_xs(a1, a2, s);
         }
         if (e == 32 && a1.tile16 == 0 && a1.wsplit) return launch_ffn_x32(a1, a2, s);
@@ -1135,8 +1142,7 @@
 #endif
     if (e == 16 && a1.tile16 == 1) return launch_ffn_strip(a1, a2, s);
     if (e == 16) {
-        const bool save = a1.h2 != nullptr, h2h3 = save && !a1.a1s && !a1.g1s && !a2.g3s;
-        if (a1.tile16 == 0 && a1.scales && (!save || h2h3)) return launch_ffn_xr(a1, a2, s);
+        if (ffn_fused_is_xr(e, a1, a2)) return launch_ffn_xr(a1, a2, s);
         return launch_ffn_xs(a1, a2, s);
     }
     if (e == 32) return (a1.tile16 == 0 && a1.wsplit) ? launch_ffn_x32(a1, a2, s) : launch_ffn_fused_t<32>(a1, a2, s);
diff --git a/lgteun_amd/csrc/k_ffn_xr.hip b/lgteun_amd/csrc/k_ffn_xr.hip
--- a/lgteun_amd/csrc/k_ffn_xr.hip
+++ b/lgteun_amd/csrc/k_ffn_xr.hip
@@ -38,7 +38,7 @@
 constexpr size_t OFF_W = 0;
 constexpr size_t OFF_TAPS = OFF_W + (size_t)NFRAG * 64 * 16;
 constexpr size_t OFF_PAR = OFF_TAPS + (size_t)N1 * 9 * 4;
-constexpr int P_B1 = 0, P_B2 = 64, P_DWB = 128, P_B3 = 192, P_N1G = 208, P_N1B = 224, P_FLOATS = 240;
+constexpr int P_B1 = 0, P_B2 = 64, P_DWB = 128, P_B3 = 192, P_N1G = 208, P_N1B = 224, P_TW = 240, P_TB = 304, P_FLOATS = 308;
 constexpr size_t OFF_RING = OFF_PAR + (size_t)P_FLOATS * 4;
 constexpr size_t LDS_BYTES = OFF_RING + (size_t)RING * HX * LDR * 4;
 static_assert(LDS_BYTES <= 80 * 1024, "two workgroups per CU");
@@ -61,6 +61,11 @@
     v = __uint_as_float(r.x) + __uint_as_float(r.y);
     r = __builtin_amdgcn_permlane16_swap(__float_as_uint(v), __float_as_uint(v), false, false);
     return __uint_as_float(r.x) + __uint_as_float(r.y);
+}
+__device__ __forceinline__ void xg_gather(float v, float (&q)[4]) {
+    const u32x2_t r = __builtin_amdgcn_permlane32_swap(__float_as_uint(v), __float_as_uint(v), false, false);
+    const u32x2_t lo = __builtin_amdgcn_permlane16_swap(r.x, r.x, false, false), hi = __builtin_amdgcn_permlane16_swap(r.y, r.y, false, false);
+    q[0] = __uint_as_float(lo.x); q[1] = __uint_as_float(lo.y); q[2] = __uint_as_float(hi.x); q[3] = __uint_as_float(hi.y);
 }
 __device__ __forceinline__ f32x4_t mfma_h(u32x4_t a, u32x4_t b, f32x4_t c) {
     return __builtin_amdgcn_mfma_f32_16x16x32_f16(__builtin_bit_cast(f16x8_t, a), __builtin_bit_cast(f16x8_t, b), c, 0, 0, 0);
@@ -111,7 +116,7 @@
 
 }
 
-template <int SAVE, int NP>
+template <int SAVE, int NP, bool TAIL>
 __global__ __launch_bounds__(256) __attribute__((amdgpu_waves_per_eu(2))) void k_ffn_xr(Ffn1Args a1, Ffn2Args a2, int tiles_x, int strips_y, int nstrips,
                                                                                        int SH, int dS) {
     using namespace xr;
@@ -188,6 +193,8 @@
         const float* const ng = a2.g ? a2.n1g : a2.b3;
         const float* const nb_ = a2.g ? a2.n1b : a2.b3;
         const float png = ng[te], pnb = nb_[te];
+        float ptw = 0.f, ptb = 0.f;
+        if constexpr (TAIL) { ptw = a2.tail_w[tn]; ptb = a2.tail_b[t & 3]; }
         lng = *reinterpret_cast<const float4*>(a1.ln2g + 4 * g);
         lnb = *reinterpret_cast<const float4*>(a1.ln2b + 4 * g);
         float2 v1[4], v2[8], v3[2];
@@ -233,6 +240,10 @@
             sPar[P_B3 + t] = pb3 * S3;
             sPar[P_N1G + t] = a2.g ? png : 0.f;
             sPar[P_N1B + t] = a2.g ? pnb : 0.f;
+        }
+        if constexpr (TAIL) {
+            if (t < 4 * E) sPar[P_TW + t] = ptw;
+            if (t < 4) sPar[P_TB + t] = ptb;
         }
     }
     lng = make_float4(lng.x * sx, lng.y * sx, lng.z * sx, lng.w * sx);
@@ -523,6 +534,16 @@
             if (role == 3) halo(IC<1>{}, IC<2>{}, y0 + 1, TY * HX, 8, xh + 2, part9, &geo9);
             XSTAMP(2);
             xh[0] = xload(y0 + TY + 1, 2 * wave); xh[1] = xload(y0 + TY + 1, 2 * wave + 1); xh[2] = xload(y0 + TY + 1, 8);
+            float zt[2] = {0.f, 0.f};
+            if constexpr (TAIL) {
+#pragma unroll
+                for (int r2 = 0; r2 < 2; ++r2) {
+                    int gl = g;
+                    asm volatile("" : "+v"(gl));
+                    const int y = min(y0 + ty0 + r2, h - 1), x = min(x0 + c, w - 1);
+                    zt[r2] = a2.tail_z[(uint32_t)(((int)b * 4 + gl) * (h * w) + y * w + x)];
+                }
+            }
             __syncthreads();
             XR_TAKE_TURNS();
             XSTAMP(3);
@@ -617,8 +638,24 @@
 #ifdef LG_XR_NOSTORE
                     if (ok && o0 == 12345.678f) *reinterpret_cast<float4*>(a2.y + ((b * h + y) * (long)w + x) * E + 4 * g) = make_float4(o0, o1, o2, o3);
 #else
-                    if (ok) *reinterpret_cast<float4*>(a2.y + ((b * h + y) * (long)w + x) * E + 4 * g) = make_float4(o0, o1, o2, o3);
-#endif
+                    if (ok && (!TAIL || a2.y)) *reinterpret_cast<float4*>(a2.y + ((b * h + y) * (long)w + x) * E + 4 * g) = make_float4(o0, o1, o2, o3);
+#endif
+                    if constexpr (TAIL) {
+                        float yq[4][4];
+                        xg_gather(o0, yq[0]); xg_gather(o1, yq[1]); xg_gather(o2, yq[2]); xg_gather(o3, yq[3]);
+                        float v = 0.f;
+#pragma unroll
+                        for (int j = 0; j < 4; ++j) {
+                            const float4 tw = *reinterpret_cast<const float4*>(sPar + P_TW + 4 * (4 * g + j));
+                            v += tw.x * yq[0][j];
+                            v += tw.y * yq[1][j];
+                            v += tw.z * yq[2][j];
+                            v += tw.w * yq[3][j];
+                        }
+                        int gl = g;
+                        asm volatile("" : "+v"(gl));
+                        if (ok) a2.tail_out[(uint32_t)(((int)b * 4 + gl) * (h * w) + y * w + x)] = v + sPar[P_TB + gl] + zt[r2];
+                    }
                     if (a2.g) {
                         const float s = xg_sum((o0 + o1) + (o2 + o3));
                         const float mu = s * (1.0f / E);
@@ -654,10 +691,10 @@
     ProfScope prof__(LG_K_FFN2, s);
     static DeviceOnce attr_once;
     if (attr_once.need()) {
-        hipError_t e = hipFuncSetAttribute((const void*)k_ffn_xr<0, 2>, hipFuncAttributeMaxDynamicSharedMemorySize, (int)LDS_BYTES);
-        if (e == hipSuccess) e = hipFuncSetAttribute((const void*)k_ffn_xr<3, 2>, hipFuncAttributeMaxDynamicSharedMemorySize, (int)LDS_BYTES);
-        if (e == hipSuccess) e = hipFuncSetAttribute((const void*)k_ffn_xr<0, 1>, hipFuncAttributeMaxDynamicSharedMemorySize, (int)LDS_BYTES);
-        if (e == hipSuccess) e = hipFuncSetAttribute((const void*)k_ffn_xr<3, 1>, hipFuncAttributeMaxDynamicSharedMemorySize, (int)LDS_BYTES);
+        const void* const kerns[8] = {(const void*)k_ffn_xr<0, 2, false>, (const void*)k_ffn_xr<3, 2, false>, (const void*)k_ffn_xr<0, 1, false>, (const void*)k_ffn_xr<3, 1, false>,
+                                      (const void*)k_ffn_xr<0, 2, true>,  (const void*)k_ffn_xr<3, 2, true>,  (const void*)k_ffn_xr<0, 1, true>,  (const void*)k_ffn_xr<3, 1, true>};
+        hipError_t e = hipSuccess;
+        for (int i = 0; i < 8 && e == hipSuccess; ++i) e = hipFuncSetAttribute(kerns[i], hipFuncAttributeMaxDynamicSharedMemorySize, (int)LDS_BYTES);
         if (e != hipSuccess) { lg_set_error("ffn_xr: hipFuncSetAttribute: %s", hipGetErrorString(e)); return (int)e; }
         attr_once.done();
     }
@@ -673,11 +710,17 @@
     const int grid = nstrips < LG_XR_GRID ? nstrips : LG_XR_GRID;
     int dS = 0;
     if (LG_XR_UNEVEN && nstrips == LG_XR_GRID && LG_XR_GRID == 512 && (strips_y & 1) == 0 && SH >= 32 && a2.h % (2 * SH) == 0) dS = (SH * LG_XR_UNEVEN / 64 + 7) / 8 * 8;
+    const bool tail = a2.tail_out != nullptr;
+    if (tail && (a2.g || !a2.tail_w || !a2.tail_b || !a2.tail_z)) { lg_set_error("ffn_xr: the tail epilogue needs its four operands and no planar LayerNorm half"); return -2; }
+    if (!tail && !a2.y) { lg_set_error("ffn_xr: y may be null only with the tail epilogue"); return -2; }
+    auto go = [&](auto kern) { kern<<<grid, 256, LDS_BYTES, s>>>(a1, a2, tiles_x, strips_y, nstrips, SH, dS); };
     if (a1.hbf) {
-        if (save) k_ffn_xr<3, 1><<<grid, 256, LDS_BYTES, s>>>(a1, a2, tiles_x, strips_y, nstrips, SH, dS);
-        else k_ffn_xr<0, 1><<<grid, 256, LDS_BYTES, s>>>(a1, a2, tiles_x, strips_y, nstrips, SH, dS);
-    } else if (save) k_ffn_xr<3, 2><<<grid, 256, LDS_BYTES, s>>>(a1, a2, tiles_x, strips_y, nstrips, SH, dS);
-    else k_ffn_xr<0, 2><<<grid, 256, LDS_BYTES, s>>>(a1, a2, tiles_x, strips_y, nstrips, SH, dS);
+        if (tail) { if (save) go(k_ffn_xr<3, 1, true>); else go(k_ffn_xr<0, 1, true>); }
+        else if (save) go(k_ffn_xr<3, 1, false>);
+        else go(k_ffn_xr<0, 1, false>);
+    } else if (tail) { if (save) go(k_ffn_xr<3, 2, true>); else go(k_ffn_xr<0, 2, true>); }
+    else if (save) go(k_ffn_xr<3, 2, false>);
+    else go(k_ffn_xr<0, 2, false>);
     LG_CHECK_LAUNCH();
     return 0;
 }
diff --git a/lgteun_amd/csrc/k_pixel.hip b/lgteun_amd/csrc/k_pixel.hip
--- a/lgteun_amd/csrc/k_pixel.hip
+++ b/lgteun_amd/csrc/k_pixel.hip
@@ -14,10 +14,52 @@
     }
 }
 
-int launch_resample(int mode, const float* x, float* y, int planes, int hi, int wi, hipStream_t s) {
+__global__ __launch_bounds__(256) void k_resample_x4q(const float* __restrict__ x, float* __restrict__ y, int nquads, int hi, int wi) {
+    const int q = blockIdx.x * 256 + threadIdx.x;
+    if (q >= nquads) return;
+    const int ho = 4 * hi;
+    const int m = q % wi, r_ = q / wi, oy = r_ % ho, p = r_ / ho;
+    const float* __restrict__ src = x + (long)p * hi * wi;
+    int iy0;
+    float wy[4];
+    resample_plan<2>(oy, iy0, wy);
+    float v[4][5];
+#pragma unroll
+    for (int a = 0; a < 4; ++a) {
+        const int yy = clampi(iy0 - 1 + a, 0, hi - 1);
+#pragma unroll
+        for (int k = 0; k < 5; ++k) v[a][k] = src[yy * wi + clampi(m - 2 + k, 0, wi - 1)];
+    }
+    float o[4];
+#pragma unroll
+    for (int r = 0; r < 4; ++r) {
+        int ix0;
+        float wx[4];
+        resample_plan<2>(r, ix0, wx);
+        const int k0 = ix0 + 1;
+        float acc = 0.f;
+#pragma unroll
+        for (int a = 0; a < 4; ++a) {
+            float rr = 0.f;
+#pragma unroll
+            for (int b = 0; b < 4; ++b) rr += wx[b] * v[a][k0 + b];
+            acc += wy[a] * rr;
+        }
+        o[r] = acc;
+    }
+    *reinterpret_cast<float4*>(y + (long)q * 4) = make_float4(o[0], o[1], o[2], o[3]);
+}
+
+int launch_resample(int mode, const float* x, float* y, int planes, int hi, int wi, hipStream_t s, bool scalar) {
     int ho, wo;
     if (mode == 0) { ho = hi / 2; wo = wi / 2; } else if (mode == 1) { ho = hi * 2; wo = wi * 2; } else { ho = hi * 4; wo = wi * 4; }
     long total = (long)planes * ho * wo;
+    if (mode == 2 && !scalar && total / 4 < (1l << 31) - 256) {
+        const int nquads = (int)(total / 4);
+        k_resample_x4q<<<(nquads + 255) / 256, 256, 0, s>>>(x, y, nquads, hi, wi);
+        LG_CHECK_LAUNCH();
+        return 0;
+    }
     int grid = (int)((total + 255) / 256);
     if (grid > 4096) grid = 4096;
     if (mode == 0) k_resample<0><<<grid, 256, 0, s>>>(x, y, planes, hi, wi, ho, wo);
diff --git a/lgteun_amd/csrc/kernels.h b/lgteun_amd/csrc/kernels.h
--- a/lgteun_amd/csrc/kernels.h
+++ b/lgteun_amd/csrc/kernels.h
@@ -27,7 +27,7 @@
     int C, planes, hi, wi, ho, wo;
 };
 int launch_resample_dw(int mode, int epi, const DwArgs& a, hipStream_t s);
-int launch_resample(int mode, const float* x, float* y, int planes, int hi, int wi, hipStream_t s);
+int launch_resample(int mode, const float* x, float* y, int planes, int hi, int wi, hipStream_t s, bool scalar = false);
 struct DstepFwdArgs {
     const float* z;
     const float* ms;
@@ -150,10 +150,15 @@
     float* g;
     const float *dww, *dwb, *w3, *b3, *n1g, *n1b;
     int B, h, w;
+    const float* tail_w = nullptr;
+    const float* tail_b = nullptr;
+    const float* tail_z = nullptr;
+    float* tail_out = nullptr;
 };
 int launch_ffn2(int e, const Ffn2Args& a, hipStream_t s);
 #define LG_FFN_NOT_FUSED (-1000)
 int launch_ffn_fused(int e, const Ffn1Args& a1, const Ffn2Args& a2, hipStream_t s);
+bool ffn_fused_is_xr(int e, const Ffn1Args& a1, const Ffn2Args& a2);
 int launch_ffn_xs(const Ffn1Args& a1, const Ffn2Args& a2, hipStream_t s);
 int launch_ffn_xr(const Ffn1Args& a1, const Ffn2Args& a2, hipStream_t s);
 int launch_ffn_xp(const Ffn1Args& a1, const Ffn2Args& a2, hipStream_t s);
```

Result: no change. 6048 image-pairs/sec, median of 6 (+0.2%).
